# zhuker/lamejs

Measured on AMD Instinct MI355X. Metric: 1152-sample frames/s encoded (44.1kHz 128kbps CBR); bit-exact, higher is better.
Workload: dtype f64; 1 GPU; BASELINE configs[2]: stereo 44.1kHz 128kbps CBR, 1 stream(s) x 100000 synthetic sine frames per GPU; input=Int16 PCM resident in HBM, output=MP3 bytes in HBM, seed_repaired_frames=0, distinct_streams=1, distinct_devices=1

## Files before the change

### lamejs_amd/csrc/k_psy.h

```cpp
#pragma once
#include <type_traits>
#include "lhip_defs.h"
#include "lhip_wave.h"
#include "lhip_math.h"
#include "lhip_layout.h"

namespace lhip {

#ifdef LHIP_NO_FZ_PAD
LHIP_DEV int fzp(int a) { return a; }
LHIP_DEV int fzo(int c) { return c; }
#else
LHIP_DEV int fzp(int a) { return a + (a >> 5); }
LHIP_DEV int fzo(int c) { return c + (c >> 5); }
#endif
LHIP_DEV void fht_item0(float* fz, int base, int k1, int kx, int m) {
    const int k2 = k1 << 1, k3 = k2 + k1, k4 = k2 << 1;
    const int K1 = fzo(k1), K2 = fzo(k2), K3 = fzo(k3);
    float* fi = fz + fzp(base + m * k4);
    float* gi = fz + fzp(base + m * k4 + kx);
    double f0, f1, f2, f3;
    f1 = (double)fi[0] - (double)fi[K1];
    f0 = (double)fi[0] + (double)fi[K1];
    f3 = (double)fi[K2] - (double)fi[K3];
    f2 = (double)fi[K2] + (double)fi[K3];
    fi[K2] = (float)(f0 - f2);
    fi[0] = (float)(f0 + f2);
    fi[K3] = (float)(f1 - f3);
    fi[K1] = (float)(f1 + f3);
    f1 = (double)gi[0] - (double)gi[K1];
    f0 = (double)gi[0] + (double)gi[K1];
    f3 = LHIP_SQRT2 * (double)gi[K3];
    f2 = LHIP_SQRT2 * (double)gi[K2];
    gi[K2] = (float)(f0 - f2);
    gi[0] = (float)(f0 + f2);
    gi[K3] = (float)(f1 - f3);
    gi[K1] = (float)(f1 + f3);
}
LHIP_DEV void fht_item1(float* fz, int base, int k1, int kx, int m, int i, const double* tw) {
    const int k2 = k1 << 1, k3 = k2 + k1, k4 = k2 << 1;
    const int K1 = fzo(k1), K2 = fzo(k2), K3 = fzo(k3);
    (void)kx;
    float* fi = fz + fzp(base + m * k4 + i);
    float* gi = fz + fzp(base + m * k4 + k1 - i);
    const double c1 = tw[4 * (i - 1) + 0], s1 = tw[4 * (i - 1) + 1], c2 = tw[4 * (i - 1) + 2], s2 = tw[4 * (i - 1) + 3];
    double a, b, g0, f0, f1, g1, f2, g2, f3, g3;
    b = s2 * (double)fi[K1] - c2 * (double)gi[K1];
    a = c2 * (double)fi[K1] + s2 * (double)gi[K1];
    f1 = (double)fi[0] - a;
    f0 = (double)fi[0] + a;
    g1 = (double)gi[0] - b;
    g0 = (double)gi[0] + b;
    b = s2 * (double)fi[K3] - c2 * (double)gi[K3];
    a = c2 * (double)fi[K3] + s2 * (double)gi[K3];
    f3 = (double)fi[K2] - a;
    f2 = (double)fi[K2] + a;
    g3 = (double)gi[K2] - b;
    g2 = (double)gi[K2] + b;
    b = s1 * f2 - c1 * g3;
    a = c1 * f2 + s1 * g3;
    fi[K2] = (float)(f0 - a);
    fi[0] = (float)(f0 + a);
    gi[K3] = (float)(g1 - b);
    gi[K1] = (float)(g1 + b);
    b = c1 * g2 - s1 * f3;
    a = s1 * g2 + c1 * f3;
    gi[K2] = (float)(g0 - a);
    gi[0] = (float)(g0 + a);
    fi[K3] = (float)(f1 - b);
    fi[K1] = (float)(f1 + b);
}
LHIP_DEV void fht_pass(float* fz, int n, int k1, int kx, int lane, int nl, int base, const double* tw) {
    const int items = n / 8, nz = items / kx, kx1 = kx - 1;
    for (int t = lane - base; t < nz; t += nl) if (t >= 0) fht_item0(fz, 0, k1, kx, t);
    for (int t = lane - base; t < items - nz; t += nl) if (t >= 0) { const int m = t / kx1; fht_item1(fz, 0, k1, kx, m, 1 + t - m * kx1, tw); }
}

LHIP_DEV void fht_pass_blocks(float* fz, int nb, int n, int k1, int kx, int lane, int nl, const double* tw) {
    const int items = n / 8, nz = items / kx, kx1 = kx - 1, n1 = items - nz;
    for (int t = lane; t < nb * nz; t += nl) { const int b = t / nz; fht_item0(fz, b * n, k1, kx, t - b * nz); }
    for (int t = lane; t < nb * n1; t += nl) {
        const int b = t / n1, r = t - b * n1, m = r / kx1;
        fht_item1(fz, b * n, k1, kx, m, 1 + r - m * kx1, tw);
    }
}

struct PsyALds {
    float fz[BLKSIZE + BLKSIZE / 32];
    float fs[3][BLKSIZE_s];
    float fs_pad[3 * BLKSIZE_s / 32];
};
static_assert(offsetof(PsyALds, fs_pad) == offsetof(PsyALds, fs) + sizeof(float) * 3 * BLKSIZE_s, "the short transform buffer is one flat padded array");
#define PSYA_FE(L) ((L).fz)
#define PSYA_FES(L, b) ((L).fs[b])
#define PSYA_EB(L) ((L).fz + 516)
#define PSYA_MX(L) ((L).fz + 516 + CBANDS)
#define PSYA_AV(L) ((L).fz + 516 + 2 * CBANDS)
#define PSYA_EBS(L, b) ((L).fz + 516 + (3 + (b)) * CBANDS)

#if defined(LHIP_PHASE_PROF) && !defined(LHIP_HOSTSIM)
#define PSY_STAMP(i) psy_t_[i] = __builtin_amdgcn_s_memtime()
#define PSY_FLUSH() do { if (lane == 0 && ((gslot & 63) == 0 || (W.ngslots <= 4 && ch == 0 && gslot - sd.gslot0 == 1))) {    if (psy_t_[2] == 0) psy_t_[2] = psy_t_[1]; \
    for (int i_ = 0; i_ < 7; i_++) atomicAdd((unsigned long long*)W.prof + 22 + i_, psy_t_[i_ + 1] - psy_t_[i_]); atomicAdd((unsigned long long*)W.prof + 54, 1ull); } } while (0)
#define PSY_DECL() unsigned long long psy_t_[8] = {0, 0, 0, 0, 0, 0, 0, 0}
#else
#define PSY_STAMP(i) do {} while (0)
#define PSY_FLUSH() do {} while (0)
#define PSY_DECL() do {} while (0)
#endif
template <int K> LHIP_DEV int guarded_f32_of_sum(const double (&p)[K], double scale, double add, float* out) {
#if LHIP_NL == 1
    (void)p; (void)scale; (void)add; (void)out;
    return 0;
#else
    double s = 0.0;
#pragma unroll
    for (int k = 0; k < K; k++) s += p[k];
    s = wave_sumd(s);
    const float lo = (float)((s * (1.0 - 2e-13)) * scale + add), hi = (float)((s * (1.0 + 2e-13)) * scale + add);
    *out = lo;
#ifdef LHIP_WAVESIM
    if (lo == hi) {
        const float ref = (float)(wave_seq_sum<K>(p) * scale + add);
        if (ref != lo) { fprintf(stderr, "wavesim: guarded_f32_of_sum disagrees with the sequential sum (%a vs %a)\n", (double)lo, (double)ref); abort(); }
    }
#endif
    return lo == hi;
#endif
}

template <int F32, int UNIT, int MIX>
LHIP_DEV void psya_stage_new(const PcmSrc& P, int first, int lane, float* fz) {
    typedef typename std::conditional<F32 != 0, float, int16_t>::type elem_t;
    const int str = UNIT ? 1 : P.stride;
    const elem_t* src = (const elem_t*)P.src + (int64_t)first * str;
    if (MIX == 2) {
        const elem_t* src2 = (const elem_t*)P.src2 + (int64_t)first * str;
        enum { STG = 8 };
        for (int i0 = lane; i0 < BLKSIZE; i0 += LHIP_NL * STG) {
            typename std::conditional<F32 != 0, float, int>::type ra[STG], rb[STG];
#pragma unroll
            for (int k = 0; k < STG; k++) {
                int i = i0 + LHIP_NL * k;
                if (i >= BLKSIZE) i = BLKSIZE - 1;
                ra[k] = src[i * str]; rb[k] = src2[i * str];
            }
#pragma unroll
            for (int k = 0; k < STG; k++) { LHIP_PIN_LOADED(ra[k]); LHIP_PIN_LOADED(rb[k]); }
#pragma unroll
            for (int k = 0; k < STG; k++) {
                const int i = i0 + LHIP_NL * k;
                float v = F32 ? pcm_f32_clean((float)ra[k], P.limit) : (float)ra[k];
                if (P.do_scale) v = (float)((double)v * P.scale);
                v = pcm_mix(P, v, F32 ? pcm_f32_clean((float)rb[k], P.limit) : (float)rb[k]);
                if (i < BLKSIZE) fz[i] = v;
            }
        }
        return;
    }
    for (int i = lane; i < BLKSIZE; i += LHIP_NL) {
        float v = F32 ? pcm_f32_clean((float)src[i * str], P.limit) : (float)src[i * str];
        if (P.do_scale) v = (float)((double)v * P.scale);
        if (MIX) v = pcm_mix(P, v, 0.f);
        fz[i] = v;
    }
}

template <int PART = 0>
LHIP_DEV void kb_psyA(const Tables& T, const Workspace& W, const StreamDesc* SD, const StreamIO* IO, int gslot, int ch, int lane, PsyALds& L) {
    const int C = T.channels_out, Cp = T.psy_channels;
    const int st = W.gslot_stream[gslot];
    const StreamDesc sd = SD[st];
    const int q = gslot - sd.gslot0 - 1;
    if (q < 0) return;
    if (PART != 4 && ch < 2) {
        const PcmSrc P = pcm_source(T, W, sd, IO[st], ch);
        const int b0 = 576 * q + 304;
        if (!P.plane && b0 >= P.mf) {
            if (!P.mix) {
                if (!P.f32 && P.stride == 1) psya_stage_new<0, 1, 0>(P, b0 - P.mf, lane, L.fz);
                else if (!P.f32) psya_stage_new<0, 0, 0>(P, b0 - P.mf, lane, L.fz);
                else psya_stage_new<1, 0, 0>(P, b0 - P.mf, lane, L.fz);
            } else if (P.mix == 1) {
                if (!P.f32) psya_stage_new<0, 0, 1>(P, b0 - P.mf, lane, L.fz);
                else psya_stage_new<1, 0, 1>(P, b0 - P.mf, lane, L.fz);
            } else {
                if (!P.f32) psya_stage_new<0, 0, 2>(P, b0 - P.mf, lane, L.fz);
                else psya_stage_new<1, 0, 2>(P, b0 - P.mf, lane, L.fz);
            }
        } else {
            for (int i = lane; i < BLKSIZE; i += LHIP_NL) L.fz[i] = pcm_at(P, b0 + i);
        }
        wave_sync();
    }
#define buf(i) L.fz[i]
    const int64_t o = (int64_t)gslot * Cp + ch;
    PSY_DECL();
    PSY_STAMP(0);

    if (PART == 4) goto psya_tail;
    if (PART == 0 || PART == 1) {
        const float* fir = L.fz + 397;
        enum { HO = (576 + LHIP_NL - 1) / LHIP_NL };
        float* mag = &L.fs[0][0];
        if (ch >= 2) {
            const float* hl = W.hpf + (int64_t)gslot * 2 * 576;
            for (int i = lane; i < 576; i += LHIP_NL) {
                const double l = hl[i], r = hl[576 + i];
                float v = (ch == 2) ? (float)(l + r) : (float)(l - r);
                mag[i] = v < 0 ? -v : v;
            }
        } else {
            double x[HO + 21];
#pragma unroll
            for (int t = 0; t < HO + 21; t++) { const int n = HO * lane + t; x[t] = (n < 576 + 21) ? (double)fir[n] : 0.0; }
#pragma unroll
            for (int k = 0; k < HO; k++) {
                double sum1 = x[k + 10], sum2 = 0.0;
#pragma unroll
                for (int j = 0; j < 9; j += 2) {
                    sum1 += T.hpf_fircoef[j] * (x[k + j] + x[k + 21 - j]);
                    sum2 += T.hpf_fircoef[j + 1] * (x[k + j + 1] + x[k + 21 - j - 1]);
                }
                float v = (float)(sum1 + sum2);
                if (Cp == 4 && HO * lane + k < 576) W.hpf[((int64_t)gslot * 2 + ch) * 576 + HO * lane + k] = v;
                v = v < 0 ? -v : v;
                if (HO * lane + k < 576) mag[HO * lane + k] = v;
            }
        }
        wave_sync();
        enum { KP = (64 + LHIP_NL - 1) / LHIP_NL };
        float pk[9];
#pragma unroll
        for (int sbk = 0; sbk < 9; sbk++) {
            float m = 1.0f;
            for (int u = 0; u < KP; u++) { const float v = mag[sbk * 64 + lane + LHIP_NL * u]; if (m < v) m = v; }
            pk[sbk] = m;
        }
        wave_sync();
        {
            int pb[9];
#pragma unroll
            for (int sbk = 0; sbk < 9; sbk++) __builtin_memcpy(&pb[sbk], &pk[sbk], 4);
            wave_max_n(pb);
#pragma unroll
            for (int sbk = 0; sbk < 9; sbk++) __builtin_memcpy(&pk[sbk], &pb[sbk], 4);
        }
        if (lane == 0) {
#pragma unroll
            for (int sbk = 0; sbk < 9; sbk++) W.peaks[o * PK_STRIDE + sbk] = pk[sbk];
        }
    }
    if (PART == 1) return;

    PSY_STAMP(1);
    if (ch >= 2) {
        const float* fl = W.fht + (int64_t)gslot * 2 * FHT_STRIDE;
        for (int i = lane; i < FHT_STRIDE; i += LHIP_NL) {
            const double l = fl[i], r = fl[FHT_STRIDE + i];
            const float v = (ch == 2) ? (float)((l + r) * LHIP_SQRT2 * 0.5) : (float)((l - r) * LHIP_SQRT2 * 0.5);
            if (i < BLKSIZE) L.fz[fzp(i)] = v; else (&L.fs[0][0])[fzp(i - BLKSIZE)] = v;
        }
        wave_sync();
    } else {
    for (int it = lane; it < 3 * (BLKSIZE_s / 8); it += LHIP_NL) {
        const int b = it / (BLKSIZE_s / 8), j = it - b * (BLKSIZE_s / 8);
        const int k = (576 / 3) * (b + 1);
        const int i = T.fft_rv_tbl[j << 2] & 0xff;
        float* x = &L.fs[0][0] + fzp(b * BLKSIZE_s + 4 * j);
        double f0, f1, f2, f3, w;
        f0 = (double)T.window_s[i] * (double)buf(i + k);
        w = (double)T.window_s[0x7f - i] * (double)buf(i + k + 0x80);
        f1 = f0 - w; f0 = f0 + w;
        f2 = (double)T.window_s[i + 0x40] * (double)buf(i + k + 0x40);
        w = (double)T.window_s[0x3f - i] * (double)buf(i + k + 0xc0);
        f3 = f2 - w; f2 = f2 + w;
        x[0] = (float)(f0 + f2); x[2] = (float)(f0 - f2); x[1] = (float)(f1 + f3); x[3] = (float)(f1 - f3);
        f0 = (double)T.window_s[i + 0x01] * (double)buf(i + k + 0x01);
        w = (double)T.window_s[0x7e - i] * (double)buf(i + k + 0x81);
        f1 = f0 - w; f0 = f0 + w;
        f2 = (double)T.window_s[i + 0x41] * (double)buf(i + k + 0x41);
        w = (double)T.window_s[0x3e - i] * (double)buf(i + k + 0xc1);
        f3 = f2 - w; f2 = f2 + w;
        x[fzo(BLKSIZE_s / 2) + 0] = (float)(f0 + f2); x[fzo(BLKSIZE_s / 2) + 2] = (float)(f0 - f2);
        x[fzo(BLKSIZE_s / 2) + 1] = (float)(f1 + f3); x[fzo(BLKSIZE_s / 2) + 3] = (float)(f1 - f3);
    }
    {
        enum { KL = (BLKSIZE / 8 + LHIP_NL - 1) / LHIP_NL };
        float xin[KL][8];
#pragma unroll
        for (int u = 0; u < KL; u++) {
            const int jj = lane + LHIP_NL * u;
            if (jj < BLKSIZE / 8) {
                const int i = T.fft_rv_tbl[jj] & 0xff;
                xin[u][0] = buf(i); xin[u][1] = buf(i + 0x200); xin[u][2] = buf(i + 0x100); xin[u][3] = buf(i + 0x300);
                xin[u][4] = buf(i + 0x001); xin[u][5] = buf(i + 0x201); xin[u][6] = buf(i + 0x101); xin[u][7] = buf(i + 0x301);
            }
        }
        wave_sync();
#pragma unroll
        for (int u = 0; u < KL; u++) {
            const int jj = lane + LHIP_NL * u;
            if (jj < BLKSIZE / 8) {
                const int i = T.fft_rv_tbl[jj] & 0xff;
                float* x = L.fz + fzp(4 * jj);
                double f0, f1, f2, f3, w;
                f0 = (double)T.window[i] * (double)xin[u][0];
                w = (double)T.window[i + 0x200] * (double)xin[u][1];
                f1 = f0 - w; f0 = f0 + w;
                f2 = (double)T.window[i + 0x100] * (double)xin[u][2];
                w = (double)T.window[i + 0x300] * (double)xin[u][3];
                f3 = f2 - w; f2 = f2 + w;
                x[0] = (float)(f0 + f2); x[2] = (float)(f0 - f2); x[1] = (float)(f1 + f3); x[3] = (float)(f1 - f3);
                f0 = (double)T.window[i + 0x001] * (double)xin[u][4];
                w = (double)T.window[i + 0x201] * (double)xin[u][5];
                f1 = f0 - w; f0 = f0 + w;
                f2 = (double)T.window[i + 0x101] * (double)xin[u][6];
                w = (double)T.window[i + 0x301] * (double)xin[u][7];
                f3 = f2 - w; f2 = f2 + w;
                x[fzo(BLKSIZE / 2) + 0] = (float)(f0 + f2); x[fzo(BLKSIZE / 2) + 2] = (float)(f0 - f2);
                x[fzo(BLKSIZE / 2) + 1] = (float)(f1 + f3); x[fzo(BLKSIZE / 2) + 3] = (float)(f1 - f3);
            }
        }
    }
    wave_sync();

    PSY_STAMP(2);
    {
        int off = 0;
#pragma unroll
        for (int k1 = 4, kx = 2; k1 < BLKSIZE; k1 <<= 2, kx <<= 2) {
            fht_pass(L.fz, BLKSIZE, k1, kx, lane, LHIP_NL, 0, T.fht_twiddle + 4 * off);
            if (k1 < BLKSIZE_s) fht_pass_blocks(&L.fs[0][0], 3, BLKSIZE_s, k1, kx, lane, LHIP_NL, T.fht_twiddle + 4 * off);
            wave_sync();
            off += kx - 1;
        }
    }
    if (Cp == 4) {
        float* fo = W.fht + ((int64_t)gslot * 2 + ch) * FHT_STRIDE;
        for (int i = lane; i < FHT_STRIDE; i += LHIP_NL) fo[i] = (i < BLKSIZE) ? L.fz[fzp(i)] : (&L.fs[0][0])[fzp(i - BLKSIZE)];
    }
    }

    PSY_STAMP(3);
    {
        enum { KE = (BLKSIZE / 2 + 1 + LHIP_NL - 1) / LHIP_NL, KS = (3 * (BLKSIZE_s / 2 + 1) + LHIP_NL - 1) / LHIP_NL };
        float el[KE], es[KS];
#pragma unroll
        for (int u = 0; u < KE; u++) {
            const int j = lane + LHIP_NL * u;
            el[u] = 0.f;
            if (j == 0) { const float e0 = L.fz[0]; el[u] = (float)((double)e0 * (double)e0); }
            else if (j <= BLKSIZE / 2) { const double re = L.fz[fzp(j)], im = L.fz[fzp(BLKSIZE - j)]; el[u] = (float)((re * re + im * im) * 0.5); }
        }
#pragma unroll
        for (int u = 0; u < KS; u++) {
            const int it = lane + LHIP_NL * u;
            es[u] = 0.f;
            if (it < 3 * (BLKSIZE_s / 2 + 1)) {
                const int b = it / (BLKSIZE_s / 2 + 1), j = it - b * (BLKSIZE_s / 2 + 1);
                const float* fsf = &L.fs[0][0];
                if (j == 0) { const float e0 = fsf[fzp(b * BLKSIZE_s)]; es[u] = (float)((double)e0 * (double)e0); }
                else { const double re = fsf[fzp(b * BLKSIZE_s + j)], im = fsf[fzp(b * BLKSIZE_s + BLKSIZE_s - j)]; es[u] = (float)((re * re + im * im) * 0.5); }
            }
        }
        wave_sync();
#pragma unroll
        for (int u = 0; u < KE; u++) { const int j = lane + LHIP_NL * u; if (j <= BLKSIZE / 2) PSYA_FE(L)[j] = el[u]; }
#pragma unroll
        for (int u = 0; u < KS; u++) {
            const int it = lane + LHIP_NL * u;
            if (it < 3 * (BLKSIZE_s / 2 + 1)) { const int b = it / (BLKSIZE_s / 2 + 1), j = it - b * (BLKSIZE_s / 2 + 1); PSYA_FES(L, b)[j] = es[u]; }
        }
    }
    wave_sync();

    PSY_STAMP(4);
    {
        enum { K = (BLKSIZE / 2) / LHIP_NL };
        double pr[K];
#pragma unroll
        for (int k = 0; k < K; k++) { const int i = K * lane + k; pr[k] = (double)PSYA_FE(L)[i] * (double)T.eql_w[i]; }
        if (ch < 2) {
            float lf;
            if (!guarded_f32_of_sum<K>(pr, T.VO_SCALE, 0.0, &lf)) lf = (float)(wave_seq_sum<K>(pr) * T.VO_SCALE);
            if (lane == 0) W.loud[(int64_t)gslot * C + ch] = lf;
        }
        if (Cp == 4) {
#pragma unroll
            for (int k = 0; k < K; k++) { const int i = K * lane + k; pr[k] = (i >= 11) ? (double)PSYA_FE(L)[i] : 0.0; }
            const double last = (double)PSYA_FE(L)[BLKSIZE / 2];
            float tf;
            if (!guarded_f32_of_sum<K>(pr, 1.0, last, &tf)) tf = (float)(wave_seq_sum<K>(pr) + last);
            if (lane == 0) W.tot_ener[(int64_t)gslot * 4 + ch] = tf;
        }
    }

    PSY_STAMP(5);
    if (PART == 3) return;
psya_tail:
#if LHIP_NL == 1
    LHIP_LANE_ONCE(b, 0, T.npart_l) {
        double ebb = 0, m = 0;
        int j = T.lineoff_l[b];
        for (int i = 0; i < T.numlines_l[b]; ++i, ++j) {
            const double el = PSYA_FE(L)[j];
            ebb += el;
            if (m < el) m = el;
        }
        PSYA_EB(L)[b] = (float)ebb;
        PSYA_MX(L)[b] = (float)m;
        PSYA_AV(L)[b] = (float)(ebb * (double)T.rnumlines_l[b]);
    }
#else
    {
        enum { KF = 8 };
        static_assert(BLKSIZE / 2 == KF * LHIP_NL, "psy_fold is laid out for 8 lines per lane");
        const int32_t* pf = T.psy_fold + 3 * lane;
        const uint32_t marks = (uint32_t)pf[0], pw0 = (uint32_t)pf[1], pw1 = (uint32_t)pf[2];
        LHIP_LANE_ONCE(b, 0, CBANDS) PSYA_MX(L)[b] = 0.f;
        double tq[KF], keep[KF];
        float ev[KF];
#pragma unroll
        for (int k = 0; k < KF; k++) { ev[k] = PSYA_FE(L)[KF * lane + k]; tq[k] = (double)ev[k]; keep[k] = one_unless_bit(marks, k); }
        const float e512 = PSYA_FE(L)[BLKSIZE / 2];
        wave_sync();
        {
            float m = 0.f;
#pragma unroll
            for (int k = 0; k < KF; k++) {
                m = ((marks >> k) & 1u) ? ev[k] : fmax_nonneg(m, ev[k]);
                const int bnd = (int)(((k < 4 ? pw0 : pw1) >> (8 * (k & 3))) & 0xffu);
                float mm = m;
                if (lane == LHIP_NL - 1 && k == KF - 1 && !((marks >> (8 + k)) & 1u)) mm = fmax_nonneg(mm, e512);
                if (((marks >> (8 + k)) & 1u) || k == KF - 1) { int32_t bits; __builtin_memcpy(&bits, &mm, 4); lds_max((int32_t*)&PSYA_MX(L)[bnd], bits); }
            }
            if (lane == LHIP_NL - 1 && ((marks >> (8 + KF - 1)) & 1u)) {
                int32_t bits; __builtin_memcpy(&bits, &e512, 4); lds_max((int32_t*)&PSYA_MX(L)[T.npart_l - 1], bits);
            }
        }
        const int nsteps = (T.psy_maxlen_l + KF - 1) / KF + 1;
        double carry = 0.0;
        for (int st = 0; st + 1 < nsteps; st++) {
            double sacc = carry;
#pragma unroll
            for (int k = 0; k < KF; k++) sacc = __builtin_fma(sacc, keep[k], tq[k]);
            carry = wave_shr1d(sacc, 0.0);
        }
        {
            double sacc = carry;
#pragma unroll
            for (int k = 0; k < KF; k++) { sacc = __builtin_fma(sacc, keep[k], tq[k]); tq[k] = sacc; }
        }
#pragma unroll
        for (int k = 0; k < KF; k++) {
            const int bnd = (int)(((k < 4 ? pw0 : pw1) >> (8 * (k & 3))) & 0xffu);
            if ((marks >> (8 + k)) & 1u) { PSYA_EB(L)[bnd] = (float)tq[k]; PSYA_AV(L)[bnd] = (float)(tq[k] * (double)T.rnumlines_l[bnd]); }
        }
        if (lane == LHIP_NL - 1) {
            const int bl = T.npart_l - 1;
            const double ebb = ((marks >> (8 + KF - 1)) & 1u) ? (double)e512 : tq[KF - 1] + (double)e512;
            PSYA_EB(L)[bl] = (float)ebb; PSYA_AV(L)[bl] = (float)(ebb * (double)T.rnumlines_l[bl]);
        }
    }
#endif
    for (int it = lane; it < 3 * T.npart_s; it += LHIP_NL) {
        const int sblock = it / T.npart_s, b = it - sblock * T.npart_s;
        double ebb = 0;
        int j = T.lineoff_s[b];
        for (int i = 0; i < T.numlines_s[b]; ++i, ++j) ebb += (double)PSYA_FES(L, sblock)[j];
        PSYA_EBS(L, sblock)[b] = (float)ebb;
    }
    wave_sync();

    PSY_STAMP(6);
    for (int b = lane; b < CBANDS; b += LHIP_NL) {
        int k = 0;
        float ebv = 0.f;
        if (b < T.npart_l) {
            const int last = T.npart_l - 1;
            const int lo = b > 0 ? b - 1 : b, hi = b < last ? b + 1 : b;
            double a, m;
            int nl;
            if (b == 0) { a = (double)PSYA_AV(L)[0] + (double)PSYA_AV(L)[1]; nl = T.numlines_l[0] + T.numlines_l[1] - 1; }
            else if (b == last) { a = (double)PSYA_AV(L)[b - 1] + (double)PSYA_AV(L)[b]; nl = T.numlines_l[b - 1] + T.numlines_l[b] - 1; }
            else { a = (double)PSYA_AV(L)[b - 1] + (double)PSYA_AV(L)[b] + (double)PSYA_AV(L)[b + 1]; nl = T.numlines_l[b - 1] + T.numlines_l[b] + T.numlines_l[b + 1] - 1; }
            if (a > 0.0) {
                m = PSYA_MX(L)[lo];
                for (int t = lo + 1; t <= hi; t++) if (m < (double)PSYA_MX(L)[t]) m = PSYA_MX(L)[t];
                a = 20.0 * (m * (double)(hi - lo + 1) - a) / (a * nl);
                k = js_toint32(a);
                if (k > 8) k = 8;
            }
            ebv = PSYA_EB(L)[b];
        }
        W.eb_l[o * EBL_STRIDE + b] = ebv;
        W.mask_idx[o * EBL_STRIDE + b] = k;
    }
    for (int b = lane; b < CBANDS; b += LHIP_NL) {
        float ecbv[3] = {0.f, 0.f, 0.f}, ebv[3] = {0.f, 0.f, 0.f};
        if (b < T.npart_s) {
            enum { MT = 12 };
            const int k0 = T.s3ind_s[2 * b], k1 = T.s3ind_s[2 * b + 1], j0 = T.s3off_s[b];
            float cf[MT];
#pragma unroll
            for (int u = 0; u < MT; u++) cf[u] = (k0 + u <= k1) ? T.s3_ss[j0 + u] : 0.f;
            for (int sblock = 0; sblock < 3; sblock++) {
                const float* e = PSYA_EBS(L, sblock);
                double ecb = (double)cf[0] * (double)e[k0];
#pragma unroll
                for (int u = 1; u < MT; u++) if (k0 + u <= k1) ecb += (double)cf[u] * (double)e[k0 + u];
                for (int kk = k0 + MT; kk <= k1; kk++) ecb += (double)T.s3_ss[j0 + (kk - k0)] * (double)e[kk];
                ecbv[sblock] = (float)ecb;
                ebv[sblock] = e[b];
            }
        }
        for (int sblock = 0; sblock < 3; sblock++) {
            W.ecb_s[o * EBS_STRIDE + sblock * CBANDS + b] = ecbv[sblock];
            W.eb_s[o * EBS_STRIDE + sblock * CBANDS + b] = ebv[sblock];
        }
    }
    PSY_STAMP(7);
    if (PART == 0 || PART == 2) PSY_FLUSH();
#undef buf
}

LHIP_DEV int attack_flags_raw(const Tables& T, const float* cur, const float* prev, int chn) {
    const double thr = (chn == 3) ? T.attackthre_s : T.attackthre;
    float ai[4];
    ai[0] = (float)((double)prev[6] / (double)prev[4]);
    const double refv[3] = {(double)prev[7], (double)cur[1], (double)cur[4]};
    for (int t = 0; t < 3; t++) {
        double p = cur[3 * t];
        const double r = refv[t];
        if (p > r) p = p / r;
        else if (r > p * 10.0) p = r / (p * 10.0);
        else p = 0.0;
        ai[t + 1] = (float)p;
    }
    double en_short[4];
    en_short[0] = 0.0;
    for (int i = 0; i < 3; i++) en_short[0] += (double)prev[i + 6];
    en_short[1] = 0.0 + (double)cur[0]; en_short[2] = 0.0 + (double)cur[3]; en_short[3] = 0.0 + (double)cur[6];
    int a[4];
    for (int j = 0; j < 4; j++) a[j] = ((double)ai[j] > thr) ? 1 : 0;
    for (int i = 1; i < 4; i++) {
        double ratio;
        if (en_short[i - 1] > en_short[i]) ratio = en_short[i - 1] / en_short[i];
        else ratio = en_short[i] / en_short[i - 1];
        if (ratio < 1.7) { a[i] = 0; if (i == 1) a[0] = 0; }
    }
    return a[0] | (a[1] << 1) | (a[2] << 2) | (a[3] << 3);
}

LHIP_DEV void kb_scan_raw(const Tables& T, const Workspace& W, const StreamDesc* SD, int gslot) {
    const int Cp = T.psy_channels;
    const StreamDesc sd = SD[W.gslot_stream[gslot]];
    if (gslot - sd.gslot0 - 1 < 0) return;
    for (int ch = 0; ch < Cp; ch++) {
        const int64_t o = (int64_t)gslot * Cp + ch;
        W.att_raw[o] = attack_flags_raw(T, W.peaks + o * PK_STRIDE, W.peaks + (o - Cp) * PK_STRIDE, ch);
    }
}

LHIP_DEV int last_attack_after(const Workspace& W, int C, int gcarry, int gslot, int ch) {
    int flips = 0, g = gslot;
    for (;;) {
        if (g == gcarry) { const int v = W.last_attack[(int64_t)g * C + ch] != 0; return flips ? !v : v; }
        const int raw = W.att_raw[(int64_t)g * C + ch];
        const int a0 = raw & 1, a1 = (raw >> 1) & 1, a2 = (raw >> 2) & 1;
        int v;
        if (!a2) v = 0;
        else if (!a1) v = 1;
        else if (!a0) v = 0;
        else { flips ^= 1; g--; continue; }
        return flips ? !v : v;
    }
}

LHIP_DEV void kb_scan_attack(const Tables& T, const Workspace& W, const StreamDesc* SD, int gslot) {
    const int C = T.channels_out, Cp = T.psy_channels;
    const StreamDesc sd = SD[W.gslot_stream[gslot]];
    if (gslot - sd.gslot0 - 1 < 0) return;
    int ul[2] = {1, 1};
    for (int ch = 0; ch < Cp; ch++) {
        const int last = last_attack_after(W, Cp, sd.gslot0, gslot - 1, ch);
        const int raw = W.att_raw[(int64_t)gslot * Cp + ch];
        int a0 = raw & 1, a1 = (raw >> 1) & 1, a2 = (raw >> 2) & 1, a3 = (raw >> 3) & 1;
        if (a0 != 0 && last != 0) a0 = 0;
        if ((a0 + a1 + a2 + a3) != 0) {
            if (ch < 2) ul[ch] = 0;
            else ul[0] = ul[1] = 0;
            if (a1 != 0 && a0 != 0) a1 = 0;
            if (a2 != 0 && a1 != 0) a2 = 0;
            if (a3 != 0 && a2 != 0) a3 = 0;
        }
        W.att_clean[(int64_t)gslot * Cp + ch] = a0 | (a1 << 1) | (a2 << 2) | (a3 << 3);
        W.ul_tmp[(int64_t)gslot * Cp + ch] = a2;
    }
    if (T.short_blocks_coupled && !(ul[0] != 0 && ul[1] != 0)) ul[0] = ul[1] = 0;
    for (int ch = 0; ch < C; ch++) W.uselong[(int64_t)gslot * C + ch] = ul[ch];
}

LHIP_DEV void kb_scan_blocktype(const Tables& T, const Workspace& W, const StreamDesc* SD, int gslot) {
    const int C = T.channels_out;
    const StreamDesc sd = SD[W.gslot_stream[gslot]];
    const int q = gslot - sd.gslot0 - 1;
    if (q < 0) return;
    for (int ch = 0; ch < C; ch++) {
        int old;
        if (q == 0) old = W.tent[(int64_t)sd.gslot0 * C + ch];
        else {
            const int ul1 = W.uselong[(int64_t)(gslot - 1) * C + ch];
            int pshort;
            if (q == 1) pshort = W.tent[(int64_t)sd.gslot0 * C + ch] == SHORT_TYPE;
            else pshort = W.uselong[(int64_t)(gslot - 2) * C + ch] == 0;
            old = ul1 ? (pshort ? STOP_TYPE : NORM_TYPE) : SHORT_TYPE;
        }
        const int ul = W.uselong[(int64_t)gslot * C + ch];
        W.prev_short[(int64_t)gslot * C + ch] = (old == SHORT_TYPE) ? 1 : 0;
        int bt = NORM_TYPE;
        if (ul != 0) { if (old == SHORT_TYPE) bt = STOP_TYPE; }
        else {
            bt = SHORT_TYPE;
            if (old == NORM_TYPE) old = START_TYPE;
            if (old == STOP_TYPE) old = SHORT_TYPE;
        }
        W.blocktype[(int64_t)gslot * C + ch] = old;
        W.tent[(int64_t)gslot * C + ch] = bt;
    }
    const int Cp = T.psy_channels;
    for (int ch = 0; ch < Cp; ch++) W.last_attack[(int64_t)gslot * Cp + ch] = W.ul_tmp[(int64_t)gslot * Cp + ch];
}

#if defined(LHIP_HOSTSIM) && defined(LHIP_WAVESIM)
enum { ATH_NT = 128, ATH_SEG = 2 };
LHIP_DEV void block_sync() { wg_barrier(); }
LHIP_DEV int block_any(int p) { static int any_ = 0; wg_barrier(); if (p) any_ = 1; wg_barrier(); const int r = any_; wg_barrier(); any_ = 0; return r; }
#elif defined(LHIP_HOSTSIM)
enum { ATH_NT = 1, ATH_SEG = 1 << 20 };
LHIP_DEV void block_sync() {}
LHIP_DEV int block_any(int p) { return p != 0; }
#else
enum { ATH_NT = 1024, ATH_SEG = 16 };
LHIP_DEV void block_sync() { __syncthreads(); }
LHIP_DEV int block_any(int p) { return __syncthreads_or(p); }
#endif
struct AthLds { double e_adj[ATH_NT + 1], e_lim[ATH_NT + 1]; int known[ATH_NT + 1], first_reset[ATH_NT + 1]; double c_adj, c_lim, c_mp; };

LHIP_DEV void ath_step(const Tables& T, double max_pow, double& adj, double& lim) {
    if (T.ATH_useAdjust == 0) { adj = 1.0; return; }
    if (max_pow > 0.03125) {
        if (adj >= 1.0) adj = 1.0;
        else if (adj < lim) adj = lim;
        lim = 1.0;
    } else {
        const double adj_lim_new = 31.98 * max_pow + 0.000625;
        if (adj >= adj_lim_new) {
            adj *= adj_lim_new * 0.075 + 0.925;
            if (adj < adj_lim_new) adj = adj_lim_new;
        } else {
            if (lim >= adj_lim_new) adj = adj_lim_new;
            else if (adj < lim) adj = lim;
        }
        lim = adj_lim_new;
    }
}

LHIP_DEV double ath_max_pow(const Tables& T, const Workspace& W, const StreamDesc& sd, int C, int k) {
    const int GR = T.mode_gr;
    const int64_t g0 = (int64_t)(sd.gslot0 + GR * k) * C, g1 = g0 + C;
    double max_pow = W.loud[g0], gr2_max = (GR == 2) ? (double)W.loud[g1] : 0.0;
    if (C == 2) { max_pow += (double)W.loud[g0 + 1]; if (GR == 2) gr2_max += (double)W.loud[g1 + 1]; }
    else { max_pow += max_pow; gr2_max += gr2_max; }
    if (GR == 2) max_pow = max_pow > gr2_max ? max_pow : gr2_max;
    max_pow *= 0.5;
    max_pow *= T.ATH_aaSensitivityP;
    return max_pow;
}

LHIP_DEV void kb_scan_ath(const Tables& T, const Workspace& W, const StreamDesc* SD, int st, int tid, AthLds& L) {
    const int C = T.channels_out;
    const StreamDesc sd = SD[st];
    if (tid == 0) { L.c_adj = W.ath_adjust[sd.fslot0]; L.c_lim = W.ath_limit[sd.fslot0]; L.c_mp = 0.0; }
    block_sync();
    for (int k0 = 0; k0 < sd.nframes; k0 += ATH_NT * ATH_SEG) {
        const int rem = sd.nframes - k0;
        const int n = rem < ATH_NT * ATH_SEG ? rem : ATH_NT * ATH_SEG;
        const int seglen = (n + ATH_NT - 1) / ATH_NT;
        const int s0 = tid * seglen < n ? tid * seglen : n, s1 = (tid + 1) * seglen < n ? (tid + 1) * seglen : n;
        const double cadj = L.c_adj, clim = L.c_lim, prev_mp = L.c_mp;
        {
            int fr = -1;
            if (T.ATH_useAdjust != 0) {
                double pm = (s0 < s1) ? (s0 > 0 ? ath_max_pow(T, W, sd, C, k0 + s0 - 1) : prev_mp) : 0.0;
                for (int k = s0; k < s1; k++) {
                    const double m = ath_max_pow(T, W, sd, C, k0 + k);
                    if (pm > 0.03125 && m > 0.03125) { fr = k; break; }
                    pm = m;
                }
            } else if (s0 < s1) fr = s0;
            double a = 1.0, l = 1.0;
            if (fr >= 0) {
                l = (T.ATH_useAdjust != 0) ? 1.0 : clim;
                W.ath_adjust[sd.fslot0 + 1 + k0 + fr] = 1.0; W.ath_limit[sd.fslot0 + 1 + k0 + fr] = l;
                for (int k = fr + 1; k < s1; k++) {
                    ath_step(T, ath_max_pow(T, W, sd, C, k0 + k), a, l);
                    W.ath_adjust[sd.fslot0 + 1 + k0 + k] = a; W.ath_limit[sd.fslot0 + 1 + k0 + k] = l;
                }
            }
            L.first_reset[tid] = fr;
            L.known[tid + 1] = (fr >= 0) || (s0 >= s1);
            L.e_adj[tid + 1] = a; L.e_lim[tid + 1] = l;
            if (tid == 0) { L.known[0] = 1; L.e_adj[0] = cadj; L.e_lim[0] = clim; }
        }
        block_sync();
        int done = (s0 >= s1);
        for (int round = 0; round < ATH_NT + 1; round++) {
            int progressed = 0;
            if (!done && L.known[tid]) {
                double a = L.e_adj[tid], l = L.e_lim[tid];
                const int fr = L.first_reset[tid];
                const int stop = fr >= 0 ? fr : s1;
                for (int k = s0; k < stop; k++) {
                    ath_step(T, ath_max_pow(T, W, sd, C, k0 + k), a, l);
                    W.ath_adjust[sd.fslot0 + 1 + k0 + k] = a; W.ath_limit[sd.fslot0 + 1 + k0 + k] = l;
                }
                if (fr < 0) { L.e_adj[tid + 1] = a; L.e_lim[tid + 1] = l; }
                done = 1; progressed = 1;
            }
            block_sync();
            if (progressed && L.first_reset[tid] < 0) L.known[tid + 1] = 1;
            if (s0 >= s1 && L.known[tid] && !L.known[tid + 1]) { L.e_adj[tid + 1] = L.e_adj[tid]; L.e_lim[tid + 1] = L.e_lim[tid]; L.known[tid + 1] = 1; }
            block_sync();
            if (!block_any(!done || !L.known[tid + 1])) break;
        }
        if (s0 < s1 && s1 == n) { L.c_adj = L.e_adj[tid + 1]; L.c_lim = L.e_lim[tid + 1]; L.c_mp = ath_max_pow(T, W, sd, C, k0 + n - 1); }
        block_sync();
    }
}

struct PsyBTabs { double mt1[25], mt2[10], mt3[14], mtab[9]; };
enum { PSYB_S3_LDS = 1024 };
template <int NCH> struct PsyBLdsT : PsyBTabs {
    double ebm[CBANDS], athc[CBANDS];
    float thr_l[NCH][CBANDS + 2];
    union {
        struct { float thr_s[NCH][3][CBANDS + 2]; float E[NCH][E_STRIDE]; };
        float s3[PSYB_S3_LDS];
    };
};
typedef PsyBLdsT<2> PsyBLds;
typedef PsyBLdsT<4> PsyBLds4;

LHIP_DEV int ma_index16(double ratio) {
    const float t = fast_log2f((float)ratio) * 4.81647993062369912f;
    const float k = __builtin_floorf(t);
    const float fr = t - k;
    int i = -1;
    if (fr >= 2e-4f && fr <= 1.0f - 2e-4f) i = (int)k;
#ifdef LHIP_HOSTSIM
    if (i >= 0 && i != js_toint32(v8_log10_pos(ratio) * 16.0)) { fprintf(stderr, "hostsim: ma_index16 disagrees with the logarithm at %a\n", ratio); abort(); }
#endif
    return i;
}
LHIP_DEV int ma_index16_exact(double ratio) {
    int i = ma_index16(ratio);
    if (i < 0) i = js_toint32(v8_log10_pos(ratio) * 16.0);
    return i;
}

LHIP_DEV double mask_add_l(const Tables& T, const PsyBTabs& L, double ath_cb, double m1, double m2, int b) {
    double ratio;
    if (m2 > m1) {
        if (m2 < (m1 * T.ma_max_i2)) ratio = m2 / m1;
        else return (m1 + m2);
    } else {
        if (m1 >= (m2 * T.ma_max_i2)) return (m1 + m2);
        ratio = m1 / m2;
    }
    m1 += m2;
    if ((b + 3) <= 3 + 3) {
        if (ratio >= T.ma_max_i1) return m1;
        const int i = ma_index16_exact(ratio);
        return m1 * L.mt2[i];
    }
    const int i = ma_index16_exact(ratio);
    m2 = ath_cb;
    if (m1 < T.ma_max_m * m2) {
        if (m1 > m2) {
            double f = 1.0;
            if (i <= 13) f = L.mt3[i];
            const double r = v8_log10_pos(m1 / m2) * (10.0 / 15.0);
            return m1 * ((L.mt1[i] - f) * r + f);
        }
        if (i > 13) return m1;
        return m1 * L.mt3[i];
    }
    return m1 * L.mt1[i];
}


LHIP_DEV double ns_interp(double x, double y, double r) {
    if (r >= 1.0) return x;
    if (r <= 0.0) return y;
    if (y > 0.0) return v8_pow(x / y, r) * y;
    return 0.0;
}

template <int NCH> LHIP_DEV void kb_psyB(const Tables& T, const PowBase& pb10, const Workspace& W, const StreamDesc* SD, int gslot, int lane, PsyBLdsT<NCH>& L, int par = -1,
                                         int resv_size = 0, int resv_max = 0) {
    const int C = T.channels_out, Cp = T.psy_channels;
    const int st = W.gslot_stream[gslot];
    const StreamDesc sd = SD[st];
    const int q = gslot - sd.gslot0 - 1;
    if (q < 0) return;
    if (par >= 0 && q % T.mode_gr != par) return;
    double pcfact = 0.0;
    if (!T.disable_reservoir) pcfact = resv_max == 0 ? 0.0 : (double)resv_size / resv_max * 0.5;
    const int fs = sd.fslot0 + q / T.mode_gr;
    const double ath_adjust = W.ath_adjust[fs];
    for (int i = lane; i < 25; i += LHIP_NL) {
        L.mt1[i] = T.ma_table1[i];
        if (i < 10) L.mt2[i] = T.ma_table2[i];
        if (i < 14) L.mt3[i] = T.ma_table3[i];
        if (i < 9) L.mtab[i] = T.ma_tab[i];
    }
    wave_sync();

    for (int i = lane; i < T.n_s3_ll; i += LHIP_NL) L.s3[i] = T.s3_ll[i];
    LHIP_LANE_ONCE(k, 0, T.npart_l) L.athc[k] = (double)T.ATH_cb_l[k] * ath_adjust;
    for (int ch = 0; ch < Cp; ch++) {
        const int64_t o = (int64_t)gslot * Cp + ch;
        const float* eb_l = W.eb_l + o * EBL_STRIDE;
        const int32_t* midx = W.mask_idx + o * EBL_STRIDE;
        LHIP_LANE_ONCE(k, 0, T.npart_l) L.ebm[k] = (double)eb_l[k] * L.mtab[midx[k]];
        wave_sync();
        LHIP_LANE_ONCE(b, 0, T.npart_l) {
            const int k0 = T.s3ind[2 * b], k1 = T.s3ind[2 * b + 1], j0 = T.s3off_l[b];
            double ecb = (double)L.s3[j0] * L.ebm[k0];
            for (int kk = k0 + 1; kk <= k1; kk++)
                ecb = mask_add_l(T, L, L.athc[kk], ecb, (double)L.s3[j0 + (kk - k0)] * L.ebm[kk], kk - b);
            ecb *= 0.158489319246111;
            float thr = (float)ecb;
            if (!T.disable_reservoir) {
                const float n1 = W.nb1[(o - Cp) * EBL_STRIDE + b], n2 = W.nb2[(o - Cp) * EBL_STRIDE + b];
                if (pcfact > 0.0 && !W.prev_short[(int64_t)gslot * C + (ch & 1)]) {
                    const double a = 2 * (double)n1, b2 = 16 * (double)n2, m = a < b2 ? a : b2;
                    thr = (float)ns_interp(ecb < m ? ecb : m, ecb, pcfact);
                }
                W.nb2[o * EBL_STRIDE + b] = n1;
                W.nb1[o * EBL_STRIDE + b] = (float)ecb;
            }
            L.thr_l[ch][b] = thr;
        }
        wave_sync();
    }
    for (int ch = 0; ch < Cp; ch++) {
        const int64_t o = (int64_t)gslot * Cp + ch;
        const int pshort = W.prev_short[(int64_t)gslot * C + (ch & 1)];
        for (int it = lane; it < 3 * T.npart_s; it += LHIP_NL) {
            const int sblock = it / T.npart_s, b = it - sblock * T.npart_s;
            const float* e0 = W.ecb_s + o * EBS_STRIDE;
            const float* em = W.ecb_s + (o - Cp) * EBS_STRIDE;
            const float ecb = e0[sblock * CBANDS + b];
            const float nb1 = sblock >= 1 ? e0[(sblock - 1) * CBANDS + b] : em[2 * CBANDS + b];
            const float nb2 = sblock >= 2 ? e0[(sblock - 2) * CBANDS + b] : em[(sblock + 1) * CBANDS + b];
            double x = 2 * (double)nb1;
            float thr = (float)((double)ecb < x ? (double)ecb : x);
            if (pshort) {
                x = 16 * (double)nb2;
                const double y = thr;
                thr = (float)(x < y ? x : y);
            }
            L.thr_s[ch][sblock][b] = thr;
        }
    }
    wave_sync();

    for (int ch = 0; ch < Cp; ch++) {
        const int64_t o = (int64_t)gslot * Cp + ch;
        const float* eb_l = W.eb_l + o * EBL_STRIDE;
        float* Eo = L.E[ch];
        for (int sb = lane; sb < SBMAX_l; sb += LHIP_NL) {
            const int npart = T.npart_l;
            const int bstart = sb == 0 ? 0 : T.bo_l[sb - 1];
            float en_f = 0.f, thm_f = 0.f;
            if (sb == 0 || bstart < npart) {
                double enn = 0.0, thmm = 0.0;
                int b = bstart;
                if (sb > 0) {
                    const double w_next = 1.0 - (double)T.bo_l_weight[sb - 1];
                    enn = w_next * (double)eb_l[b];
                    thmm = w_next * (double)L.thr_l[ch][b];
                    b++;
                }
                const int bo = T.bo_l[sb];
                const int b_lim = bo < npart ? bo : npart;
                while (b < b_lim) { enn += (double)eb_l[b]; thmm += (double)L.thr_l[ch][b]; b++; }
                en_f = (float)enn; thm_f = (float)thmm;
                if (b < npart) {
                    const double w_curr = T.bo_l_weight[sb];
                    en_f = (float)((double)en_f + w_curr * (double)eb_l[b]);
                    thm_f = (float)((double)thm_f + w_curr * (double)L.thr_l[ch][b]);
                }
            }
            Eo[E_EN_L + sb] = en_f;
            Eo[E_THM_L + sb] = thm_f;
        }
        for (int it = lane; it < 3 * SBMAX_s; it += LHIP_NL) {
            const int sblock = it / SBMAX_s, sb = it - sblock * SBMAX_s;
            const float* ebs = W.eb_s + o * EBS_STRIDE + sblock * CBANDS;
            const float* thr = L.thr_s[ch][sblock];
            const int npart = T.npart_s;
            const int bstart = sb == 0 ? 0 : T.bo_s[sb - 1];
            float en_f = 0.f, thm_f = 0.f;
            if (sb == 0 || bstart < npart) {
                double enn = 0.0, thmm = 0.0;
                int b = bstart;
                if (sb > 0) {
                    const double w_next = 1.0 - (double)T.bo_s_weight[sb - 1];
                    enn = w_next * (double)ebs[b];
                    thmm = w_next * (double)thr[b];
                    b++;
                }
                const int bo = T.bo_s[sb];
                const int b_lim = bo < npart ? bo : npart;
                while (b < b_lim) { enn += (double)ebs[b]; thmm += (double)thr[b]; b++; }
                en_f = (float)enn; thm_f = (float)thmm;
                if (b < npart) {
                    const double w_curr = T.bo_s_weight[sb];
                    en_f = (float)((double)en_f + w_curr * (double)ebs[b]);
                    thm_f = (float)((double)thm_f + w_curr * (double)thr[b]);
                }
            }
            Eo[E_EN_S + sb * 3 + sblock] = en_f;
            Eo[E_THM_S + sb * 3 + sblock] = thm_f;
        }
    }
    wave_sync();
    for (int ch = 0; ch < Cp; ch++) {
        const int64_t o = (int64_t)gslot * Cp + ch;
        const float* pk = W.peaks + o * PK_STRIDE;
        const int att = W.att_clean[o];
        float* Eo = L.E[ch];
        LHIP_LANE_ONCE(sb, 0, SBMAX_s) {
            float prev = pcfact > 0.0 ? W.E[(o - Cp) * E_STRIDE + E_THM_S + sb * 3 + 2] : 0.f;
            for (int sblock = 0; sblock < 3; sblock++) {
                double thmm = Eo[E_THM_S + sb * 3 + sblock];
                thmm *= 0.8;
                if ((att >> (sblock + 1)) & 1) { const double p = ns_interp(prev, thmm, 0.6 * pcfact); thmm = thmm < p ? thmm : p; }
                if ((att >> sblock) & 1) { const double p = ns_interp(prev, thmm, 0.3 * pcfact); thmm = thmm < p ? thmm : p; }
                const double e3 = pk[sblock * 3 + 0], e4 = pk[sblock * 3 + 1], e5 = pk[sblock * 3 + 2];
                const double enn = e3 + e4 + e5;
                if (e5 * 6 < enn) {
                    thmm *= 0.5;
                    if (e4 * 6 < enn) thmm *= 0.5;
                }
                prev = (float)thmm;
                Eo[E_THM_S + sb * 3 + sblock] = prev;
            }
        }
    }
    wave_sync();
    if ((T.mode == 0 || T.mode == 1) && T.interChRatio > 0.0 && C > 1) {
        const double r_ = T.interChRatio;
        float nl[2] = {0.f, 0.f};
        for (int i = lane; i < SBMAX_l + 3 * SBMAX_s; i += LHIP_NL) {
            const int idx = E_THM_L + i;
            const double l = L.E[0][idx], r = L.E[1][idx];
            nl[0] = (float)(l + r * r_);
            nl[1] = (float)(r + l * r_);
            L.E[0][idx] = nl[0];
            L.E[1][idx] = nl[1];
        }
        wave_sync();
    }
    if constexpr (NCH == 4) if (Cp == 4) {
        const double msfix = T.msfix;
        const bool do_ns = d_abs(msfix) > 0.0;
        const double athlower_l = do_ns ? v8_pow_base(pb10, T.ATHlower * ath_adjust) : 0.0;
        const double athlower_s = athlower_l * ((double)BLKSIZE_s / BLKSIZE);
        for (int i = lane; i < SBMAX_l + 3 * SBMAX_s; i += LHIP_NL) {
            const int it = E_THM_L + i, ie = E_EN_L + i;
            const bool lng = i < SBMAX_l;
            const int sb = lng ? i : (i - SBMAX_l) / 3;
            float t0 = L.E[0][it], t1 = L.E[1][it], t2 = L.E[2][it], t3 = L.E[3][it];
            if (!((double)t0 > 1.58 * (double)t1 || (double)t1 > 1.58 * (double)t0)) {
                const double m = lng ? (double)T.mld_l[sb] : (double)T.mld_s[sb];
                double mld = m * (double)L.E[3][ie];
                const double lo1 = (double)t3 < mld ? (double)t3 : mld;
                const double rmid = (double)t2 > lo1 ? (double)t2 : lo1;
                mld = m * (double)L.E[2][ie];
                const double lo2 = (double)t2 < mld ? (double)t2 : mld;
                const double rside = (double)t3 > lo2 ? (double)t3 : lo2;
                t2 = (float)rmid; t3 = (float)rside;
            }
            if (do_ns) {
                const double ath = lng ? (double)T.ATH_cb_l[T.bm_l[sb]] * athlower_l : (double)T.ATH_cb_s[T.bm_s[sb]] * athlower_s;
                const double a0 = (double)t0 > ath ? (double)t0 : ath, a1 = (double)t1 > ath ? (double)t1 : ath;
                const double thmLR = a0 < a1 ? a0 : a1;
                double thmM = (double)t2 > ath ? (double)t2 : ath, thmS = (double)t3 > ath ? (double)t3 : ath;
                if (thmLR * (msfix * 2.0) < thmM + thmS) {
                    const double f = thmLR * (msfix * 2.0) / (thmM + thmS);
                    thmM *= f;
                    thmS *= f;
                }
                t2 = (float)(thmM < (double)t2 ? thmM : (double)t2);
                t3 = (float)(thmS < (double)t3 ? thmS : (double)t3);
            }
            L.E[2][it] = t2; L.E[3][it] = t3;
        }
        wave_sync();
    }
    for (int ch = 0; ch < Cp; ch++)
        for (int i = lane; i < E_STRIDE; i += LHIP_NL) W.E[((int64_t)gslot * Cp + ch) * E_STRIDE + i] = L.E[ch][i];
}

}
```

### lamejs_amd/csrc/lhip_api.cpp

```cpp
#include "../../include/lamejs_hip.h"
#include "lhip_defs.h"
#include "lhip_wave.h"
#include "lhip_math.h"
#include "lhip_layout.h"
#include "k_psy.h"
#include "k_fb.h"
#include "k_quant.h"
#if !defined(LHIP_HOSTSIM) || defined(LHIP_WAVESIM)
#include "k_quant_tail.h"
#endif
#include "k_quant_fast.h"
#include "k_quant_probe.h"
#include "k_bits.h"
#include "k_crc.h"
#include "k_ingest.h"
#include "k_gain.h"

#include <string>
#include <vector>
#include <map>
#include <mutex>
#include <thread>
#include <atomic>
#include <memory>
// ... 325 lines not shown
    std::vector<int16_t> zeros(z, 0);
    const void* l = zeros.data();
    const void* r = zeros.data();
    int64_t w = 0;
    const double end_padding = flush_end_padding(s);
    const int rc = tagged_call(&s, 1, nullptr, &out, &out_cap, &w, false, [&](uint8_t* const* o, const size_t* c, int64_t* wr) -> int {
        return encode_many(&s, 1, LHIP_PCM_S16, &l, &r, &z, o, c, wr, false, true, true); });
    if (rc < 0) return rc;
    s->mf_samples_to_encode = 0;
    if (s->tag) { s->tag->padding = end_padding; s->tag->flushed = true; }
    return w;
}

static int encode_batch_pcm_inner(lhip_stream* const* streams, size_t nstreams, int format, const void* const* left, const void* const* right,
                                  const size_t* nsamples, uint8_t* const* out, const size_t* out_cap, int64_t* written);
int lhip_encode_batch_pcm(lhip_stream* const* streams, size_t nstreams, int format, const void* const* left, const void* const* right,
                          const size_t* nsamples, uint8_t* const* out, const size_t* out_cap, int64_t* written) {
    return tagged_call(streams, nstreams, nsamples, out, out_cap, written, false, [&](uint8_t* const* o, const size_t* c, int64_t* wr) -> int {
        return encode_batch_pcm_inner(streams, nstreams, format, left, right, nsamples, o, c, wr); });
}
static int encode_batch_pcm_inner(lhip_stream* const* streams, size_t nstreams, int format, const void* const* left, const void* const* right,
                                  const size_t* nsamples, uint8_t* const* out, const size_t* out_cap, int64_t* written) {
    if (!fmt_ok(format)) { set_err("unknown sample format"); return LHIP_ERR_INTERNAL; }
    if (fmt_scanned(format) && streams && left && nsamples)
        for (size_t i = 0; i < nstreams; i++)
            if (streams[i] && streams[i]->magic == 0x4c484950 && !host_samples_ok(i, streams[i]->ts->T.channels_in, streams[i]->ts->T.pcm_limit, format, left[i], right ? right[i] : nullptr, nsamples[i])) {
                for (size_t k = 0; k < nstreams; k++) if (written) written[k] = LHIP_ERR_INTERNAL;
                return LHIP_ERR_INTERNAL;
            }
    if (nstreams > 1 && streams && left && nsamples && out && out_cap) {
        static const bool no_chunk = []() { const char* e = getenv("LAMEJS_HIP_NO_HOST_CHUNKS"); return e && e[0] == '1'; }();
        bool ok = !no_chunk;
        size_t total = 0;
        for (size_t i = 0; i < nstreams && ok; i++) {
            ok = streams[i] && streams[i]->magic == 0x4c484950 && streams[i]->ctx == streams[0]->ctx && streams[i]->ts.get() == streams[0]->ts.get() && left[i] && nsamples[i] > 0;
            if (ok) for (size_t k = 0; k < i; k++) if (streams[k] == streams[i]) { ok = false; break; }
            total += nsamples[i];
        }
        if (ok && streams[0]->ts->T.disable_reservoir && !streams[0]->ts->T.rs_frac) {
            const Tables& T = streams[0]->ts->T;
            if (total > (size_t)4 * host_chunk_schedule().first * 576 * T.mode_gr * T.rs_ratio) return encode_host_groups(streams, nstreams, format, left, right, nsamples, out, out_cap, written);
        }
    }
    return encode_many(streams, nstreams, format, left, right, nsamples, out, out_cap, written, false, true);
}
int lhip_encode_batch(lhip_stream* const* streams, size_t nstreams, const int16_t* const* left, const int16_t* const* right,
                      const size_t* nsamples, uint8_t* const* out, const size_t* out_cap, int64_t* written) {
    return lhip_encode_batch_pcm(streams, nstreams, LHIP_PCM_S16, (const void* const*)left, (const void* const*)right, nsamples, out, out_cap, written);
}

int lhip_flush_batch(lhip_stream* const* streams, size_t nstreams, uint8_t* const* out, const size_t* out_cap, int64_t* written) {
    std::vector<std::vector<int16_t>> zs(nstreams);
    std::vector<const void*> l(nstreams);
    std::vector<size_t> ns(nstreams);
    bool any_frac = false;
    for (size_t i = 0; i < nstreams; i++) any_frac |= streams[i] && streams[i]->magic == 0x4c484950 && streams[i]->ts->T.rs_frac;
    if (any_frac) {
        int rc = 0;
        for (size_t i = 0; i < nstreams; i++) {
            const int64_t w = lhip_flush(streams[i], out[i], out_cap[i]);
            if (written) written[i] = w;
            if (w < 0 && rc == 0) rc = (int)w;
        }
        return rc;
    }
    for (size_t i = 0; i < nstreams; i++) {
        if (!streams[i] || streams[i]->magic != 0x4c484950) { set_err("bad stream handle"); return LHIP_ERR_BAD_HANDLE; }
        ns[i] = flush_zeros(streams[i]);
        zs[i].assign(ns[i] ? ns[i] : 1, 0);
        l[i] = zs[i].data();
    }
    std::vector<double> end_padding(nstreams);
    for (size_t i = 0; i < nstreams; i++) end_padding[i] = flush_end_padding(streams[i]);
    const int rc = tagged_call(streams, nstreams, ns.data(), out, out_cap, written, false, [&](uint8_t* const* o, const size_t* c, int64_t* wr) -> int {
        return encode_many(streams, nstreams, LHIP_PCM_S16, l.data(), l.data(), ns.data(), o, c, wr, false, true, true); });
    if (rc >= 0) for (size_t i = 0; i < nstreams; i++) {
        streams[i]->mf_samples_to_encode = 0;
        if (streams[i]->tag && ns[i] > 0) { streams[i]->tag->padding = end_padding[i]; streams[i]->tag->flushed = true; }
    }
    return rc;
}

int lhip_encode_batch_device(lhip_stream* const* streams, size_t nstreams, const int16_t* const* d_left, const int16_t* const* d_right,
                             const size_t* nsamples, uint8_t* const* d_out, const size_t* out_cap, int64_t* written, int sync) {
    return lhip_encode_batch_device_pcm(streams, nstreams, LHIP_PCM_S16, (const void* const*)d_left, (const void* const*)d_right, nsamples, d_out, out_cap, written, sync);
}
int lhip_encode_batch_device_pcm(lhip_stream* const* streams, size_t nstreams, int format, const void* const* d_left, const void* const* d_right,
                                 const size_t* nsamples, uint8_t* const* d_out, const size_t* out_cap, int64_t* written, int sync) {
    if (!fmt_ok(format)) { set_err("unknown sample format"); return LHIP_ERR_INTERNAL; }
    return tagged_call(streams, nstreams, nsamples, d_out, out_cap, written, true, [&](uint8_t* const* o, const size_t* c, int64_t* wr) -> int {
        return encode_many(streams, nstreams, format, d_left, d_right, nsamples, o, c, wr, true, sync != 0); });
}
int64_t lhip_last_batch_rejected_samples(void) {
    if (g_rej_pending) {
        Context* ctx = g_rej_pending;
        g_rej_pending = nullptr;
        std::lock_guard<std::mutex> lk(ctx->mu);
        unsigned long long v = 0;
        if (!rt::set_device(ctx->device) || !rt::d2h(&v, ctx->ws.rejected.p, sizeof v, ctx->stream) || !rt::sync(ctx->stream)) return LHIP_ERR_INTERNAL;
        g_rejected = (int64_t)v;
    }
    return g_rejected;
}

struct StateHdr { uint32_t magic, bytes; int32_t mf_size, mf_samples_to_encode, slot_lag, config; int64_t frame_num, rs_n_in; };
static int32_t state_config_tag(const Tables& T) {
    const int32_t f[] = {T.channels_out, T.mode, T.disable_reservoir != 0, T.samplerate_index, T.version, T.bitrate_index, T.rs_ratio,
                         T.out_samplerate, T.in_samplerate, T.brate, T.mode_gr, T.psy_channels};
    uint32_t h = 2166136261u;
    for (int32_t v : f) for (int b = 0; b < 4; b++) { h ^= (uint32_t)(v >> (8 * b)) & 0xffu; h *= 16777619u; }
    return (int32_t)h;
}
size_t lhip_state_bytes(const lhip_stream* s) {
    if (!s || s->magic != 0x4c484950) return 0;
    return sizeof(StateHdr) + sizeof(StreamState);
}
int lhip_state_get(lhip_stream* s, void* buf, size_t cap) {
    if (!s || s->magic != 0x4c484950) { set_err("bad stream handle"); return LHIP_ERR_BAD_HANDLE; }
    if (s->ts->T.rs_frac) { set_err("lhip_state_get: not for fractionalResample streams (call-sequence streams: the resampler's clock is not part of the state record)"); return LHIP_ERR_INTERNAL; }
    if (!buf || cap < lhip_state_bytes(s)) { set_err("state buffer too small"); return LHIP_ERR_BUFFER_TOO_SMALL; }
    Context* ctx = s->ctx;
    std::lock_guard<std::mutex> lk(ctx->mu);
    if (!rt::set_device(ctx->device)) return LHIP_ERR_INTERNAL;
    StateHdr h; memset(&h, 0, sizeof h);
    h.magic = 0x5453484cu; h.bytes = (uint32_t)lhip_state_bytes(s);
    h.mf_size = s->mf_size; h.mf_samples_to_encode = s->mf_samples_to_encode; h.slot_lag = s->slot_lag; h.frame_num = s->frame_num; h.rs_n_in = s->rs_n_in;
    h.config = state_config_tag(s->ts->T);
    memcpy(buf, &h, sizeof h);
    if (!rt::set_device(ctx->device) || !rt::d2h((uint8_t*)buf + sizeof h, s->d_state, sizeof(StreamState), ctx->stream) || !rt::sync(ctx->stream)) return LHIP_ERR_INTERNAL;
    {
        const Tables& T = s->ts->T;
        StreamState* S = (StreamState*)((uint8_t*)buf + sizeof h);
        for (int ch = 0; ch < 2; ch++) {
            const int live = ch < T.channels_out ? s->mf_size : 0;
            for (int i = live; i < MF_NEEDED; i++) S->pcm_tail[ch][i] = 0.f;
        }
        if (T.rs_ratio == 1) memset(S->rs_old, 0, sizeof S->rs_old);
        if (T.disable_reservoir) { memset(S->nb1, 0, sizeof S->nb1); memset(S->nb2, 0, sizeof S->nb2); memset(&S->rv, 0, sizeof S->rv); }
    }
    return 0;
}
int lhip_state_set(lhip_stream* s, const void* buf, size_t n) {
    if (!s || s->magic != 0x4c484950) { set_err("bad stream handle"); return LHIP_ERR_BAD_HANDLE; }
    StateHdr h;
    if (s->ts->T.rs_frac) { set_err("lhip_state_set: not for fractionalResample streams"); return LHIP_ERR_INTERNAL; }
    if (!buf || n < sizeof h) { set_err("state blob too small"); return LHIP_ERR_INTERNAL; }
    memcpy(&h, buf, sizeof h);
    Context* ctx = s->ctx;
    std::lock_guard<std::mutex> lk(ctx->mu);
    if (h.magic != 0x5453484cu || h.bytes != lhip_state_bytes(s) || n < h.bytes || h.config != state_config_tag(s->ts->T)) { set_err("state blob does not belong to this build / configuration"); return LHIP_ERR_INTERNAL; }
    if (!rt::set_device(ctx->device)) return LHIP_ERR_INTERNAL;
    if (!rt::set_device(ctx->device) || !rt::h2d(s->d_state, (const uint8_t*)buf + sizeof h, sizeof(StreamState), ctx->stream) || !rt::sync(ctx->stream)) return LHIP_ERR_INTERNAL;
    s->mf_size = h.mf_size; s->mf_samples_to_encode = h.mf_samples_to_encode; s->slot_lag = h.slot_lag; s->frame_num = h.frame_num; s->rs_n_in = h.rs_n_in;
    if (s->tag) s->tag->moved = true;
    if (s->gain) s->gain->moved = true;
    return 0;
}
size_t lhip_seek_tail_samples(const lhip_stream* s) {
    if (!s || s->magic != 0x4c484950) return 0;
    return (size_t)(MF_INIT + 576 * s->ts->T.mode_gr);
}
int lhip_seek(lhip_stream* s, int64_t sample_pos, const int16_t* tail_left, const int16_t* tail_right) {
    if (!s || s->magic != 0x4c484950) { set_err("bad stream handle"); return LHIP_ERR_BAD_HANDLE; }
    const Tables& T = s->ts->T;
    const int frame = 576 * T.mode_gr, ntail = MF_INIT + frame;
    Context* ctx = s->ctx;
    std::lock_guard<std::mutex> lk(ctx->mu);
    if (T.rs_ratio != 1 || !T.disable_reservoir) { set_err("lhip_seek: not for resampling or bit-reservoir streams"); return LHIP_ERR_INTERNAL; }
    if (s->frame_num != 0 || s->mf_size != MF_INIT) { set_err("lhip_seek: the stream has been used"); return LHIP_ERR_INTERNAL; }
    if (sample_pos < 2 * frame || sample_pos % frame != 0 || !tail_left) { set_err("lhip_seek: position must be a whole number (>= 2) of frames"); return LHIP_ERR_INTERNAL; }
    if (T.channels_in == 2 && !tail_right) { set_err("lhip_seek: a two-channel stream needs both tails"); return LHIP_ERR_INTERNAL; }
    const bool down = T.in_mix == 2;
    std::vector<float> t((size_t)2 * MF_NEEDED, 0.f);
    for (int ch = 0; ch < T.channels_out; ch++) {
        const int16_t* src = (ch == 1 && tail_right) ? tail_right : tail_left;
        const bool do_g2 = ch ? T.do_scale_right : T.do_scale_left;
        const double g2 = ch ? T.scale_right : T.scale_left;
        for (int i = 0; i < ntail; i++) {
            float v = (float)src[i];
            if (T.do_scale) v = (float)((double)v * T.scale);
            if (do_g2) v = (float)((double)v * g2);
            if (down) {
                float b = (float)tail_right[i];
                if (T.do_scale_right) b = (float)((double)b * T.scale_right);
                v = (float)(0.5 * ((double)v + (double)b));
            }
            t[(size_t)ch * MF_NEEDED + i] = v;
        }
    }
    if (!rt::set_device(ctx->device) || !rt::h2d((uint8_t*)s->d_state + offsetof(StreamState, pcm_tail), t.data(), sizeof(float) * 2 * MF_NEEDED, ctx->stream) || !rt::sync(ctx->stream)) return LHIP_ERR_INTERNAL;
    const int64_t k = sample_pos / frame;
    s->frame_num = k - 1;
    if (s->tag) s->tag->moved = true;
    if (s->gain) s->gain->moved = true;
    s->rs_n_in = sample_pos;
    s->mf_size = ntail;
    s->mf_samples_to_encode = 576 + 1152 + frame;
    if (T.frac_SpF != 0) {
        int64_t m = ((int64_t)T.frac_SpF - (k - 1) * (int64_t)T.frac_SpF) % T.out_samplerate;
        if (m < 0) m += T.out_samplerate;
        s->slot_lag = (int)m;
    }
    return 0;
}

int64_t lhip_frac_call_limit(const lhip_stream* s) {
    if (!s || s->magic != 0x4c484950) { set_err("bad stream handle"); return LHIP_ERR_BAD_HANDLE; }
    return s->ts->T.rs_frac ? frac_call_limit(s->ts->T) : 0;
}
int lhip_debug_frac_call(const lhip_stream* s, size_t nsamples, int32_t* k, int32_t* frames) {
    if (!s || s->magic != 0x4c484950) { set_err("bad stream handle"); return LHIP_ERR_BAD_HANDLE; }
    const Tables& T = s->ts->T;
    if (!T.rs_frac) { set_err("not a fractionalResample stream"); return LHIP_ERR_INTERNAL; }
    const FracPass fp = frac_pass(T, s->rs_itime, (double)nsamples);
    if (k) *k = fp.k;
    const int F = call_frames(s, nsamples);
    if (frames) *frames = F;
    if (F < 0) { set_err(frac_refusal(T, nsamples)); return LHIP_ERR_INTERNAL; }
    return 0;
}
int lhip_debug_frac_flush(const lhip_stream* s, int32_t* bytes, int32_t* clean, int cap) {
    if (!s || s->magic != 0x4c484950) { set_err("bad stream handle"); return LHIP_ERR_BAD_HANDLE; }
    if (!s->ts->T.rs_frac) { set_err("not a fractionalResample stream"); return LHIP_ERR_INTERNAL; }
    std::vector<FracStep> steps;
    if (!frac_flush_plan(s, steps)) return LHIP_ERR_INTERNAL;
    int n = 0;
    for (const FracStep& st : steps) if (st.frame) { if (n < cap) { if (bytes) bytes[n] = st.bytes; if (clean) clean[n] = st.clean ? 1 : 0; } n++; }
    return n;
}

int lhip_debug_release_context(int device) {
#ifndef LHIP_HOSTSIM
    Context* ctx = get_context(device);
    std::lock_guard<std::mutex> lk(ctx->mu);
    if (ctx->live_streams != 0) { set_err("lhip_debug_release_context: the context still has streams"); return LHIP_ERR_INTERNAL; }
    if (!rt::set_device(ctx->device)) return LHIP_ERR_INTERNAL;
    (void)hipStreamSynchronize((hipStream_t)ctx->stream);
    WorkSet& ws = ctx->ws;
    if (ws.aux_stream) { (void)hipStreamSynchronize((hipStream_t)ws.aux_stream); (void)hipStreamDestroy((hipStream_t)ws.aux_stream); (void)hipEventDestroy((hipEvent_t)ws.ev_fork); (void)hipEventDestroy((hipEvent_t)ws.ev_join); ws.aux_stream = ws.ev_fork = ws.ev_join = nullptr; }
    if (ctx->own_stream) { (void)hipStreamDestroy((hipStream_t)ctx->stream); ctx->stream = nullptr; ctx->own_stream = false; }
#else
    (void)device;
#endif
    return 0;
}

int lhip_set_hip_stream(int device, void* hip_stream) {
#ifndef LHIP_HOSTSIM
    if (device < 0) { if (hipGetDevice(&device) != hipSuccess) return LHIP_ERR_INTERNAL; }
#else
    if (device < 0) device = 0;
#endif
    Context* ctx = get_context(device);
    std::lock_guard<std::mutex> lk(ctx->mu);
    ctx->stream = hip_stream;
    return 0;
}

void lhip_last_batch_stats(int64_t* frames, int64_t* repaired_frames, int64_t* repair_iterations) {
#ifndef LHIP_HOSTSIM
    if (g_stat_pending) {
        Context* ctx = g_stat_pending;
        g_stat_pending = nullptr;
        std::lock_guard<std::mutex> lk(ctx->mu);
        int32_t fx[3] = {0, 0, 0};
        WorkSet& ws = ctx->ws;
        void* st = ctx->stream;
        if (rt::set_device(ctx->device) && rt::d2h(fx, (const int32_t*)ws.nflagged.p + FX_STATS, sizeof fx, st) && rt::sync(st)) {
            g_stat_repaired = fx[0]; g_stat_iters = fx[1];
            if (fx[2]) set_err("seed-chain repair did not converge");
        }
    }
#endif
    if (frames) *frames = g_stat_frames;
    if (repaired_frames) *repaired_frames = g_stat_repaired;
    if (repair_iterations) *repair_iterations = g_stat_iters;
}

int lhip_debug_last_paths(uint32_t* mask) {
    if (!mask) { set_err("lhip_debug_last_paths: null argument"); return LHIP_ERR_INTERNAL; }
    *mask = g_last_paths;
    return 0;
}

int64_t lhip_debug_read(int what, void* dst, size_t cap) {
    if (what == 11) {
        if (!dst) { set_err("lhip_debug_read: null argument"); return LHIP_ERR_INTERNAL; }
        const size_t n = cap < sizeof g_last_quant ? cap : sizeof g_last_quant; memcpy(dst, &g_last_quant, n); return (int64_t)n;
    }
#ifdef LHIP_HOSTSIM
    if (what == 10) {
        const int64_t v[2] = {(int64_t)__atomic_load_n(&round_stats().head, __ATOMIC_RELAXED), (int64_t)__atomic_load_n(&round_stats().full, __ATOMIC_RELAXED)};
        const size_t n = cap < sizeof v ? cap : sizeof v; memcpy(dst, v, n); return (int64_t)n;
    }
    if (what == 12) {
        const int64_t v[3] = {(int64_t)__atomic_load_n(&noise_line_stats().n7, __ATOMIC_RELAXED), (int64_t)__atomic_load_n(&noise_line_stats().n9, __ATOMIC_RELAXED), (int64_t)__atomic_load_n(&noise_line_stats().n3, __ATOMIC_RELAXED)};
        const size_t n = cap < sizeof v ? cap : sizeof v; memcpy(dst, v, n); return (int64_t)n;
    }
#endif
#ifdef LHIP_PHASE_PROF
    if (what == 9) { const size_t n = cap < sizeof g_call_prof ? cap : sizeof g_call_prof; memcpy(dst, g_call_prof, n); return (int64_t)n; }
#endif
    Context* ctx = nullptr;
    { std::lock_guard<std::mutex> lk(g_ctx_mu); for (auto& kv : g_ctx) if (kv.second->ws.have_last) ctx = kv.second.get(); }
    if (!ctx) { set_err("no batch has run"); return LHIP_ERR_INTERNAL; }
    std::lock_guard<std::mutex> lk(ctx->mu);
    rt::set_device(ctx->device);
    const WorkSet& ws = ctx->ws;
    const Workspace& W = ws.lastW;
    const size_t GC = (size_t)W.ngslots * ws.lastC;
    const void* src = nullptr; size_t n = 0;
    switch (what) {
        case 0: src = W.xr; n = GC * 576 * 4; break;
        case 1: src = W.blocktype; n = GC * 4; break;
        case 2: src = W.E; n = (size_t)W.ngslots * ws.lastCp * E_STRIDE * 4; break;
        case 3: src = W.ath_adjust; n = (size_t)W.nfslots * 8; break;
        case 4: src = W.side; n = (size_t)W.nframes_total * 2 * ws.lastC * sizeof(GrSide); break;
        case 5: src = W.sb; n = GC * SB_STRIDE * 4; break;
        case 6: src = W.peaks; n = GC * PK_STRIDE * 4; break;
        case 7: src = W.prof; n = PROF_BYTES; break;
        case 8: src = W.nflagged; n = 256; break;
        default: set_err("unknown tap"); return LHIP_ERR_INTERNAL;
    }
    if (n > cap) n = cap;
    if (!rt::d2h(dst, src, n, ctx->stream) || !rt::sync(ctx->stream)) return LHIP_ERR_INTERNAL;
    return (int64_t)n;
}

int lhip_stream_info(const lhip_stream* s, lhip_stream_info_t* info) {
    if (!s || s->magic != 0x4c484950) { set_err("bad stream handle"); return LHIP_ERR_BAD_HANDLE; }
    if (!info) { set_err("lhip_stream_info: null argument"); return LHIP_ERR_INTERNAL; }
    if (!s->tag) { set_err("lhip_stream_info: the stream was not created with the infoTag option (its totals are not kept)"); return LHIP_ERR_INTERNAL; }
    const TagTotals& v = *s->tag;
    info->frames = v.frames; info->audio_bytes = v.bytes; info->music_crc = v.crc & 0xffff; info->delay = s->ts->tag.delay;
    info->padding = v.padding < 0 ? -1 : (int32_t)v.padding; info->tag_bytes = s->ts->tag.size;
    return 0;
}
int64_t lhip_info_tag(lhip_stream* s, uint8_t* out, size_t cap) {
    if (!s || s->magic != 0x4c484950) { set_err("bad stream handle"); return LHIP_ERR_BAD_HANDLE; }
    if (!s->tag) { set_err("lhip_info_tag: the stream was not created with the infoTag option"); return LHIP_ERR_INTERNAL; }
    if (s->tag->moved) { set_err("lhip_info_tag: the stream was moved with lhip_seek or lhip_state_set; state blobs do not carry the tag's totals (combining the tags of shards is not supported)"); return LHIP_ERR_INTERNAL; }
    if (!s->tag->flushed) { set_err("lhip_info_tag: the stream has not been flushed (the tag reports the totals and the end padding of the complete stream)"); return LHIP_ERR_INTERNAL; }
    const size_t n = (size_t)s->ts->tag.size;
    if (!out || cap < n) { set_err("output buffer too small"); return LHIP_ERR_BUFFER_TOO_SMALL; }
    uint32_t radio = 0;
    if (s->gain) {
        int32_t tenth = 0; int64_t windows = 0, samples = 0;
        const int rc = lhip_replay_gain(s, &tenth, &windows, &samples);
        if (rc < 0) return rc;
        if (rc == 0) radio = gain_tag_field(tenth);
    }
    tag_write(s->ts->T, s->ts->tag, *s->tag, out, radio);
    return (int64_t)n;
}
size_t lhip_debug_crc_span(void) { return (size_t)CRC_SPAN_BYTES; }
int lhip_debug_crc16(const void* bytes, size_t n, size_t misalign, uint32_t* crc) {
    if ((!bytes && n) || !crc || misalign > 15 || n > (size_t)1 << 40) { set_err("lhip_debug_crc16: bad argument"); return LHIP_ERR_INTERNAL; }
    if (rt::device_count() <= 0) { set_err("no HIP device available (this library has no CPU fallback)"); return LHIP_ERR_INTERNAL; }
    CrcDesc d;
    d.n = (int64_t)n; d.n_dev = nullptr; d.part0 = 0; d.nparts = (int32_t)((n + CRC_SPAN_BYTES - 1) / CRC_SPAN_BYTES);
    uint8_t* buf = (uint8_t*)rt::dmalloc(n + 32);
    uint8_t* aux = (uint8_t*)rt::dmalloc(sizeof(CrcDesc) + 16 + (size_t)d.nparts * 4);
    bool ok = buf && aux;
    if (ok) {
        d.base = buf + ((16 - ((uintptr_t)buf & 15)) & 15) + misalign;
        CrcDesc* dD = (CrcDesc*)aux; uint32_t* dOut = (uint32_t*)(aux + sizeof(CrcDesc)); uint32_t* dPart = dOut + 4;
        ok = rt::h2d((void*)d.base, bytes, n, nullptr) && rt::h2d(dD, &d, sizeof d, nullptr) && rt::sync(nullptr);
#ifndef LHIP_HOSTSIM
        if (ok) {
            if (d.nparts > 0) hipLaunchKernelGGL(g_out_crc, dim3(d.nparts), dim3(64), 0, 0, (const CrcDesc*)dD, 1, dPart);
            hipLaunchKernelGGL(g_out_crc_fold, dim3(1), dim3(64), 0, 0, (const CrcDesc*)dD, (const uint32_t*)dPart, dOut);
            const hipError_t e = hipGetLastError();
            if (e != hipSuccess) { set_err(std::string("g_out_crc: ") + hipGetErrorString(e)); ok = false; }
        }
#else
        if (ok) {
#ifdef LHIP_WAVESIM
            for (int b = 0; b < d.nparts; b++) wsim::run([&](int lane_) { kb_out_crc(dD, crc_find_stream(dD, 1, b), b, lane_, dPart); });
            wsim::run([&](int lane_) { kb_crc_fold(dD, 0, lane_, dPart, dOut); });
#else
            for (int b = 0; b < d.nparts; b++) kb_out_crc(dD, crc_find_stream(dD, 1, b), b, 0, dPart);
            kb_crc_fold(dD, 0, 0, dPart, dOut);
#endif
        }
#endif
        uint32_t r = 0;
        ok = ok && rt::d2h(&r, dOut, 4, nullptr) && rt::sync(nullptr);
        *crc = r & 0xffff;
    } else set_err("hipMalloc failed");
    rt::dfree(buf); rt::dfree(aux);
    return ok ? 0 : LHIP_ERR_INTERNAL;
}
int lhip_debug_ingest(int format, int channels, const void* bytes, size_t nsamples, size_t misalign, float* left, float* right, int64_t* rejected) {
    const int type = fmt_type(format);
    if (!fmt_ok(format) || !fmt_ingest(type) || (channels != 1 && channels != 2) || (!bytes && nsamples) || !left || (channels == 2 && !right) || !rejected || misalign > 15 ||
        nsamples > (size_t)1 << 31 || (fmt_bps(type) >= 4 && misalign % fmt_bps(type))) { set_err("lhip_debug_ingest: bad argument"); return LHIP_ERR_INTERNAL; }
    if (rt::device_count() <= 0) { set_err("no HIP device available (this library has no CPU fallback)"); return LHIP_ERR_INTERNAL; }
    const size_t bps = fmt_bps(type), nb = nsamples * bps * (size_t)channels;
    const bool il = (format & LHIP_PCM_INTERLEAVED) && channels == 2;
    *rejected = 0;
    if (nsamples == 0) return 0;
    uint8_t* buf = (uint8_t*)rt::dmalloc(16 + misalign + nb);
    float* pl = (float*)rt::dmalloc(nsamples * 4);
    float* pr = channels == 2 ? (float*)rt::dmalloc(nsamples * 4) : nullptr;
    uint8_t* aux = (uint8_t*)rt::dmalloc(sizeof(IngestDesc) + 16);
    bool ok = buf && pl && (pr || channels == 1) && aux && ((uintptr_t)buf & 15) == 0;
    uint8_t* const smp = buf ? buf + 16 + misalign : nullptr;
#if defined(LHIP_HOSTSIM) && defined(LHIP_ASAN_POISON)
    if (ok) ASAN_POISON_MEMORY_REGION(buf, 16 + (misalign & ~(size_t)7));
#endif
    if (ok) {
        IngestDesc d; memset(&d, 0, sizeof d);
        d.type = type; d.blk0 = 0; d.inter = il ? 1 : 0; d.narr = (channels == 2 && !il) ? 2 : 1;
        d.src[0] = smp; d.src[1] = d.narr == 2 ? smp + nsamples * bps : nullptr;
        d.dst[0] = pl; d.dst[1] = channels == 2 ? pr : pl;
        d.nelem = (int64_t)nsamples * (il ? 2 : 1); d.tiles = ingest_tiles(type, d.nelem);
        const int grid = (int)(d.tiles * d.narr);
        IngestDesc* dD = (IngestDesc*)aux; unsigned long long* dC = (unsigned long long*)(aux + sizeof(IngestDesc));
        unsigned long long zero = 0, cnt = 0;
        ok = rt::h2d(smp, bytes, nb, nullptr) && rt::h2d(dD, &d, sizeof d, nullptr) && rt::h2d(dC, &zero, 8, nullptr) && rt::sync(nullptr);
#ifndef LHIP_HOSTSIM
        if (ok) {
            hipLaunchKernelGGL(g_ingest, dim3(grid), dim3(64), 0, 0, (const IngestDesc*)dD, 1, PCM_F32_LIMIT, dC);
            const hipError_t e = hipGetLastError();
            if (e != hipSuccess) { set_err(std::string("g_ingest: ") + hipGetErrorString(e)); ok = false; }
        }
#else
        if (ok) {
            alignas(16) static thread_local uint8_t LI[ING_WINDOW];
            for (int b = 0; b < grid; b++) {
#ifdef LHIP_WAVESIM
                wsim::run([&](int lane_) { const unsigned r = kb_ingest(dD, 0, b, lane_, LI, PCM_F32_LIMIT); if (lane_ == 0) *dC += r; });
#else
                *dC += kb_ingest(dD, 0, b, 0, LI, PCM_F32_LIMIT);
#endif
            }
        }
#endif
        ok = ok && rt::d2h(left, pl, nsamples * 4, nullptr) && (channels == 1 || rt::d2h(right, pr, nsamples * 4, nullptr)) && rt::d2h(&cnt, dC, 8, nullptr) && rt::sync(nullptr);
        *rejected = (int64_t)cnt;
    } else set_err("hipMalloc failed");
#if defined(LHIP_HOSTSIM) && defined(LHIP_ASAN_POISON)
    if (buf) ASAN_UNPOISON_MEMORY_REGION(buf, 16 + misalign);
#endif
    rt::dfree(buf); rt::dfree(pl); rt::dfree(pr); rt::dfree(aux);
    return ok ? 0 : LHIP_ERR_INTERNAL;
}
static int gain_fetch(lhip_stream* s, const char* who, std::vector<uint32_t>& A, GainState& gs) {
    if (!s || s->magic != 0x4c484950) { set_err("bad stream handle"); return LHIP_ERR_BAD_HANDLE; }
    if (!s->gain) { set_err(std::string(who) + ": the stream was not created with the replayGain option"); return LHIP_ERR_INTERNAL; }
    if (s->gain->moved) { set_err(std::string(who) + ": the stream was moved with lhip_seek or lhip_state_set (or a chunked call failed half way); state blobs do not carry the analysis' history and histogram"); return LHIP_ERR_INTERNAL; }
    Context* ctx = s->ctx;
    std::lock_guard<std::mutex> lk(ctx->mu);
    A.assign(GAIN_BINS, 0u);
    if (!rt::set_device(ctx->device) || !rt::d2h(&gs, s->gain->state(), sizeof gs, ctx->stream) || !rt::d2h(A.data(), s->gain->bins(), (size_t)GAIN_BINS * 4, ctx->stream) || !rt::sync(ctx->stream)) return LHIP_ERR_INTERNAL;
    return 0;
}
int lhip_replay_gain(lhip_stream* s, int32_t* tenth_db, int64_t* windows, int64_t* samples) {
    if (!tenth_db || !windows || !samples) { set_err("lhip_replay_gain: null argument"); return LHIP_ERR_INTERNAL; }
    std::vector<uint32_t> A; GainState gs;
    const int rc = gain_fetch(s, "lhip_replay_gain", A, gs);
    if (rc < 0) return rc;
    *samples = gs.samples;
    return gain_result(A.data(), tenth_db, windows);
}
int lhip_debug_gain_histogram(lhip_stream* s, uint32_t* A) {
    if (!A) { set_err("lhip_debug_gain_histogram: null argument"); return LHIP_ERR_INTERNAL; }
    std::vector<uint32_t> v; GainState gs;
    const int rc = gain_fetch(s, "lhip_debug_gain_histogram", v, gs);
    if (rc < 0) return rc;
    memcpy(A, v.data(), (size_t)GAIN_BINS * 4);
    return 0;
}
int lhip_debug_gain_windows(int fs, int channels, const float* l, const float* r, size_t n, int32_t* bins, double* energies) {
    const int ri = gain_rate_index(fs);
    if (ri < 0 || (channels != 1 && channels != 2) || !l || (channels == 2 && !r) || n == 0 || n > 0x7fffffff || !bins || !energies) { set_err("lhip_debug_gain_windows: bad argument"); return LHIP_ERR_INTERNAL; }
    if (rt::device_count() <= 0) { set_err("no HIP device available (this library has no CPU fallback)"); return LHIP_ERR_INTERNAL; }
    const size_t nwin = n / (size_t)gain_window(ri);
    std::unique_ptr<GainRec> g(gain_create(fs, channels, nullptr));
    float* src = (float*)rt::dmalloc((size_t)channels * n * 4);
    int32_t* dB = (int32_t*)rt::dmalloc(nwin * 4 + 4); double* dE = (double*)rt::dmalloc(nwin * 8 + 8);
    StreamIO* dIO = (StreamIO*)rt::dmalloc(sizeof(StreamIO)); StreamDesc* dSD = (StreamDesc*)rt::dmalloc(sizeof(StreamDesc)); GainDesc* dGD = (GainDesc*)rt::dmalloc(sizeof(GainDesc));
    GainPlan P; GainRec* rec = g.get(); const int64_t nn = (int64_t)n;
    bool ok = g && src && dB && dE && dIO && dSD && dGD && gain_plan(&rec, &nn, 1, P, dB, dE);
    float* rows = ok ? (float*)rt::dmalloc(P.row_floats * 4) : nullptr;
    ok = ok && rows;
    if (ok) {
        gain_bind_rows(P, rows);
        Tables T; memset(&T, 0, sizeof T);
        T.channels_out = channels; T.channels_in = channels; T.rs_ratio = 1; T.pcm_limit = PCM_F32_LIMIT; T.scale = 1.0;
        Workspace W; memset(&W, 0, sizeof W);
        StreamDesc sd; memset(&sd, 0, sizeof sd);
        StreamIO io; memset(&io, 0, sizeof io);
        io.src[0] = src; io.src[1] = channels == 2 ? src + n : src; io.f32 = 1; io.stride = 1; io.n_new = (int32_t)n; io.n_in = (int32_t)n;
        ok = rt::h2d(src, l, n * 4, nullptr) && (channels == 1 || rt::h2d(src + n, r, n * 4, nullptr)) && rt::h2d(dIO, &io, sizeof io, nullptr) && rt::h2d(dSD, &sd, sizeof sd, nullptr) &&
             rt::h2d(dGD, P.d.data(), sizeof(GainDesc), nullptr) && rt::sync(nullptr);
#ifndef LHIP_HOSTSIM
        if (ok) {
            hipLaunchKernelGGL(g_gain_stage, dim3(P.stage_blocks), dim3(GAIN_STAGE_NT), 0, 0, T, W, (const StreamDesc*)dSD, (const StreamIO*)dIO, (const GainDesc*)dGD, 1);
            if (P.waves > 0) { if (channels == 2) hipLaunchKernelGGL(g_gain<2>, dim3(P.waves), dim3(64), 0, 0, (const GainDesc*)dGD, 1); else hipLaunchKernelGGL(g_gain<1>, dim3(P.waves), dim3(64), 0, 0, (const GainDesc*)dGD, 1); }
            const hipError_t e = hipGetLastError();
            if (e != hipSuccess) { set_err(std::string("g_gain: ") + hipGetErrorString(e)); ok = false; }
        }
#else
        if (ok) gain_sim_run(T, W, dSD, dIO, dGD, 1, P.stage_blocks, P.waves);
#endif
        ok = ok && rt::d2h(bins, dB, nwin * 4, nullptr) && rt::d2h(energies, dE, nwin * 8, nullptr) && rt::sync(nullptr);
    } else if (g) set_err("hipMalloc failed");
    rt::dfree(src); rt::dfree(dB); rt::dfree(dE); rt::dfree(dIO); rt::dfree(dSD); rt::dfree(dGD); rt::dfree(rows);
    return ok ? (int)nwin : LHIP_ERR_INTERNAL;
}
static const char* probe_check_record(const ProbeIn& I, const int32_t* pretab) {
    if (I.block_type < 0 || I.block_type > 3) return "block_type outside 0..3";
    if (I.global_gain < 0 || I.global_gain > 255) return "global_gain outside 0..255";
    if ((I.scalefac_scale | 1) != 1 || (I.preflag | 1) != 1) return "scalefac_scale / preflag outside 0..1";
    const bool sh = I.block_type == SHORT_TYPE;
    if (sh && I.preflag) return "preflag on a short block (pretab has long bands only)";
    for (int w = 0; w < 3; w++) if (I.subblock_gain[w] < 0 || I.subblock_gain[w] > 7 || (!sh && I.subblock_gain[w])) return "subblock_gain outside 0..7 (0 unless the block is short)";
    if (!(I.ath_adjust > 0.0) || !(I.ath_adjust < 1e30)) return "ath_adjust not positive and finite";
    for (int i = 0; i < 576; i++) if (!(std::fabs((double)I.xr[i]) < 1e30)) return "xr not finite";
    for (int i = 0; i < E_STRIDE; i++) if (!(I.ratio[i] >= 0.f) || !(I.ratio[i] < 3e38f)) return "ratio negative or not finite";
    const int psymax = sh ? 3 * SBPSY_s : SBPSY_l;
    for (int sfb = 0; sfb < SFBMAX; sfb++) if (I.scalefac[sfb] < 0 || I.scalefac[sfb] > 255) return "scalefac outside 0..255";
    for (int sfb = 0; sfb < psymax; sfb++) {
        for (int flip = 0; flip < 2; flip++) {
            const int sf = I.scalefac[sfb] ^ flip;
            const int st = I.global_gain - ((sf + (I.preflag ? pretab[sfb] : 0)) << (I.scalefac_scale + 1)) - (sh ? I.subblock_gain[sfb % 3] : 0) * 8;
            if (st < -Q_MAX2 || st > Q_MAX) return "a band's step outside the pow20 table";
        }
    }
    if (I.flags & ~1) return "unknown flag";
    if (I.flags & 1) for (int i = 0; i < 576; i++) if (I.ix_in[i] < 0 || I.ix_in[i] > IXMAX_VAL) return "ix_in outside 0..IXMAX_VAL";
    return nullptr;
}
int lhip_debug_quant_probe(lhip_stream* s, const void* in, size_t n, void* out, int max_workgroups) {
    if (!s || s->magic != 0x4c484950) { set_err("bad stream handle"); return LHIP_ERR_BAD_HANDLE; }
    if (!in || !out || n == 0 || n > (size_t)1 << 20 || max_workgroups < 0) { set_err("lhip_debug_quant_probe: bad argument"); return LHIP_ERR_INTERNAL; }
    if (s->ts->fast) { set_err("lhip_debug_quant_probe: a quality 7 stream (its table set never calls calc_noise)"); return LHIP_ERR_INTERNAL; }
    const lhtb_entry* pt = find_entry(s->ts->blob.data(), "pretab");
    if (!pt || pt->dtype != 1 || pt->count < (uint32_t)SBMAX_l) { set_err("lhip_debug_quant_probe: tables blob without pretab"); return LHIP_ERR_INTERNAL; }
    const int32_t* pretab = (const int32_t*)(s->ts->blob.data() + pt->offset);
    const ProbeIn* rec = (const ProbeIn*)in;
    for (size_t i = 0; i < n; i++) {
        ProbeIn I; memcpy(&I, rec + i, sizeof I);
        if (const char* why = probe_check_record(I, pretab)) { set_err("lhip_debug_quant_probe: record " + std::to_string(i) + ": " + why); return LHIP_ERR_INTERNAL; }
    }
    Context* ctx = s->ctx;
    std::lock_guard<std::mutex> lk(ctx->mu);
    if (!rt::set_device(ctx->device)) return LHIP_ERR_INTERNAL;
    void* st = ctx->stream;
    ProbeIn* dIn = (ProbeIn*)rt::dmalloc(n * sizeof(ProbeIn));
    ProbeOut* dOut = (ProbeOut*)rt::dmalloc(n * sizeof(ProbeOut));
    bool ok = dIn && dOut;
    if (ok) {
        ok = rt::h2d(dIn, in, n * sizeof(ProbeIn), st) && rt::dzero(dOut, n * sizeof(ProbeOut), st);
        const int nn = (int)n;
#ifndef LHIP_HOSTSIM
        if (ok) {
            const int grid = max_workgroups > 0 ? (nn < max_workgroups ? nn : max_workgroups) : (nn < 1024 ? nn : 1024);
            ProbeArgs a; a.T = s->ts->T; a.pb = s->ts->pb10; a.in = dIn; a.out = dOut; a.n = nn; a.grid = grid;
            const std::string e = probe_launch(rt::phys(ctx->device), a, st);
            if (!e.empty()) { set_err("g_quant_probe: " + e); ok = false; }
        }
#else
        if (ok) {
            ok = rt::sync(st);
            const int cap = max_workgroups > 0 && max_workgroups < PROBE_SIM_WAVES ? max_workgroups : PROBE_SIM_WAVES;
            if (ok) quant_probe_sim_run(s->ts->T, s->ts->pb10, dIn, dOut, nn, nn < cap ? nn : cap);
        }
#endif
        ok = ok && rt::d2h(out, dOut, n * sizeof(ProbeOut), st) && rt::sync(st);
    } else set_err("hipMalloc failed");
    rt::dfree(dIn); rt::dfree(dOut);
    return ok ? 0 : LHIP_ERR_INTERNAL;
}
int lhip_debug_info_toc(const int64_t* frames, size_t ncalls, int kbps, uint8_t* toc) {
    if ((!frames && ncalls) || !toc || kbps <= 0) { set_err("lhip_debug_info_toc: bad argument"); return LHIP_ERR_INTERNAL; }
    std::unique_ptr<TagTotals> v(new TagTotals());
    for (size_t i = 0; i < ncalls; i++) { if (frames[i] < 0) { set_err("lhip_debug_info_toc: bad argument"); return LHIP_ERR_INTERNAL; } tag_toc_add(*v, frames[i], kbps); }
    tag_toc(*v, toc);
    return v->pos;
}

int lhip_kernel_timing(int enable) {
#ifndef LHIP_HOSTSIM
    std::lock_guard<std::mutex> lk(g_kt_mu);
    g_kt_on = enable != 0;
    for (int i = 0; i < KT_N; i++) { g_kt_ms[i] = 0; g_kt_calls[i] = 0; }
    return KT_N;
#else
    (void)enable; return 0;
#endif
}

int lhip_kernel_times(int idx, const char** name, double* total_ms, int64_t* launches) {
#ifndef LHIP_HOSTSIM
    if (idx < 0 || idx >= KT_N) return -1;
    std::lock_guard<std::mutex> lk(g_kt_mu);
    if (name) *name = g_kt_names[idx];
    if (total_ms) *total_ms = g_kt_ms[idx];
    if (launches) *launches = g_kt_calls[idx];
    return 0;
#else
    (void)idx; (void)name; (void)total_ms; (void)launches; return -1;
#endif
}

// ... 42 lines not shown
```

### lamejs_amd/csrc/lhip_batch.h

```cpp
#pragma once
struct Job {
    lhip_stream* s; const void* l; const void* r; size_t n; uint8_t* out; size_t cap; int64_t written;
    int F; int64_t bytes;
    int64_t n_out;
    bool flush = false;
    double rs_len = -1;
    double rs_used = 0;
    int f32 = 0, inter = 0;
    bool count_rejected = false;
    int type = 0;
    void set_format(int format) { type = format & ~LHIP_PCM_INTERLEAVED; f32 = type == LHIP_PCM_F32; inter = (format & LHIP_PCM_INTERLEAVED) != 0; }
};
static_assert(LHIP_PCM_U8 == ING_U8 && LHIP_PCM_S24 == ING_S24 && LHIP_PCM_S32 == ING_S32 && LHIP_PCM_F32N == ING_F32N && LHIP_PCM_F64N == ING_F64N && LHIP_PCM_F64 == ING_F64, "k_ingest.h states the header's sample types");
static inline size_t fmt_bps(int type) { return type == LHIP_PCM_S16 ? 2 : type == LHIP_PCM_F32 ? 4 : (size_t)ingest_bps(type); }
static inline bool fmt_ok(int format) {
    const int t = format & ~LHIP_PCM_INTERLEAVED;
    return format >= 0 && (t == LHIP_PCM_S16 || t == LHIP_PCM_F32 || t == LHIP_PCM_U8 || t == LHIP_PCM_S24 || t == LHIP_PCM_S32 || t == LHIP_PCM_F32N || t == LHIP_PCM_F64N || t == LHIP_PCM_F64);
}
static inline int fmt_type(int format) { return format & ~LHIP_PCM_INTERLEAVED; }
static inline bool fmt_ingest(int type) { return type >= LHIP_PCM_U8; }

static int64_t rs_outputs(int64_t n_in_total, int r) { return n_in_total > 16 ? (n_in_total - 16 + r - 1) / r : 0; }

struct FracPass { int k; double num_used; int j_last; };
static FracPass frac_pass(const Tables& T, double itime, double len) {
    const int frame = 576 * T.mode_gr;
    int k, j = 0;
    for (k = 0; k < frame; k++) {
        j = (int)floor(k * T.resample_ratio - itime);
        if ((31 + j - 15.5) >= len) break;
    }
    const double reach = 31 + j - 15.5;
    return FracPass{k, len < reach ? len : reach, j};
}
static int64_t frac_call_limit(const Tables& T) { return (int64_t)floor((576 * T.mode_gr - 1) * T.resample_ratio - 15.5) + 15; }
static std::string frac_refusal(const Tables& T, size_t n) {
    return "fractionalResample: the reference does not consume a call of " + std::to_string(n) + " samples whole at this point of the stream (its resampler would turn to fractional "
           "positions and NaN samples); nothing was consumed -- calls of at most " + std::to_string(frac_call_limit(T)) + " samples are always accepted for this configuration";
}
static int host_next_padding(const Tables& T, int* slot_lag) {
    if (T.frac_SpF == 0) return 0;
    int64_t m = (int64_t)*slot_lag % T.out_samplerate; if (m < 0) m += T.out_samplerate;
    const int pad = (m - T.frac_SpF) < 0 ? 1 : 0;
    m = (m - T.frac_SpF) % T.out_samplerate; if (m < 0) m += T.out_samplerate;
    *slot_lag = (int)m;
    return pad;
}

static int64_t batch_bytes(const TableSet& ts, int slot_lag, int F) {
    int64_t npad = 0;
    const Tables& T = ts.T;
    if (T.frac_SpF != 0 && F > 0) {
        const int64_t sr = T.out_samplerate;
        int64_t m0 = slot_lag % sr; if (m0 < 0) m0 += sr;
        const int64_t need = (int64_t)F * T.frac_SpF - m0;
        npad = need > 0 ? (need + sr - 1) / sr : 0;
    }
    return (int64_t)F * ts.base_frame_bytes + npad;
}
static int call_frames(const lhip_stream* s, size_t nsamples) {
    const Tables& T = s->ts->T;
    const int frame = 576 * T.mode_gr, mf_needed = 1024 + frame - 272;
    int64_t n_out;
    if (T.rs_frac) {
        if (nsamples == 0) return 0;
        const FracPass fp = frac_pass(T, s->rs_itime, (double)nsamples);
        if (fp.k >= frame || s->rs_flushed) return -1;
        n_out = fp.k;
    } else n_out = T.rs_ratio == 1 ? (int64_t)nsamples : rs_outputs(s->rs_n_in + (int64_t)nsamples, T.rs_ratio) - rs_outputs(s->rs_n_in, T.rs_ratio);
    const int64_t total = (int64_t)s->mf_size + n_out;
    return total >= mf_needed ? (int)((total - mf_needed) / frame) + 1 : 0;
}

static std::atomic<int> g_spec_start{180}, g_spec_step{4};
#ifdef LHIP_PHASE_PROF
static double g_call_prof[8];
#define CALL_STAMP(i) do { const auto n_ = std::chrono::steady_clock::now(); g_call_prof[i] += std::chrono::duration<double>(n_ - cp_t_).count(); cp_t_ = n_; } while (0)
#else
#define CALL_STAMP(i) do {} while (0)
#endif
enum { FX_STATS_OFF = 32 * 4 };
enum { SMALL_CALL_BYTES = 1 << 20 };
struct CallLayout {
    size_t desc_sd, desc_io, desc_fm, desc_gm, desc_bytes;
    size_t sm_out, sm_nfl, sm_ob, sm_sf, sm_rv, sm_desc, sm_in, sm_end, copy_in, copy_out;
    void set(int S, int nfs, int ngs, size_t FR, int64_t out_total, size_t in_bytes) {
        auto a16 = [](size_t v) { return (v + 15) & ~(size_t)15; };
        desc_sd = 0; desc_io = a16(desc_sd + (size_t)S * sizeof(StreamDesc)); desc_fm = a16(desc_io + (size_t)S * sizeof(StreamIO));
        desc_gm = a16(desc_fm + (size_t)nfs * 4); desc_bytes = desc_gm + (size_t)ngs * 4;
        sm_out = 0; sm_nfl = a16((size_t)out_total + 64); sm_ob = sm_nfl + 256; sm_sf = a16(sm_ob + (size_t)S * 4 + 64); sm_rv = sm_sf + a16(FR * 4);
        sm_desc = sm_rv + a16(FR * 4); sm_in = a16(sm_desc + desc_bytes); sm_end = sm_in + in_bytes + 64;
        copy_in = sm_end - 64 - sm_nfl;
        copy_out = sm_sf;
    }
    size_t pin(size_t o) const { return o - sm_nfl; }
};
struct BatchPlan {
    TableSet* ts = nullptr;
    bool dev_io = false, resv = false, count_rej = false, use_frame = false, small = false;
    bool count_f32 = false;
    int ingest = 0, ingest_tiles = 0; size_t ingest_floats = 0; const IngestDesc* dING = nullptr;
    int S = 0, nfs = 0, ngs = 0, nfr = 0, maxF = 0;
    uint32_t paths = 0;
    QuantLaunch ql;
    int64_t pcm_plane = 0, in_total = 0, out_total = 0, repaired = 0, iters = 0;
    size_t in_bytes = 0, FR = 1;
    std::vector<StreamDesc> sd; std::vector<StreamIO> io;
    std::vector<int64_t> out_rel;
    CallLayout L; Workspace W;
    const StreamDesc* dSD = nullptr; const StreamIO* dIO = nullptr;
    int crc_mode = 0, crc_parts = 0;
    uint32_t* crc_dst = nullptr;
    std::vector<uint32_t> crc;
    GainPlan gain; const GainDesc* dGD = nullptr;
};

static bool plan_batch(Context* ctx, std::vector<Job>& jobs, bool dev_io, BatchPlan& P) {
    TableSet& ts = *jobs[0].s->ts;
    const Tables& T = ts.T;
    const int Cin = T.channels_in;
    const int GR = T.mode_gr, frame = 576 * GR, mf_needed = 1024 + frame - 272;
    const int S = (int)jobs.size();
    const bool resv = !T.disable_reservoir;
    P.ts = &ts; P.dev_io = dev_io; P.S = S; P.resv = resv;
    P.sd.resize(S); P.io.resize(S);
    for (int i = 0; i < S; i++) {
        Job& j = jobs[i];
        lhip_stream* s = j.s;
        if (s->ts.get() != &ts) { set_err("batch: all streams must share one configuration"); return false; }
        if (T.rs_frac) {
            FracPass fp = frac_pass(T, s->rs_itime, j.rs_len >= 0 ? j.rs_len : (double)j.n);
            if (j.n == 0 && j.rs_len < 0) fp = FracPass{0, 0.0, 0};
            if ((fp.k >= frame && j.rs_len < 0) || (s->rs_flushed && j.n > 0)) { j.written = LHIP_ERR_INTERNAL; set_err(s->rs_flushed ? std::string("fractionalResample: the stream has been flushed") : frac_refusal(T, j.n)); return false; }
            j.n_out = fp.k; j.rs_used = fp.num_used;
        } else
        j.n_out = T.rs_ratio == 1 ? (int64_t)j.n : rs_outputs(s->rs_n_in + (int64_t)j.n, T.rs_ratio) - rs_outputs(s->rs_n_in, T.rs_ratio);
        const int64_t total = (int64_t)s->mf_size + j.n_out;
        if (total > 0x7fffffff || (int64_t)j.n > 0x7fffffff) { set_err("too many samples in one call"); return false; }
        j.F = total >= mf_needed ? (int)((total - mf_needed) / frame) + 1 : 0;
        j.bytes = batch_bytes(ts, s->slot_lag, j.F);
        if (resv)
            j.bytes = (int64_t)j.F * (ts.base_frame_bytes + 1) + (j.F > 0 || j.flush ? 512 + RESV_HQ * RESV_HDR : 0) + (j.flush ? 1440 + RESV_HQ * RESV_HDR : 0);
        if ((size_t)j.bytes > j.cap) { j.written = LHIP_ERR_BUFFER_TOO_SMALL; set_err("output buffer too small"); return false; }
        StreamDesc& d = P.sd[i];
        memset(&d, 0, sizeof d);
        d.nframes = j.F; d.fslot0 = P.nfs; d.gslot0 = P.ngs; d.out_slot0 = P.nfr;
        d.pcm_off = P.pcm_plane; d.out_off = P.out_total; d.seg_len = (int)total; d.first_call = s->frame_num == 0;
        d.slot_lag = s->slot_lag; d.frame_num0 = s->frame_num; d.flush = (resv && j.flush) ? 1 : 0;
        P.nfs += j.F + 1; P.ngs += GR * j.F + 1; P.nfr += j.F;
        if (j.F > P.maxF) P.maxF = j.F;
        P.pcm_plane += (total + 63) & ~(int64_t)63;
        P.in_total += (int64_t)j.n; P.out_total += (j.bytes + 15) & ~(int64_t)15;
        if (fmt_ingest(j.type)) {
            const size_t b = fmt_bps(j.type);
            P.in_bytes += (j.n * (size_t)Cin * (b > 4 ? b : 4) + 15) & ~(size_t)15;
            if (j.n > 0) { P.ingest++; P.ingest_floats += (size_t)Cin * ((j.n + 3) & ~(size_t)3); }
        } else
        P.in_bytes += (j.n * (size_t)Cin * fmt_bps(j.type) + 3) & ~(size_t)3;
        P.count_f32 |= j.count_rejected && j.f32 && j.n > 0;
        P.count_rej |= j.count_rejected && (j.f32 || (fmt_ingest(j.type) && ingest_is_float(j.type))) && j.n > 0;
    }
    static const bool no_frame = []() { const char* e = getenv("LAMEJS_HIP_NO_FRAME_KERNEL"); return e && e[0] == '1'; }();
    P.use_frame = P.maxF <= 1 && !no_frame && S <= ctx->num_cus;
    return true;
}
static bool bind_workspace(Context* ctx, BatchPlan& P) {
    WorkSet& ws = ctx->ws; const Tables& T = P.ts->T; Workspace& W = P.W; CallLayout& L = P.L;
    const int C = T.channels_out, S = P.S, nfs = P.nfs, ngs = P.ngs, nfr = P.nfr;
    memset(&W, 0, sizeof W);
    W.spec_start = g_spec_start; W.spec_step = g_spec_step; W.mode_gr = T.mode_gr;
    W.nstreams = S; W.nframes_total = nfr; W.nfslots = nfs; W.ngslots = ngs; W.pcm_plane = P.pcm_plane;
    const int Cp = T.psy_channels;
    const size_t GC = (size_t)ngs * C, GP = (size_t)ngs * Cp, FR = P.FR = (size_t)(nfr > 0 ? nfr : 1);
#define BIND(name, type, bytes) do { if (!ws.name.ensure(bytes)) return false; W.name = (type*)ws.name.p; } while (0)
    BIND(pcm, float, T.rs_ratio != 1 ? (size_t)P.pcm_plane * C * 4 + 64 : 64);
    BIND(peaks, float, GP * PK_STRIDE * 4); BIND(loud, float, GC * 4); BIND(eb_l, float, GP * EBL_STRIDE * 4); BIND(mask_idx, int32_t, GP * EBL_STRIDE * 4);
    BIND(eb_s, float, GP * EBS_STRIDE * 4); BIND(ecb_s, float, GP * EBS_STRIDE * 4); BIND(att_raw, int32_t, GP * 4); BIND(uselong, int32_t, GC * 4); BIND(ul_tmp, int32_t, GP * 4); BIND(last_attack, int32_t, GP * 4);
    BIND(tent, int32_t, GC * 4); BIND(prev_short, int32_t, GC * 4); BIND(blocktype, int32_t, GC * 4); BIND(ath_adjust, double, (size_t)nfs * 8);
    BIND(ath_limit, double, (size_t)nfs * 8); BIND(E, float, GP * E_STRIDE * 4); BIND(sb, float, GC * SB_STRIDE * 4); BIND(xr, float, GC * 576 * 4);
    BIND(att_clean, int32_t, GP * 4); BIND(nb1, float, GP * EBL_STRIDE * 4); BIND(nb2, float, GP * EBL_STRIDE * 4); BIND(fr, FrameResv, FR * sizeof(FrameResv)); BIND(out_bytes, int32_t, (size_t)S * 4 + 64);
    BIND(fht, float, Cp == 4 ? (size_t)ngs * 2 * FHT_STRIDE * 4 : 64); BIND(hpf, float, Cp == 4 ? (size_t)ngs * 2 * 576 * 4 : 64); BIND(tot_ener, float, (size_t)ngs * 4 * 4);
    BIND(side, GrSide, FR * 2 * C * sizeof(GrSide)); BIND(l3, int16_t, FR * 2 * C * 576 * 2); BIND(seed, int32_t, (size_t)nfs * C * 2 * 4);
    BIND(vdig, uint32_t, FR * 2 * C * VD_WORDS * 4);
    BIND(seed_flag, int32_t, FR * 4); BIND(reval, int32_t, FR * 4); BIND(nflagged, int32_t, 256); BIND(slow_list, int32_t, (size_t)nfs * 4); BIND(frame_bytes, int32_t, FR * 4);
    BIND(prof, unsigned long long, PROF_BYTES);
#undef BIND
    W.vdig_n = (int64_t)FR * 2 * C; W.work_ctr = W.nflagged + 16; W.out = nullptr;
    L.set(S, nfs, ngs, FR, P.out_total, P.in_bytes);
    static const bool no_small = []() { const char* e = getenv("LAMEJS_HIP_NO_SMALL_CALLS"); return e && e[0] == '1'; }();
    P.small = !P.dev_io && !no_small && L.sm_end <= SMALL_CALL_BYTES;
    if (P.small && !(ws.pin_in.ensure(L.pin(L.sm_end)) && ws.pin_out.ensure(L.copy_out))) P.small = false;
    if (P.small) {
        if (!ws.small.ensure(L.sm_end)) return false;
        uint8_t* const smb = (uint8_t*)ws.small.p;
        W.nflagged = (int32_t*)(smb + L.sm_nfl); W.work_ctr = W.nflagged + 16; W.out_bytes = (int32_t*)(smb + L.sm_ob);
        W.seed_flag = (int32_t*)(smb + L.sm_sf); W.reval = (int32_t*)(smb + L.sm_rv);
    } else if (!P.dev_io && !(ws.in16.ensure(P.in_bytes + 64) && ws.out8.ensure((size_t)P.out_total + 64))) return false;
    if (P.small) P.paths |= LHIP_PATH_SMALL_CALL;
    if (P.ts->tag.on) { P.crc_mode = P.small ? 1 : 2; P.crc.assign((size_t)S, 0u); }
    return true;
}
static bool stage_crc(Context* ctx, const std::vector<Job>& jobs, BatchPlan& P, uint32_t* crc_log) {
    WorkSet& ws = ctx->ws; const int S = P.S;
    std::vector<CrcDesc> cd((size_t)S);
    int64_t parts = 0;
    for (int i = 0; i < S; i++) {
        CrcDesc& d = cd[i];
        d.base = P.io[i].out; d.n = jobs[i].bytes; d.n_dev = P.resv ? P.W.out_bytes + i : nullptr;
        d.part0 = (int32_t)parts; d.nparts = (int32_t)((jobs[i].bytes + CRC_SPAN_BYTES - 1) / CRC_SPAN_BYTES);
        parts += d.nparts;
    }
    if (parts > 0x7fffffff) { set_err("too many output bytes in one call for the Info tag's CRC"); return false; }
    P.crc_parts = (int)parts;
    if (!ws.crc_desc.ensure((size_t)S * sizeof(CrcDesc)) || !ws.crc_part.ensure((size_t)parts * 4 + 64) || !ws.crc_out.ensure((size_t)S * 4 + 64)) return false;
    if (!rt::h2d(ws.crc_desc.p, cd.data(), (size_t)S * sizeof(CrcDesc), ctx->stream)) return false;
    P.crc_dst = crc_log ? crc_log : (uint32_t*)ws.crc_out.p;
    return true;
}
static bool stage_gain(Context* ctx, const std::vector<Job>& jobs, BatchPlan& P) {
    WorkSet& ws = ctx->ws; const int S = P.S;
    std::vector<GainRec*> recs((size_t)S); std::vector<int64_t> n((size_t)S);
    for (int i = 0; i < S; i++) { recs[i] = jobs[i].s->gain.get(); n[i] = jobs[i].n_out; }
    if (!gain_plan(recs.data(), n.data(), S, P.gain)) return false;
    if (P.gain.stage_blocks == 0) return true;
    if (!ws.gain_rows.ensure(P.gain.row_floats * 4 + 64) || !ws.gain_desc.ensure((size_t)S * sizeof(GainDesc))) return false;
    gain_bind_rows(P.gain, (float*)ws.gain_rows.p);
    if (!rt::h2d(ws.gain_desc.p, P.gain.d.data(), (size_t)S * sizeof(GainDesc), ctx->stream)) return false;
    P.dGD = (const GainDesc*)ws.gain_desc.p;
    return true;
}
static bool stage_inputs(Context* ctx, std::vector<Job>& jobs, BatchPlan& P) {
    WorkSet& ws = ctx->ws; void* st = ctx->stream; const Tables& T = P.ts->T; Workspace& W = P.W; const CallLayout& L = P.L;
    std::vector<StreamDesc>& sd = P.sd; std::vector<StreamIO>& io = P.io; std::vector<int64_t>& out_rel = P.out_rel;
    const int S = P.S, Cin = T.channels_in, GR = T.mode_gr, nfs = P.nfs, ngs = P.ngs; const size_t FR = P.FR; const bool small = P.small, dev_io = P.dev_io, resv = P.resv;
    uint8_t* const smb = (uint8_t*)ws.small.p;
    std::vector<int32_t> fmap(nfs), gmap(ngs);
    out_rel.resize(S);
    size_t in_off = 0;
    uint8_t* const pin = small ? (uint8_t*)ws.pin_in.p : nullptr;
    if (small) memset(pin, 0, L.pin(L.sm_desc));
    for (int i = 0; i < S; i++) {
        Job& j = jobs[i];
        for (int k = 0; k <= j.F; k++) fmap[sd[i].fslot0 + k] = i;
        for (int k = 0; k <= GR * j.F; k++) gmap[sd[i].gslot0 + k] = i;
        StreamIO& o = io[i];
        o.state = j.s->d_state; o.n_new = (int)j.n_out; o.mf_size = j.s->mf_size; o.n_in = (int)j.n;
        o.rs_p0 = T.rs_ratio <= 1 ? 0 : (int)(rs_outputs(j.s->rs_n_in, T.rs_ratio) * T.rs_ratio - 16 - j.s->rs_n_in);
        o.rs_itime = j.s->rs_itime;
        out_rel[i] = sd[i].out_off;
        const size_t bps = fmt_bps(j.type);
        const bool il = j.inter && Cin == 2;
        const bool ing = fmt_ingest(j.type);
        o.f32 = j.f32 ? 1 : 0; o.stride = il ? 2 : 1;
        if (ing && small) {
            uint8_t* base = smb + L.sm_in; uint8_t* hbase = pin + L.pin(L.sm_in);
            float* h0 = (float*)(hbase + in_off); float* h1 = Cin == 2 ? h0 + j.n : nullptr;
            const bool one = Cin == 2 && !il && (!j.r || j.r == j.l);
            (void)ingest_host(j.type, j.l, j.r, j.n, one ? 1 : Cin, il, h0, h1, T.pcm_limit);
            o.f32 = 1; o.stride = 1;
            o.src[0] = base + in_off; o.src[1] = (Cin == 2 && !one) ? base + in_off + j.n * 4 : o.src[0];
            in_off = (in_off + j.n * 4 * (size_t)Cin + 15) & ~(size_t)15;
            o.out = smb + L.sm_out + sd[i].out_off;
            continue;
        }
        if (dev_io) {
            o.src[0] = j.l; o.src[1] = il ? (const void*)((const uint8_t*)j.l + bps) : ((Cin == 2 && j.r) ? j.r : j.l); o.out = j.out;
        } else {
            uint8_t* base = small ? smb + L.sm_in : (uint8_t*)ws.in16.p;
            uint8_t* hbase = small ? pin + L.pin(L.sm_in) : nullptr;
            const size_t plane = j.n * bps * (il ? 2 : 1);
            o.src[0] = base + in_off;
            if (small) memcpy(hbase + in_off, j.l, plane);
            else if (!rt::h2d((void*)o.src[0], j.l, plane, st)) return false;
            if (il) o.src[1] = base + in_off + bps;
            in_off += plane;
            if (Cin == 2 && !il) {
                o.src[1] = base + in_off;
                if (small) memcpy(hbase + in_off, j.r ? j.r : j.l, plane);
                else if (!rt::h2d((void*)o.src[1], j.r ? j.r : j.l, plane, st)) return false;
                in_off += plane;
            } else if (!il) o.src[1] = o.src[0];
            in_off = ing ? (in_off + 15) & ~(size_t)15 : (in_off + 3) & ~(size_t)3;
            o.out = (small ? smb + L.sm_out : (uint8_t*)ws.out8.p) + sd[i].out_off;
        }
    }
    if (P.ingest && !small) {
        if (!ws.ingest.ensure(P.ingest_floats * 4 + 64) || !ws.ingest_desc.ensure((size_t)S * sizeof(IngestDesc))) return false;
        std::vector<IngestDesc> id((size_t)S);
        float* plane = (float*)ws.ingest.p;
        int64_t blk = 0;
        for (int i = 0; i < S; i++) {
            const Job& j = jobs[i]; StreamIO& o = io[i]; IngestDesc& d = id[i];
            memset(&d, 0, sizeof d);
            d.blk0 = (int32_t)blk; d.type = j.type;
            if (!fmt_ingest(j.type) || j.n == 0) continue;
            const bool il = j.inter && Cin == 2;
            const bool two = Cin == 2 && !il && o.src[1] != o.src[0];
            const size_t pl = (j.n + 3) & ~(size_t)3;
            d.src[0] = (const uint8_t*)o.src[0]; d.src[1] = two ? (const uint8_t*)o.src[1] : nullptr;
            d.dst[0] = plane; d.dst[1] = (il || two) ? plane + pl : plane;
            d.inter = il ? 1 : 0; d.narr = two ? 2 : 1; d.nelem = (int64_t)j.n * (il ? 2 : 1); d.tiles = ingest_tiles(j.type, d.nelem);
            blk += d.tiles * d.narr;
            o.f32 = 1; o.stride = 1; o.src[0] = d.dst[0]; o.src[1] = d.dst[1];
            plane += pl * (size_t)Cin;
        }
        if (blk > 0x7fffffff) { set_err("too many samples in one call"); return false; }
        P.ingest_tiles = (int)blk;
        if (!rt::h2d(ws.ingest_desc.p, id.data(), (size_t)S * sizeof(IngestDesc), st)) return false;
        P.dING = (const IngestDesc*)ws.ingest_desc.p;
    }
    if (!small && !ws.desc.ensure(L.desc_bytes)) return false;
    uint8_t* const ddesc = small ? smb + L.sm_desc : (uint8_t*)ws.desc.p;
    {
        std::vector<uint8_t> stage_v;
        uint8_t* stage = nullptr;
        if (small) stage = pin + L.pin(L.sm_desc);
        else { stage_v.assign(L.desc_bytes, 0); stage = stage_v.data(); }
        if (small) memset(stage, 0, L.sm_in - L.sm_desc);
        for (int i = 0; i < S; i++) sd[i].out_off = (int64_t)(uintptr_t)io[i].out;
        memcpy(stage + L.desc_sd, sd.data(), (size_t)S * sizeof(StreamDesc));
        memcpy(stage + L.desc_io, io.data(), (size_t)S * sizeof(StreamIO));
        memcpy(stage + L.desc_fm, fmap.data(), (size_t)nfs * 4);
        memcpy(stage + L.desc_gm, gmap.data(), (size_t)ngs * 4);
        if (small) { if (!rt::h2d(smb + L.sm_nfl, pin, L.copy_in, st)) return false; }
        else if (!rt::h2d(ddesc, stage, L.desc_bytes, st)) return false;
    }
    W.fslot_stream = (const int32_t*)(ddesc + L.desc_fm); W.gslot_stream = (const int32_t*)(ddesc + L.desc_gm);
    if (!small) {
        if (!rt::dzero(ws.seed_flag.p, FR * 4, st)) return false;
        if (!rt::dzero(ws.reval.p, FR * 4, st)) return false;
        if (resv && !rt::dzero(ws.out_bytes.p, (size_t)S * 4, st)) return false;
        if (!rt::dzero(ws.nflagged.p, 256, st)) return false;
    }
#if defined(LHIP_PHASE_PROF) || defined(LHIP_WAVE_TIMES)
    if (!rt::dzero(ws.prof.p, PROF_BYTES, st)) return false;
#endif
    P.dSD = (const StreamDesc*)(ddesc + L.desc_sd);
    P.dIO = (const StreamIO*)(ddesc + L.desc_io);
    W.io = P.dIO;
    return true;
}
static bool fetch_outputs(Context* ctx, std::vector<Job>& jobs, BatchPlan& P, bool want_sync, int32_t* fx_dst, bool fetch_fx, int32_t (&fx)[3], bool fetch_crc) {
    WorkSet& ws = ctx->ws; void* st = ctx->stream; const Workspace& W = P.W; const CallLayout& L = P.L;
    const int S = P.S, nfr = P.nfr; const bool small = P.small, dev_io = P.dev_io, resv = P.resv;
    const uint8_t* const smb = (const uint8_t*)ws.small.p;
    if (fx_dst) {
        if (nfr > 0) { if (!rt::d2d(fx_dst, (const uint8_t*)W.nflagged + FX_STATS_OFF, 12, st)) return false; }
        else if (!rt::dzero(fx_dst, 12, st)) return false;
    }
    if (small) {
        const uint8_t* po = (const uint8_t*)ws.pin_out.p;
        if (!rt::d2h(ws.pin_out.p, smb, L.copy_out, st) || !rt::sync(st)) return false;
        memcpy(fx, po + L.sm_nfl + FX_STATS_OFF, sizeof fx);
        if (resv) for (int i = 0; i < S; i++) jobs[i].bytes = ((const int32_t*)(po + L.sm_ob))[i];
        for (int i = 0; i < S; i++) if (jobs[i].bytes > 0) memcpy(jobs[i].out, po + L.sm_out + P.out_rel[i], (size_t)jobs[i].bytes);
        if (P.crc_mode == 1) for (int i = 0; i < S; i++) P.crc[i] = crc16r_host(po + L.sm_out + P.out_rel[i], (size_t)jobs[i].bytes);
    } else {
        if (fetch_fx && !rt::d2h(fx, (const int32_t*)ws.nflagged.p + FX_STATS_OFF / 4, sizeof fx, st)) return false;
        std::vector<int32_t> ob;
        if (resv) {
            ob.assign((size_t)S, 0);
            if (!rt::d2h(ob.data(), ws.out_bytes.p, (size_t)S * 4, st) || !rt::sync(st)) return false;
            for (int i = 0; i < S; i++) jobs[i].bytes = ob[i];
        }
        if (fetch_crc && !rt::d2h(P.crc.data(), P.crc_dst, (size_t)S * 4, st)) return false;
        if (!dev_io) {
            for (int i = 0; i < S; i++)
                if (jobs[i].bytes > 0 && !rt::d2h(jobs[i].out, P.io[i].out, (size_t)jobs[i].bytes, st)) return false;
            if (!rt::sync(st)) return false;
        } else if (want_sync || fetch_crc) {
            if (!rt::sync(st)) return false;
        }
    }
    return true;
}
static void advance_streams(std::vector<Job>& jobs, const Tables& T) {
    const int frame = 576 * T.mode_gr;
    for (int i = 0; i < (int)jobs.size(); i++) {
        Job& j = jobs[i];
        lhip_stream* s = j.s;
        const int64_t total = (int64_t)s->mf_size + j.n_out;
        if (j.n > 0) {
            if (s->mf_samples_to_encode < 1) s->mf_samples_to_encode = 576 + 1152;
            s->mf_samples_to_encode += (int)j.n_out;
        }
        s->rs_n_in += (int64_t)j.n;
        if (T.rs_frac) {
            const double len = j.rs_len >= 0 ? j.rs_len : (double)j.n;
            s->rs_itime += j.rs_used - j.n_out * T.resample_ratio;
            if (s->rs_inbuf_len == 0 || s->rs_inbuf_nsamples < len) { s->rs_inbuf_len = (int64_t)floor(len); s->rs_inbuf_nsamples = len; }
        }
        s->mf_samples_to_encode -= frame * j.F;
        s->mf_size = (int)(total - (int64_t)frame * j.F);
        if (T.frac_SpF != 0 && j.F > 0) {
            int64_t m = ((int64_t)s->slot_lag - (int64_t)j.F * T.frac_SpF) % T.out_samplerate;
            if (m < 0) m += T.out_samplerate;
            s->slot_lag = (int)m;
        }
        s->frame_num += j.F;
        j.written = j.bytes;
    }
}

#ifdef LHIP_HOSTSIM
#include "lhip_pipeline_sim.h"
#else
#include "lhip_pipeline_hip.h"
#endif

static bool run_batch(Context* ctx, std::vector<Job>& jobs, bool dev_io, bool want_sync, int32_t* fx_dst = nullptr, uint32_t* crc_log = nullptr) {
    if (jobs.empty()) return true;
#ifdef LHIP_PHASE_PROF
    auto cp_t_ = std::chrono::steady_clock::now();
    g_call_prof[7] += 1;
#endif
    std::lock_guard<std::mutex> lk(ctx->mu);
    if (!rt::set_device(ctx->device)) return false;
    BatchPlan P;
    if (!plan_batch(ctx, jobs, dev_io, P) || !bind_workspace(ctx, P)) return false;
    CALL_STAMP(0);
    if (!stage_inputs(ctx, jobs, P)) return false;
    if (P.crc_mode == 2 && !stage_crc(ctx, jobs, P, crc_log)) return false;
    if (P.ts->gain_on && !stage_gain(ctx, jobs, P)) return false;
    CALL_STAMP(1);

    g_rejected = 0; g_rej_pending = nullptr;
    if (!run_pipeline(ctx, P)) return false;
    if (P.gain.stage_blocks > 0) { for (int i = 0; i < P.S; i++) if (P.gain.d[i].n > 0) { GainRec& g = *jobs[i].s->gain; g.samples += P.gain.d[i].n; g.cur ^= 1; } }
    CALL_STAMP(2);
    int32_t fx[3] = {0, 0, 0};
    const bool fetch_fx = P.nfr > 0 && (!dev_io || want_sync || g_kt_on_());
    if (!fetch_outputs(ctx, jobs, P, want_sync, fx_dst, fetch_fx, fx, P.crc_mode == 2 && !crc_log) || !collect_kernel_times(ctx->stream)) return false;
    CALL_STAMP(3);
    advance_streams(jobs, P.ts->T);
    if (P.crc_mode && !crc_log) for (int i = 0; i < P.S; i++) tag_account(*jobs[i].s->tag, jobs[i].F, jobs[i].bytes, P.crc[i], P.ts->T.brate);
    if (!collect_repair_stats(ctx, P, fetch_fx, fx)) return false;
    g_stat_frames = P.nfr; g_stat_repaired = P.repaired; g_stat_iters = P.iters; g_last_paths = P.paths; g_last_quant = P.ql;
    WorkSet& ws = ctx->ws;
    ws.lastW = P.W; ws.lastC = P.ts->T.channels_out; ws.lastCp = P.ts->T.psy_channels; ws.have_last = true;
    return true;
}
```

### lamejs_amd/csrc/lhip_context.h

```cpp
#pragma once
struct DevBuf {
    void* p = nullptr; size_t cap = 0;
    bool ensure(size_t n) {
        if (n <= cap) return true;
        rt::dfree(p);
        cap = n + n / 4 + 4096;
        p = rt::dmalloc(cap);
        if (!p) { cap = 0; set_err("hipMalloc(workspace) failed"); return false; }
        return true;
    }
    ~DevBuf() { rt::dfree(p); }
};

struct PinBuf {
    void* p = nullptr; size_t cap = 0;
    bool ensure(size_t n) {
        if (n <= cap) return true;
        rt::host_free_pinned(p);
        cap = n + n / 4 + 4096;
        p = rt::host_alloc_pinned(cap);
        if (!p) { cap = 0; return false; }
        return true;
    }
    void release() { rt::host_free_pinned(p); p = nullptr; cap = 0; }
};

struct WorkSet {
    DevBuf pcm, peaks, loud, eb_l, mask_idx, eb_s, ecb_s, att_raw, uselong, ul_tmp, last_attack, tent, prev_short, blocktype,
        ath_adjust, ath_limit, E, sb, xr, side, l3, seed, seed_flag, nflagged, slow_list, frame_bytes, desc, in16, rejected, out8, prof, fht, hpf, tot_ener, reval, att_clean, nb1, nb2, fr, out_bytes, vdig, small;
    DevBuf crc_desc, crc_part, crc_out;
    DevBuf ingest, ingest_desc;
    DevBuf gain_rows, gain_desc;
    PinBuf pin_in, pin_out;
    Workspace lastW; int lastC = 0, lastCp = 0; bool have_last = false;
    void* aux_stream = nullptr; void* ev_fork = nullptr; void* ev_join = nullptr;
};

struct Context {
    int device = 0;
    void* stream = nullptr;
    std::mutex mu;
    void* ev_coop[2] = {nullptr, nullptr};
    bool own_stream = false;
    int live_streams = 0;
    std::map<std::string, std::shared_ptr<TableSet>> tables;
    WorkSet ws;
    int num_cus = 256;
    int qfast_wg_per_cu[4] = {0, 0, 0, 0};
    int fixup_wg_per_cu = 0;
    void* copy_stream = nullptr; void* ev_in[2] = {nullptr, nullptr}; void* ev_done[2] = {nullptr, nullptr};
    DevBuf chunk_crc;
    DevBuf chunk_in, chunk_out, chunk_fx, state_bak;
    std::mutex chunk_mu;
};

static std::mutex g_ctx_mu;
static std::map<int, std::unique_ptr<Context>> g_ctx;

static Context* get_context(int device) {
    std::lock_guard<std::mutex> lk(g_ctx_mu);
    auto it = g_ctx.find(device);
    if (it != g_ctx.end()) return it->second.get();
    std::unique_ptr<Context> c(new Context());
    c->device = device;
#ifndef LHIP_HOSTSIM
    { int n = 0; if (hipDeviceGetAttribute(&n, hipDeviceAttributeMultiprocessorCount, rt::phys(device)) == hipSuccess && n > 0) c->num_cus = n; }
    if (rt::alias_n() && device > 0 && hipSetDevice(0) == hipSuccess) { void* st = nullptr; if (rt::stream_create(&st)) { c->stream = st; c->own_stream = true; } }
#endif
    Context* r = c.get();
    g_ctx[device] = std::move(c);
    return r;
}

struct lhip_stream {
    uint32_t magic = 0x4c484950;
    Context* ctx = nullptr;
    std::shared_ptr<TableSet> ts;
    StreamState* d_state = nullptr;
    int mf_size = MF_INIT;
    int mf_samples_to_encode = 576 + 1152;
    int slot_lag = 0;
    int64_t frame_num = 0;
    int64_t rs_n_in = 0;
    double rs_itime = 0;
    double rs_inbuf_nsamples = 0;
    int64_t rs_inbuf_len = 0;
    bool rs_flushed = false;
    std::unique_ptr<TagTotals> tag;
    std::unique_ptr<GainRec> gain;
    ~lhip_stream() { rt::dfree(d_state); magic = 0; }
};
```

### lamejs_amd/csrc/lhip_kernels.h

```cpp
#pragma once
#define XCD_GRID(n) (8 * (((n) + 7) / 8))
static __device__ __forceinline__ int xcd_item(int b, int n) { const int it = (b & 7) * ((n + 7) >> 3) + (b >> 3); return it < n && (b >> 3) < ((n + 7) >> 3) ? it : -1; }
__global__ __launch_bounds__(64) void g_load(Tables T, Workspace W, const StreamDesc* SD, const StreamIO* IO) { kb_load(T, W, SD, IO, blockIdx.x, threadIdx.x); }
__global__ __launch_bounds__(64) void g_save(Tables T, Workspace W, const StreamDesc* SD, const StreamIO* IO) { kb_save(T, W, SD, IO, blockIdx.x, threadIdx.x); }
#ifndef LHIP_WPB
#define LHIP_WPB 4
#endif
enum { WPB = LHIP_WPB };
#define XCD_GRID_W(n) XCD_GRID(((n) + WPB - 1) / WPB)
static __device__ __forceinline__ int xcd_wave_item(int n, int* lane) {
    const int wv = __builtin_amdgcn_readfirstlane((int)(threadIdx.x >> 6));
    *lane = (int)(threadIdx.x & 63);
    const int g = xcd_item(blockIdx.x, (n + WPB - 1) / WPB);
    const int it = g * WPB + wv;
    return (g >= 0 && it < n) ? it : -1;
}
#define WAVE_LDS(TYPE, NAME) __shared__ TYPE NAME##_[WPB]; TYPE& NAME = NAME##_[__builtin_amdgcn_readfirstlane((int)(threadIdx.x >> 6))]
__global__ __launch_bounds__(64 * WPB) void g_psyA(Tables T, Workspace W, const StreamDesc* SD, const StreamIO* IO, int chn0, int nch) {
    WAVE_LDS(PsyALds, L);
    int lane;
    const int it = xcd_wave_item(W.ngslots * nch, &lane);
    if (it >= 0) kb_psyA(T, W, SD, IO, it / nch, chn0 + it % nch, lane, L);
}
__global__ __launch_bounds__(256) void g_prep(Tables T, Workspace W, const StreamDesc* SD, const StreamIO* IO, int nstreams) {
    kb_prep(T, W, SD, IO, nstreams, (int64_t)blockIdx.x * blockDim.x + threadIdx.x, (int64_t)gridDim.x * blockDim.x);
}
__global__ __launch_bounds__(256) void g_count_rejected(const StreamIO* IO, int nstreams, int C, float limit, unsigned long long* ctr) {
    const unsigned long long bad = kb_count_rejected(IO, nstreams, C, limit, (int64_t)blockIdx.x * blockDim.x + threadIdx.x, (int64_t)gridDim.x * blockDim.x);
    if (bad) atomicAdd(ctr, bad);
}
__global__ __launch_bounds__(64) void g_scan_raw(Tables T, Workspace W, const StreamDesc* SD, int ngs) { const int g = blockIdx.x * 64 + threadIdx.x; if (g < ngs) kb_scan_raw(T, W, SD, g); }
__global__ __launch_bounds__(64) void g_scan_attack(Tables T, Workspace W, const StreamDesc* SD, int ngs) { const int g = blockIdx.x * 64 + threadIdx.x; if (g < ngs) kb_scan_attack(T, W, SD, g); }
__global__ __launch_bounds__(64) void g_scan_blocktype(Tables T, Workspace W, const StreamDesc* SD, int ngs) { const int g = blockIdx.x * 64 + threadIdx.x; if (g < ngs) kb_scan_blocktype(T, W, SD, g); }
__global__ __launch_bounds__(ATH_NT) void g_scan_ath(Tables T, Workspace W, const StreamDesc* SD) { __shared__ AthLds L; kb_scan_ath(T, W, SD, blockIdx.x, threadIdx.x, L); }
template <int NCH> __global__ __launch_bounds__(64 * WPB) void g_psyB(Tables T, PowBase pb, Workspace W, const StreamDesc* SD, int par) {
    WAVE_LDS(PsyBLdsT<NCH>, L);
    int lane;
    const int it = xcd_wave_item(W.ngslots, &lane);
    if (it >= 0) kb_psyB<NCH>(T, pb, W, SD, it, lane, L, par);
}
__global__ __launch_bounds__(64, 4) void g_poly(Tables T, Workspace W, const StreamDesc* SD, const StreamIO* IO, int nitems) {
    __shared__ PolyLds L;
    const int it = xcd_item(blockIdx.x, (nitems + POLY_PER_WAVE - 1) / POLY_PER_WAVE);
    if (it >= 0) kb_polyphase(T, W, SD, IO, it, nitems, threadIdx.x, L);
}
__global__ __launch_bounds__(64) void g_mdct(Tables T, Workspace W, const StreamDesc* SD) {
    __shared__ MdctLds L;
    const int it = xcd_item(blockIdx.x, W.ngslots);
    if (it >= 0) kb_mdct(T, W, SD, it, threadIdx.x, L);
}
#ifdef LHIP_PHASE_PROF
enum { QWAVES = 7 };
#else
enum { QWAVES = 8 };
#endif
#ifndef LHIP_QOCC
#define LHIP_QOCC 4
#endif
LHIP_DEV int next_frame_slot(int32_t* ctr) {
    int v = 0;
    if ((threadIdx.x & 63) == 0) v = atomicAdd(ctr, 1);
    return __builtin_amdgcn_readfirstlane(v);
}
struct QArgs { Tables T; PowBase pb; Workspace W; const StreamDesc* SD; int chain, nfs, ctr; };
#ifdef LHIP_QVGPR
#define LHIP_QUANT_BOUNDS __attribute__((amdgpu_flat_work_group_size(1, 64 * QWAVES), amdgpu_waves_per_eu(LHIP_QOCC, 8), amdgpu_num_vgpr((LHIP_QVGPR) / 2)))
#else
#define LHIP_QUANT_BOUNDS __launch_bounds__(64 * QWAVES, LHIP_QOCC)
#endif
template <int RESV, int SKIP> __global__ LHIP_QUANT_BOUNDS void g_quant(QArgs a_unused) {
    __shared__ QuantTabs Q;
    __shared__ QuantLds L[QWAVES];
    __shared__ TailShare TS;
#ifndef LHIP_PHASE_PROF
    static_assert(QWAVES * sizeof(QuantLds) + sizeof(QuantTabs) + sizeof(TailShare) <= 80 * 1024, "g_quant: LDS budget for 2 workgroups per CU exceeded");
#endif
    const QArgs* A = (const QArgs*)__builtin_amdgcn_kernarg_segment_ptr();
    q_copy_tabs(A->T, Q, threadIdx.x, 64 * QWAVES);
    if (threadIdx.x == 0) TS.drawing = QWAVES;
    if (threadIdx.x < QWAVES) TS.offer[threadIdx.x].state = 0;
    const bool tail_help_on = !RESV && A->T.channels_out == 2;
    __syncthreads();
    const int wv = __builtin_amdgcn_readfirstlane(threadIdx.x >> 6);
#ifdef LHIP_PHASE_PROF
    L[wv].prof[threadIdx.x & 63] = 0;
#endif
#if defined(LHIP_PHASE_PROF) || defined(LHIP_WAVE_TIMES)
    const unsigned long long wave_t0_ = wall_clock64();
#endif
    int hint[3] = {-1, -1, -1};
    for (;;) {
        const int fslot = next_frame_slot(A->W.work_ctr + A->ctr);
        if (fslot >= A->nfs) break;
        if constexpr (!RESV) kb_quant_th<SKIP>(A->T, A->pb, A->W, A->SD, fslot, threadIdx.x & 63, L[wv], Q, hint, TS, wv);
        else kb_quant<0, RESV, SKIP>(A->T, A->pb, A->W, A->SD, fslot, A->chain, threadIdx.x & 63, L[wv], Q, -1, nullptr, nullptr, nullptr);
        hint[0] = __builtin_amdgcn_readfirstlane(hint[0]); hint[1] = __builtin_amdgcn_readfirstlane(hint[1]); hint[2] = __builtin_amdgcn_readfirstlane(hint[2]);
    }
    if (tail_help_on) tail_help<SKIP>(A->T, A->pb, A->W, A->SD, threadIdx.x & 63, L, wv, QWAVES, Q, TS);
#ifdef LHIP_PHASE_PROF
    atomicAdd((unsigned long long*)A->W.prof + (threadIdx.x & 63), (unsigned long long)L[wv].prof[threadIdx.x & 63]);
#endif
#if defined(LHIP_PHASE_PROF) || defined(LHIP_WAVE_TIMES)
    {
        const int wid = blockIdx.x * QWAVES + wv;
        if ((threadIdx.x & 63) == 0 && wid < 8192) { A->W.prof[64 + 2 * wid] = wave_t0_; A->W.prof[64 + 2 * wid + 1] = wall_clock64(); }
    }
#endif
}
template <int RESV, int SKIP> __global__ __launch_bounds__(128, LHIP_QOCC) void g_quant_pair(QArgs a_unused) {
    __shared__ QuantTabs Q;
    __shared__ QuantLds L[2];
    __shared__ int mbox[4];
    const QArgs* A = (const QArgs*)__builtin_amdgcn_kernarg_segment_ptr();
    q_copy_tabs(A->T, Q, threadIdx.x, 128);
    __syncthreads();
    const int wv = __builtin_amdgcn_readfirstlane(threadIdx.x >> 6);
    kb_quant<1, RESV, SKIP>(A->T, A->pb, A->W, A->SD, blockIdx.x, A->chain, threadIdx.x & 63, L[wv], Q, wv, mbox);
}
enum { QF_WAVES = 8 };
template <int PAIR, int SKIP> __global__ __launch_bounds__(64 * QF_WAVES, LHIP_QOCC) void g_quant_fast(QArgs a_unused) {
    __shared__ QuantTabs Q;
    __shared__ QuantLds L[QF_WAVES];
    __shared__ FastPair FP[QF_WAVES / 2];
#ifndef LHIP_PHASE_PROF
    static_assert(QF_WAVES * sizeof(QuantLds) + sizeof(QuantTabs) + sizeof(FP) <= 80 * 1024, "g_quant_fast: LDS budget for 2 workgroups per CU exceeded");
#endif
    static_assert(sizeof(FP) / sizeof(int) <= 64 * QF_WAVES, "the pair records are zeroed by one store per thread");
    const QArgs* A = (const QArgs*)__builtin_amdgcn_kernarg_segment_ptr();
    q_copy_tabs(A->T, Q, threadIdx.x, 64 * QF_WAVES);
    if (threadIdx.x < sizeof(FP) / sizeof(int)) ((int*)FP)[threadIdx.x] = 0;
    __syncthreads();
    const int wv = __builtin_amdgcn_readfirstlane(threadIdx.x >> 6), lane = threadIdx.x & 63;
    int hint[3] = {-1, -1, -1};
    for (int round = 1;; round++) {
        int fslot;
        if constexpr (PAIR != 0) {
            FastPair& fp = FP[wv >> 1];
            if ((wv & 1) == 0) { fslot = next_frame_slot(A->W.work_ctr + A->ctr); fast_pair_publish_slot(fp, round, fslot, lane); }
            else fslot = fast_pair_await_slot(fp, round, lane);
            if (fslot >= A->nfs) break;
            kb_quant_fast<1, SKIP>(A->T, A->pb, A->W, A->SD, fslot, lane, L[wv], Q, hint, wv & 1, &fp, round);
        } else {
            fslot = next_frame_slot(A->W.work_ctr + A->ctr);
            if (fslot >= A->nfs) break;
            kb_quant_fast<0, SKIP>(A->T, A->pb, A->W, A->SD, fslot, lane, L[wv], Q, hint);
        }
        hint[0] = __builtin_amdgcn_readfirstlane(hint[0]); hint[1] = __builtin_amdgcn_readfirstlane(hint[1]); hint[2] = __builtin_amdgcn_readfirstlane(hint[2]);
    }
}
__global__ __launch_bounds__(256) void g_validate_fast(Tables T, Workspace W, const StreamDesc* SD, int nfs) {
    __shared__ ValidateShare S;
    const int t = blockIdx.x * 256 + threadIdx.x, fslot = t >> 2;
    kb_validate_fast_quad(T, W, SD, fslot < nfs ? fslot : 0, t & 3, fslot < nfs, S);
}
enum { FX_NFLAG = 0, FX_NSLOW = 1, FX_WORK_REPAIR = 2, FX_WORK_SLOW = 3, FX_PARITY_STRIDE = 8, FX_BAR = 24, FX_STATS = 32 };
LHIP_DEV void grid_barrier(int32_t* bar, int nblocks) {
    __syncthreads();
    if (nblocks > 1 && threadIdx.x == 0) {
        __builtin_amdgcn_fence(__ATOMIC_RELEASE, "agent");
        asm volatile("s_waitcnt vmcnt(0)" ::: "memory");
        const int gen = __hip_atomic_load(bar + 1, __ATOMIC_RELAXED, __HIP_MEMORY_SCOPE_AGENT);
        if (__hip_atomic_fetch_add(bar, 1, __ATOMIC_RELAXED, __HIP_MEMORY_SCOPE_AGENT) == nblocks - 1) {
            __hip_atomic_store(bar, 0, __ATOMIC_RELAXED, __HIP_MEMORY_SCOPE_AGENT);
            __builtin_amdgcn_fence(__ATOMIC_RELEASE, "agent");
            asm volatile("s_waitcnt vmcnt(0)" ::: "memory");
            __hip_atomic_fetch_add(bar + 1, 1, __ATOMIC_RELAXED, __HIP_MEMORY_SCOPE_AGENT);
        } else {
            for (int n = 0; __hip_atomic_load(bar + 1, __ATOMIC_RELAXED, __HIP_MEMORY_SCOPE_AGENT) == gen; n++) { if (n > (1 << 26)) __builtin_trap(); __builtin_amdgcn_s_sleep(4); }
        }
        __builtin_amdgcn_fence(__ATOMIC_ACQUIRE, "agent");
    }
    __syncthreads();
}
#ifndef LHIP_FIXUP_OCC
#define LHIP_FIXUP_OCC 4
#endif
template <int SKIP> __global__ __launch_bounds__(64 * QWAVES, LHIP_FIXUP_OCC) void g_fixup(QArgs a_unused) {
    __shared__ QuantTabs Q;
    __shared__ QuantLds L[QWAVES];
    const QArgs* A = (const QArgs*)__builtin_amdgcn_kernarg_segment_ptr();
    const int nfs = A->nfs, nblocks = gridDim.x, nthr = 64 * QWAVES;
    const int wv = __builtin_amdgcn_readfirstlane(threadIdx.x >> 6), lane = threadIdx.x & 63;
    int32_t* base = A->W.nflagged;
    bool tabs = false;
    int repaired = 0, iters = 0, failed = 0;
    for (int it = 0;; it++) {
        int32_t* ctr = base + FX_PARITY_STRIDE * (it & 1);
        Workspace W = A->W;
        W.nflagged = ctr;
        if (blockIdx.x == 0 && threadIdx.x < FX_PARITY_STRIDE) base[FX_PARITY_STRIDE * ((it + 1) & 1) + threadIdx.x] = 0;
        if (it > 0) {
            for (int f = blockIdx.x * nthr + threadIdx.x; f < nfs; f += nblocks * nthr) kb_validate_fast(A->T, W, A->SD, f, it);
            grid_barrier(base + FX_BAR, nblocks);
        }
        const int nslow = __builtin_amdgcn_readfirstlane(__hip_atomic_load(ctr + FX_NSLOW, __ATOMIC_RELAXED, __HIP_MEMORY_SCOPE_AGENT));
        const int gw = blockIdx.x * QWAVES + wv, nw = nblocks * QWAVES;
        if (nslow > 0) {
            if (!tabs) { q_copy_tabs(A->T, Q, threadIdx.x, nthr); __syncthreads(); tabs = true; }
            for (int i = gw; i < nslow; i += nw)
                kb_validate<SKIP>(A->T, A->pb, W, A->SD, __builtin_amdgcn_readfirstlane(W.slow_list[i]), lane, L[wv], Q);
            grid_barrier(base + FX_BAR, nblocks);
        }
        const int nflag = __builtin_amdgcn_readfirstlane(__hip_atomic_load(ctr + FX_NFLAG, __ATOMIC_RELAXED, __HIP_MEMORY_SCOPE_AGENT));
        if (nflag == 0) break;
        repaired += nflag; iters++;
        if (iters > nfs + 2) { failed = 1; break; }
        if (!tabs) { q_copy_tabs(A->T, Q, threadIdx.x, nthr); __syncthreads(); tabs = true; }
        for (int b0 = gw; b0 < nfs; b0 += 64 * nw) {
            int flagged = 0;
            const int f = b0 + nw * lane;
            if (f < nfs) {
                const StreamDesc* sd = A->SD + W.fslot_stream[f];
                const int k = f - sd->fslot0 - 1;
                if (k >= 0) flagged = W.seed_flag[sd->out_slot0 + k] == 1;
            }
            uint64_t m = __ballot(flagged);
            while (m) {
                const int l = (int)__builtin_ctzll(m);
                m &= m - 1;
                const int fr = b0 + nw * l;
                kb_quant<0, 0, SKIP>(A->T, A->pb, W, A->SD, fr, 1, lane, L[wv], Q);
                if (lane == 0) {
                    const StreamDesc* sd = A->SD + W.fslot_stream[fr];
                    const int k = fr - sd->fslot0 - 1;
                    if (k + 1 < sd->nframes) W.reval[sd->out_slot0 + k + 1] = it + 1;
                }
            }
        }
        grid_barrier(base + FX_BAR, nblocks);
    }
    if (blockIdx.x == 0 && threadIdx.x == 0) { base[FX_STATS + 0] = repaired; base[FX_STATS + 1] = iters; base[FX_STATS + 2] = failed; }
}
__global__ __launch_bounds__(64) void g_bits(Tables T, Workspace W, const StreamDesc* SD) {
    __shared__ BitsLds L;
    kb_bits(T, W, SD, blockIdx.x, threadIdx.x, L);
}
__global__ __launch_bounds__(64) void g_resv_flush(Tables T, Workspace W, const StreamDesc* SD) {
    __shared__ BitsLds L;
    if (SD[blockIdx.x].flush) kb_resv_flush(T, W, blockIdx.x, threadIdx.x, L, W.io[blockIdx.x].state->rv, W.out_bytes + blockIdx.x);
}
__global__ __launch_bounds__(64) void g_out_crc(const CrcDesc* D, int nstreams, uint32_t* partial) {
    const int s = crc_find_stream(D, nstreams, (int)blockIdx.x);
    kb_out_crc(D, s, (int)blockIdx.x - D[s].part0, threadIdx.x, partial);
}
__global__ __launch_bounds__(64) void g_ingest(const IngestDesc* D, int nstreams, float limit, unsigned long long* ctr) {
    __shared__ __attribute__((aligned(16))) uint8_t L[ING_WINDOW];
    const int s = ingest_find_stream(D, nstreams, (int)blockIdx.x);
    const unsigned bad = kb_ingest(D, s, (int64_t)blockIdx.x - D[s].blk0, threadIdx.x, L, limit);
    if (ctr && bad && threadIdx.x == 0) atomicAdd(ctr, (unsigned long long)bad);
}
__global__ __launch_bounds__(GAIN_STAGE_NT) void g_gain_stage(Tables T, Workspace W, const StreamDesc* SD, const StreamIO* IO, const GainDesc* D, int nstreams) {
    const int s = gain_find_stream<true>(D, nstreams, (int)blockIdx.x);
    kb_gain_stage(T, W, SD, IO, D, s, (int64_t)((int)blockIdx.x - D[s].blk0) * GAIN_STAGE_NT + threadIdx.x);
}
template <int CH> __global__ __launch_bounds__(64) void g_gain(const GainDesc* D, int nstreams) {
    __shared__ float L[64 * CH * GAIN_STRIDE];
    const int s = gain_find_stream<false>(D, nstreams, (int)blockIdx.x);
    kb_gain<CH>(D, s, (int)blockIdx.x - D[s].wave0, threadIdx.x, L);
}
__global__ __launch_bounds__(64) void g_out_crc_fold(const CrcDesc* D, const uint32_t* partial, uint32_t* out) { kb_crc_fold(D, blockIdx.x, threadIdx.x, partial, out); }
#ifndef LHIP_FRAME_PIPE
#define LHIP_FRAME_PIPE 1
#endif
static constexpr bool g_frame_pipe = LHIP_FRAME_PIPE != 0;
__global__ __launch_bounds__(64 * RS_WAVES, 2) void g_resv_stream(QArgs a_unused) {
    __shared__ QuantTabs Q;
    __shared__ __attribute__((aligned(16))) unsigned char U[RS_WAVES][RS_LDS_PER_WAVE];
    __shared__ ResvState RV;
    __shared__ int mbox[4];
    __shared__ int32_t nout;
    __shared__ CountShare CS[2];
    const QArgs* A = (const QArgs*)__builtin_amdgcn_kernarg_segment_ptr();
    const int wv = __builtin_amdgcn_readfirstlane(threadIdx.x >> 6), lane = threadIdx.x & 63, st = blockIdx.x;
    q_copy_tabs(A->T, Q, threadIdx.x, 64 * RS_WAVES);
    static_assert(sizeof(ResvState) % 4 == 0, "the reservoir record is copied as words");
    ResvState* grv = &A->W.io[st].state->rv;
    for (int i = threadIdx.x; i < (int)(sizeof(ResvState) / 4); i += 64 * RS_WAVES) ((uint32_t*)&RV)[i] = ((const uint32_t*)grv)[i];
    if (threadIdx.x == 0) nout = 0;
    __syncthreads();
    const int F = __builtin_amdgcn_readfirstlane(A->SD[st].nframes);
    for (int k = 0; k <= F; k++)
        for (int stage = 0; stage < RS_STAGES; stage++) {
            kb_resv_stage<1>(stage, A->T, A->pb, A->W, A->SD, st, k, F, wv, lane, U[wv], Q, mbox, RV, &nout, (g_frame_pipe && A->ctr) ? CS : nullptr);
            __syncthreads();
        }
    if (wv == 3 && A->SD[st].flush) kb_resv_flush(A->T, A->W, st, lane, *(BitsLds*)U[3], RV, &nout);
    __syncthreads();
    for (int i = threadIdx.x; i < (int)(sizeof(ResvState) / 4); i += 64 * RS_WAVES) ((uint32_t*)grv)[i] = ((const uint32_t*)&RV)[i];
    if (threadIdx.x == 0) A->W.out_bytes[st] = nout;
}
template <int RESV> __global__ __launch_bounds__(64 * FR_WAVES) void g_frame(QArgs a_unused, const StreamIO* IO) {
    __shared__ QuantTabs Q;
    __shared__ __attribute__((aligned(16))) unsigned char U[FR_WAVES][FR_LDS_PER_WAVE];
    __shared__ int mbox[12];
    __shared__ CountShare CS[2];
    const QArgs* A = (const QArgs*)__builtin_amdgcn_kernarg_segment_ptr();
    const int wv = __builtin_amdgcn_readfirstlane(threadIdx.x >> 6), lane = threadIdx.x & 63;
    if (threadIdx.x < 2) CS[threadIdx.x].state = CS_IDLE;
#if defined(LHIP_PHASE_PROF) || defined(LHIP_HANDOFF_PROF)
    if (threadIdx.x < 8) CS[0].acc[threadIdx.x] = 0;
#endif
#ifdef LHIP_PHASE_PROF
    if (blockIdx.x == 0 && threadIdx.x == 0) { A->W.prof[FRAME_PROF_BASE + FR_STAGES + 1] = wall_clock64(); A->W.prof[FRAME_PROF_BASE + FR_STAGES + 3] = __builtin_amdgcn_s_memtime(); }
#endif
    q_copy_tabs(A->T, Q, threadIdx.x, 64 * FR_WAVES);
#pragma clang loop unroll(full)
    for (int stage = 0; stage < FR_STAGES; stage++) {
#ifdef LHIP_PHASE_PROF
        if (blockIdx.x == 0 && threadIdx.x == 0) A->W.prof[FRAME_PROF_BASE + stage] = __builtin_amdgcn_s_memtime();
        if (stage == FS_QUANT) ((QuantLds*)U[wv])->prof[lane] = 0;
#endif
        if (frame_stage_empty<RESV>(stage, A->T)) continue;
        kb_frame_stage<RESV, 1>(stage, A->T, A->pb, A->W, A->SD, IO, blockIdx.x, wv, FR_WAVES, lane, U[wv], Q, mbox, g_frame_pipe ? CS : nullptr);
#ifdef LHIP_PHASE_PROF
        if ((stage == FS_PSYA_POLY || stage == FS_BITS_SAVE) && blockIdx.x == 0 && lane == 0)
            A->W.prof[FRAME_PROF_BASE + (stage == FS_PSYA_POLY ? 40 : 48) + wv] = __builtin_amdgcn_s_memtime() - A->W.prof[FRAME_PROF_BASE + stage];
        if (stage == FS_QUANT && blockIdx.x == 0 && wv == 0 && (lane < 22 || (lane > 28 && lane != 54))) A->W.prof[lane] = ((QuantLds*)U[wv])->prof[lane];
        if (stage == FS_QUANT && blockIdx.x == 0 && wv == 2 && lane < 5) {
            A->W.prof[FRAME_PROF_BASE + 16 + lane] = ((QuantLds*)U[wv])->prof[PH_C_LOAD + lane]; A->W.prof[FRAME_PROF_BASE + 24 + lane] = ((QuantLds*)U[wv])->prof[32 + PH_C_LOAD + lane];
        }
        if (stage == FS_QUANT && blockIdx.x == 0 && wv == 0 && lane < 8) A->W.prof[FRAME_PROF_BASE + 32 + lane] = CS[0].acc[lane];
#endif
        __syncthreads();
    }
#ifdef LHIP_PHASE_PROF
    if (blockIdx.x == 0 && threadIdx.x == 0) { A->W.prof[FRAME_PROF_BASE + FR_STAGES] = __builtin_amdgcn_s_memtime(); A->W.prof[FRAME_PROF_BASE + FR_STAGES + 2] = wall_clock64(); }
#elif defined(LHIP_HANDOFF_PROF)
    if (blockIdx.x == 0 && threadIdx.x < 8) atomicAdd(A->W.prof + 32 + threadIdx.x, (unsigned long long)CS[0].acc[threadIdx.x]);
#endif
}
enum { KT_LOAD, KT_PREP, KT_PSYA, KT_SCAN, KT_PSYB, KT_POLY, KT_MDCT, KT_QUANT, KT_VALIDATE, KT_REPAIR, KT_BITS, KT_SAVE, KT_COUNT, KT_OUT_CRC, KT_INGEST, KT_GAIN_STAGE, KT_GAIN, KT_N };
static const char* const g_kt_names[KT_N] = {"load", "prep", "psyA", "scan", "psyB", "polyphase", "mdct", "quant", "validate", "repair", "bits", "save", "count_rejected", "out_crc", "ingest", "gain_stage", "gain"};
static std::atomic<bool> g_kt_on{false};
static std::mutex g_kt_mu;
static double g_kt_ms[KT_N];
static int64_t g_kt_calls[KT_N];
struct KtPending { int id; hipEvent_t a, b; };
static thread_local std::vector<KtPending> g_kt_pending;
static void kt_begin(int id, void* st) {
    if (!g_kt_on) return;
    KtPending p; p.id = id;
    hipEventCreate(&p.a); hipEventCreate(&p.b);
// ... 48 lines not shown
```

### lamejs_amd/csrc/lhip_pipeline_hip.h

```cpp
#pragma once
static inline bool g_kt_on_() { return g_kt_on; }
static_assert(FX_STATS_OFF == FX_STATS * 4, "counter block layout");
static bool collect_kernel_times(void* st) { if (g_kt_on) { if (!rt::sync(st)) return false; kt_collect(); } return true; }
static bool collect_repair_stats(Context* ctx, BatchPlan& P, bool fetch_fx, const int32_t* fx) {
    g_stat_pending = nullptr;
    if (fetch_fx) {
        P.repaired = fx[0]; P.iters = fx[1];
        if (fx[2]) { set_err("seed-chain repair did not converge"); return false; }
    } else if (P.nfr > 0) g_stat_pending = ctx;
    return true;
}
static int quant_grid_cap(int grid) {
    static const int cap = []() { const char* e = getenv("LAMEJS_HIP_QUANT_GRID_MAX"); return e ? atoi(e) : 0; }();
    return cap >= 1 && grid > cap ? cap : grid;
}
static bool run_pipeline(Context* ctx, BatchPlan& P) {
    const TableSet& ts = *P.ts; const Tables& T = ts.T; Workspace& W = P.W; const std::vector<StreamDesc>& sd = P.sd;
    const StreamDesc* dSD = P.dSD; const StreamIO* dIO = P.dIO;
    const int S = P.S, C = T.channels_out, ngs = P.ngs, nfs = P.nfs, nfr = P.nfr; const bool resv = P.resv, use_frame = P.use_frame;
    WorkSet& ws = ctx->ws; void* st = ctx->stream; const int64_t in_total = P.in_total;
    if (P.count_rej) {
        if (!ws.rejected.ensure(64) || !rt::dzero(ws.rejected.p, 8, st)) return false;
        int64_t nb = (in_total + 255) / 256;
        if (nb > 2048) nb = 2048;
        if (nb < 1) nb = 1;
        if (P.count_f32) LAUNCHB(KT_COUNT, g_count_rejected, (int)nb, 256, st, dIO, S, T.channels_in, T.pcm_limit, (unsigned long long*)ws.rejected.p);
        g_rej_pending = ctx;
    }
    if (P.ingest_tiles > 0) {
        P.paths |= LHIP_PATH_INGEST;
        LAUNCH(KT_INGEST, g_ingest, P.ingest_tiles, st, P.dING, S, T.pcm_limit, P.count_rej ? (unsigned long long*)ws.rejected.p : (unsigned long long*)nullptr);
    }
    if (use_frame) {
        QArgs qa; qa.T = T; qa.pb = ts.pb10; qa.W = W; qa.SD = dSD; qa.chain = 0; qa.nfs = nfs; qa.ctr = 0;
        P.paths |= resv ? LHIP_PATH_FRAME_RESV : LHIP_PATH_FRAME;
        if (resv) LAUNCHB(KT_QUANT, g_frame<1>, S, 64 * FR_WAVES, st, qa, dIO); else LAUNCHB(KT_QUANT, g_frame<0>, S, 64 * FR_WAVES, st, qa, dIO);
        if (resv) { bool any_flush = false; for (int i = 0; i < S; i++) any_flush |= sd[i].flush != 0; if (any_flush) { P.paths |= LHIP_PATH_RESV_FLUSH; LAUNCH(KT_BITS, g_resv_flush, S, st, T, W, dSD); } }
    } else {
    P.paths |= LHIP_PATH_SEPARATE | (T.rs_ratio != 1 ? LHIP_PATH_PREP : 0) | (T.psy_channels == 4 ? LHIP_PATH_PSY4 : 0);
    LAUNCH(KT_LOAD, g_load, S, st, T, W, dSD, dIO);
    if (T.rs_ratio != 1) {
        int64_t nb = (in_total / C + 255) / 256;
        if (nb > 8192) nb = 8192;
        if (nb < 1) nb = 1;
        LAUNCHB(KT_PREP, g_prep, (int)nb, 256, st, T, W, dSD, dIO, S);
    }
    LAUNCHB(KT_PSYA, g_psyA, XCD_GRID_W(ngs * C), 64 * WPB, st, T, W, dSD, dIO, 0, C);
    if (T.psy_channels == 4) LAUNCHB(KT_PSYA, g_psyA, XCD_GRID_W(ngs * 2), 64 * WPB, st, T, W, dSD, dIO, 2, 2);
    LAUNCH(KT_SCAN, g_scan_raw, (ngs + 63) / 64, st, T, W, dSD, ngs);
    LAUNCH(KT_SCAN, g_scan_attack, (ngs + 63) / 64, st, T, W, dSD, ngs);
    LAUNCH(KT_SCAN, g_scan_blocktype, (ngs + 63) / 64, st, T, W, dSD, ngs);
    bool forked = false;
    struct AuxJoin {
        void* aux = nullptr;
        ~AuxJoin() { if (aux) (void)hipStreamSynchronize((hipStream_t)aux); }
    } aux_guard;
    if (!g_kt_on) {
        if (!ws.aux_stream) {
            hipStream_t a; hipEvent_t e1, e2;
            if (hipStreamCreateWithFlags(&a, hipStreamNonBlocking) == hipSuccess && hipEventCreateWithFlags(&e1, hipEventDisableTiming) == hipSuccess &&
                hipEventCreateWithFlags(&e2, hipEventDisableTiming) == hipSuccess) { ws.aux_stream = a; ws.ev_fork = e1; ws.ev_join = e2; }
        }
        if (ws.aux_stream && hipEventRecord((hipEvent_t)ws.ev_fork, (hipStream_t)st) == hipSuccess &&
            hipStreamWaitEvent((hipStream_t)ws.aux_stream, (hipEvent_t)ws.ev_fork, 0) == hipSuccess) {
            LAUNCHB(KT_SCAN, g_scan_ath, S, ATH_NT, ws.aux_stream, T, W, dSD);
            aux_guard.aux = ws.aux_stream;
            HIPCK(hipEventRecord((hipEvent_t)ws.ev_join, (hipStream_t)ws.aux_stream));
            forked = true;
        }
    }
    if (!forked) LAUNCHB(KT_SCAN, g_scan_ath, S, ATH_NT, st, T, W, dSD);
    LAUNCH(KT_POLY, g_poly, XCD_GRID((ngs * C + POLY_PER_WAVE - 1) / POLY_PER_WAVE), st, T, W, dSD, dIO, ngs * C);
    LAUNCH(KT_MDCT, g_mdct, XCD_GRID(ngs), st, T, W, dSD);
    if (forked) { HIPCK(hipStreamWaitEvent((hipStream_t)st, (hipEvent_t)ws.ev_join, 0)); aux_guard.aux = nullptr; }
    if (resv) {
        QArgs qa; qa.T = T; qa.pb = ts.pb10; qa.W = W; qa.SD = dSD; qa.chain = 2; qa.nfs = nfs; qa.ctr = S <= ctx->num_cus ? 1 : 0;
        P.paths |= qa.ctr ? LHIP_PATH_RESV_STREAM_HELPERS : LHIP_PATH_RESV_STREAM_NOHELPERS;
        LAUNCHB(KT_QUANT, g_resv_stream, S, 64 * RS_WAVES, st, qa);
    } else {
    if (T.psy_channels == 4) LAUNCHB(KT_PSYB, g_psyB<4>, XCD_GRID_W(ngs), 64 * WPB, st, T, ts.pb10, W, dSD, -1);
    else LAUNCHB(KT_PSYB, g_psyB<2>, XCD_GRID_W(ngs), 64 * WPB, st, T, ts.pb10, W, dSD, -1);
    int qgrid = (nfs + QWAVES - 1) / QWAVES;
    if (qgrid > ctx->num_cus * 2) qgrid = ctx->num_cus * 2;
    qgrid = quant_grid_cap(qgrid);
#ifdef LHIP_PHASE_PROF
    const bool pair = false;
#else
    static const int pair_max = []() { const char* e = getenv("LAMEJS_HIP_PAIR_MAX_FRAMES"); return e ? atoi(e) : -1; }();
    const bool pair = (C == 2 && nfs <= (pair_max >= 0 ? pair_max : 6 * ctx->num_cus));
#endif
    const bool fastq = ts.fast && fast_quant_allowed();
    P.paths |= fastq ? LHIP_PATH_QUANT_FAST : pair ? LHIP_PATH_QUANT_PAIR : LHIP_PATH_QUANT_PERSISTENT;
    if (fastq) {
        QArgs qa; qa.T = T; qa.pb = ts.pb10; qa.W = W; qa.SD = dSD; qa.chain = 0; qa.nfs = nfs; qa.ctr = 0;
        const void* const fns[4] = {(const void*)g_quant_fast<0, 0>, (const void*)g_quant_fast<0, 1>, (const void*)g_quant_fast<1, 0>, (const void*)g_quant_fast<1, 1>};
        int& wg_per_cu = ctx->qfast_wg_per_cu[(C == 2 ? 2 : 0) + (ts.skip_tail ? 1 : 0)];
        if (wg_per_cu == 0) {
            int nb = 0;
            if (hipOccupancyMaxActiveBlocksPerMultiprocessor(&nb, fns[(C == 2 ? 2 : 0) + (ts.skip_tail ? 1 : 0)], 64 * QF_WAVES, 0) != hipSuccess || nb < 1) nb = 1;
            wg_per_cu = nb;
        }
        const int per_wg = C == 2 ? QF_WAVES / 2 : QF_WAVES;
        int fq = (nfs + per_wg - 1) / per_wg;
        if (fq > ctx->num_cus * wg_per_cu) fq = ctx->num_cus * wg_per_cu;
        fq = quant_grid_cap(fq);
        P.ql.workgroups = fq; P.ql.waves = QF_WAVES; P.ql.nfs = nfs; P.ql.kernel = QL_FAST; P.ql.pair = C == 2; P.ql.skip = ts.skip_tail;
        if (C == 2) { if (ts.skip_tail) LAUNCHB(KT_QUANT, (g_quant_fast<1, 1>), fq, 64 * QF_WAVES, st, qa); else LAUNCHB(KT_QUANT, (g_quant_fast<1, 0>), fq, 64 * QF_WAVES, st, qa); }
        else { if (ts.skip_tail) LAUNCHB(KT_QUANT, (g_quant_fast<0, 1>), fq, 64 * QF_WAVES, st, qa); else LAUNCHB(KT_QUANT, (g_quant_fast<0, 0>), fq, 64 * QF_WAVES, st, qa); }
    } else
    { QArgs qa; qa.T = T; qa.pb = ts.pb10; qa.W = W; qa.SD = dSD; qa.chain = 0; qa.nfs = nfs; qa.ctr = 0;
      P.ql.workgroups = pair ? nfs : qgrid; P.ql.waves = pair ? 2 : QWAVES; P.ql.nfs = nfs; P.ql.kernel = pair ? QL_PAIR : QL_PERSISTENT; P.ql.pair = pair; P.ql.skip = ts.skip_tail;
      if (pair) { if (ts.skip_tail) LAUNCHB(KT_QUANT, (g_quant_pair<0, 1>), nfs, 128, st, qa); else LAUNCHB(KT_QUANT, (g_quant_pair<0, 0>), nfs, 128, st, qa); }
      else { if (ts.skip_tail) LAUNCHB(KT_QUANT, (g_quant<0, 1>), qgrid, 64 * QWAVES, st, qa); else LAUNCHB(KT_QUANT, (g_quant<0, 0>), qgrid, 64 * QWAVES, st, qa); } }
    if (nfr > 0) {
        QArgs qa; qa.T = T; qa.pb = ts.pb10; qa.W = W; qa.SD = dSD; qa.chain = 1; qa.nfs = nfs; qa.ctr = 0;
        LAUNCHB(KT_VALIDATE, g_validate_fast, (nfs + 63) / 64, 256, st, T, W, dSD, nfs);
        int fgrid = (nfs + 63) / 64;
        if (ctx->fixup_wg_per_cu == 0) {
            int nb = 0;
            if (hipOccupancyMaxActiveBlocksPerMultiprocessor(&nb, (const void*)g_fixup<1>, 64 * QWAVES, 0) != hipSuccess || nb < 1) nb = 1;
            ctx->fixup_wg_per_cu = nb < LHIP_FIXUP_OCC / 2 ? nb : LHIP_FIXUP_OCC / 2;
        }
        if (fgrid > ctx->num_cus * ctx->fixup_wg_per_cu) fgrid = ctx->num_cus * ctx->fixup_wg_per_cu;
        if (fgrid < 1) fgrid = 1;
        P.paths |= fgrid == 1 ? LHIP_PATH_FIXUP_SINGLE : LHIP_PATH_FIXUP_COOP;
        const void* fixup_fn = ts.skip_tail ? (const void*)g_fixup<1> : (const void*)g_fixup<0>;
        if (fgrid == 1) { if (ts.skip_tail) LAUNCHB(KT_VALIDATE, g_fixup<1>, 1, 64 * QWAVES, st, qa); else LAUNCHB(KT_VALIDATE, g_fixup<0>, 1, 64 * QWAVES, st, qa); }
        else {
            kt_begin(KT_VALIDATE, st);
            void* kargs[] = {(void*)&qa};
            hipStream_t cst = (hipStream_t)st;
            if (ctx->own_stream) {
                if (!ctx->ev_coop[0]) { if (!rt::event_create(&ctx->ev_coop[0]) || !rt::event_create(&ctx->ev_coop[1])) return false; }
                if (!rt::event_record(ctx->ev_coop[0], st) || !rt::stream_wait_event(nullptr, ctx->ev_coop[0])) return false;
                cst = nullptr;
            }
            hipError_t e_ = hipLaunchCooperativeKernel(fixup_fn, dim3(fgrid), dim3(64 * QWAVES), kargs, 0, cst);
            if (ctx->own_stream && e_ == hipSuccess) { if (!rt::event_record(ctx->ev_coop[1], nullptr) || !rt::stream_wait_event(st, ctx->ev_coop[1])) return false; }
            kt_end(st);
            TRACE_SYNC(g_fixup_cooperative, st);
            if (e_ != hipSuccess) { set_err(std::string("g_fixup (cooperative launch): ") + hipGetErrorString(e_)); return false; }
        }
    }
    LAUNCH(KT_BITS, g_bits, nfs, st, T, W, dSD);
    }
    LAUNCH(KT_SAVE, g_save, S, st, T, W, dSD, dIO);
    }
    if (P.crc_mode == 2) {
        P.paths |= LHIP_PATH_OUT_CRC;
        LAUNCH(KT_OUT_CRC, g_out_crc, P.crc_parts, st, (const CrcDesc*)ws.crc_desc.p, S, (uint32_t*)ws.crc_part.p);
        LAUNCH(KT_OUT_CRC, g_out_crc_fold, S, st, (const CrcDesc*)ws.crc_desc.p, (const uint32_t*)ws.crc_part.p, P.crc_dst);
    }
    if (P.gain.stage_blocks > 0) {
        P.paths |= LHIP_PATH_GAIN;
        LAUNCHB(KT_GAIN_STAGE, g_gain_stage, P.gain.stage_blocks, GAIN_STAGE_NT, st, T, W, dSD, dIO, P.dGD, S);
        if (C == 2) LAUNCH(KT_GAIN, g_gain<2>, P.gain.waves, st, P.dGD, S); else LAUNCH(KT_GAIN, g_gain<1>, P.gain.waves, st, P.dGD, S);
    }
    return true;
}
```

### lamejs_amd/csrc/lhip_pipeline_sim.h

```cpp
#pragma once
#ifdef LHIP_WAVESIM
#define WAVE_RUN(...) wsim::run([&](int lane_) { __VA_ARGS__; })
#else
#define WAVE_RUN(...) do { const int lane_ = 0; __VA_ARGS__; } while (0)
#endif
#ifdef LHIP_WAVESIM
#define QUANT_RUN(chain_) do { if (pair) wsim::run_block(2, [&](int wave_, int lane_) { kb_quant<1, 0, 1>(T, ts.pb10, W, dSD, b, chain_, lane_, LQ2[wave_], QT, wave_, mbox); }); \
                       else WAVE_RUN(kb_quant<0, 0, 1>(T, ts.pb10, W, dSD, b, chain_, lane_, LQ, QT)); } while (0)
#else
#define QUANT_RUN(chain_) WAVE_RUN(kb_quant<0, 0, 1>(T, ts.pb10, W, dSD, b, chain_, lane_, LQ, QT))
#endif
static void gain_sim_run(const Tables& T, const Workspace& W, const StreamDesc* SD, const StreamIO* IO, const GainDesc* D, int S, int stage_blocks, int waves) {
    static thread_local float LG[LHIP_NL * 2 * GAIN_STRIDE];
    for (int b = 0; b < stage_blocks; b++) { const int s = gain_find_stream<true>(D, S, b); for (int t = 0; t < GAIN_STAGE_NT; t++) kb_gain_stage(T, W, SD, IO, D, s, (int64_t)(b - D[s].blk0) * GAIN_STAGE_NT + t); }
    for (int b = 0; b < waves; b++) {
        const int s = gain_find_stream<false>(D, S, b);
        if (D[s].channels == 2) WAVE_RUN(kb_gain<2>(D, s, b - D[s].wave0, lane_, LG)); else WAVE_RUN(kb_gain<1>(D, s, b - D[s].wave0, lane_, LG));
    }
}
enum { PROBE_SIM_WAVES = 3 };
static void quant_probe_sim_run(const Tables& T, const PowBase& pb, const ProbeIn* in, ProbeOut* out, int n, int grid) {
    static thread_local QuantLds LP[PROBE_SIM_WAVES]; static thread_local QuantTabs QT;
    q_load_tabs(T, QT, 0, 1);
    for (int b = 0; b < grid; b++)
        for (int r = b; r < n; r += grid) WAVE_RUN(kb_quant_probe(T, pb, in, out, r, lane_, LP[b], QT));
}
static inline bool g_kt_on_() { return false; }
static bool collect_kernel_times(void*) { return true; }
static bool collect_repair_stats(Context*, BatchPlan&, bool, const int32_t*) { return true; }
static bool run_pipeline(Context* ctx, BatchPlan& P) {
    const TableSet& ts = *P.ts; const Tables& T = ts.T; Workspace& W = P.W; const std::vector<StreamDesc>& sd = P.sd;
    const StreamDesc* dSD = P.dSD; const StreamIO* dIO = P.dIO;
    const int S = P.S, C = T.channels_out, ngs = P.ngs, nfs = P.nfs, nfr = P.nfr; const bool resv = P.resv, use_frame = P.use_frame;
    int64_t& repaired = P.repaired; int64_t& iters = P.iters;
    if (P.count_f32) g_rejected = (int64_t)kb_count_rejected(dIO, S, T.channels_in, T.pcm_limit, 0, 1);
    if (P.ingest_tiles > 0) {
        P.paths |= LHIP_PATH_INGEST;
        alignas(16) static thread_local uint8_t LI[ING_WINDOW];
        unsigned long long bad = 0;
        for (int b = 0; b < P.ingest_tiles; b++) { const int s = ingest_find_stream(P.dING, S, b); WAVE_RUN(const unsigned r = kb_ingest(P.dING, s, (int64_t)b - P.dING[s].blk0, lane_, LI, T.pcm_limit); if (lane_ == 0) bad += r); }
        if (P.count_rej) g_rejected += (int64_t)bad;
    }
    static thread_local PsyALds LA; static thread_local PsyBLds4 LB; static thread_local MdctLds LM; static thread_local PolyLds LP; static thread_local QuantLds LQ; static thread_local BitsLds LBi; static thread_local QuantTabs QT;
    q_load_tabs(T, QT, 0, 1);
    if (use_frame) {
        P.paths |= resv ? LHIP_PATH_FRAME_RESV : LHIP_PATH_FRAME;
        const int NW = FR_WAVES;
        alignas(16) static thread_local unsigned char UL[FR_WAVES][FR_LDS_PER_WAVE]; static thread_local int fmbox[12]; static thread_local CountShare fcs[2];
        for (int s = 0; s < S; s++) {
            fcs[0].state = CS_IDLE; fcs[1].state = CS_IDLE;
#ifdef LHIP_WAVESIM
            wsim::run_block(NW, [&](int wave_, int lane_) {
                for (int stage = 0; stage < FR_STAGES; stage++) {
                    if (resv ? frame_stage_empty<1>(stage, T) : frame_stage_empty<0>(stage, T)) continue;
                    if (resv) kb_frame_stage<1, 1>(stage, T, ts.pb10, W, dSD, dIO, s, wave_, NW, lane_, UL[wave_], QT, fmbox, fcs);
                    else kb_frame_stage<0, 1>(stage, T, ts.pb10, W, dSD, dIO, s, wave_, NW, lane_, UL[wave_], QT, fmbox, fcs);
                    wg_barrier();
                }
            });
#else
            for (int stage = 0; stage < FR_STAGES; stage++)
                for (int wv = 0; wv < NW; wv++) {
                    if (resv) kb_frame_stage<1, 0>(stage, T, ts.pb10, W, dSD, dIO, s, wv, NW, 0, UL[wv], QT, fmbox);
                    else kb_frame_stage<0, 0>(stage, T, ts.pb10, W, dSD, dIO, s, wv, NW, 0, UL[wv], QT, fmbox);
                }
#endif
        }
        if (resv) for (int s = 0; s < S; s++) if (sd[s].flush) P.paths |= LHIP_PATH_RESV_FLUSH;
        if (resv) for (int s = 0; s < S; s++) if (sd[s].flush) WAVE_RUN(kb_resv_flush(T, W, s, lane_, LBi, dIO[s].state->rv, W.out_bytes + s));
    } else {
    P.paths |= LHIP_PATH_SEPARATE | (T.rs_ratio != 1 ? LHIP_PATH_PREP : 0) | (T.psy_channels == 4 ? LHIP_PATH_PSY4 : 0);
    for (int s = 0; s < S; s++) WAVE_RUN(kb_load(T, W, dSD, dIO, s, lane_));
    if (T.rs_ratio != 1) kb_prep(T, W, dSD, dIO, S, 0, 1);
    for (int b = 0; b < ngs * C; b++) WAVE_RUN(kb_psyA(T, W, dSD, dIO, b / C, b % C, lane_, LA));
    if (T.psy_channels == 4) for (int b = 0; b < ngs * 2; b++) WAVE_RUN(kb_psyA(T, W, dSD, dIO, b / 2, 2 + b % 2, lane_, LA));
    for (int b = 0; b < ngs; b++) kb_scan_raw(T, W, dSD, b);
    for (int b = 0; b < ngs; b++) kb_scan_attack(T, W, dSD, b);
    for (int b = 0; b < ngs; b++) kb_scan_blocktype(T, W, dSD, b);
#ifdef LHIP_WAVESIM
    { static thread_local AthLds LAth; for (int s = 0; s < S; s++) wsim::run_block(ATH_NT / 64, [&](int wave_, int lane_) { kb_scan_ath(T, W, dSD, s, 64 * wave_ + lane_, LAth); }); }
#else
    { static thread_local AthLds LAth; for (int s = 0; s < S; s++) kb_scan_ath(T, W, dSD, s, 0, LAth); }
#endif
    if (!resv) for (int b = 0; b < ngs; b++) WAVE_RUN(kb_psyB<4>(T, ts.pb10, W, dSD, b, lane_, LB, -1));
    for (int b = 0; b < (ngs * C + POLY_PER_WAVE - 1) / POLY_PER_WAVE; b++) WAVE_RUN(kb_polyphase(T, W, dSD, dIO, b, ngs * C, lane_, LP));
    for (int b = 0; b < ngs; b++) WAVE_RUN(kb_mdct(T, W, dSD, b, lane_, LM));
    if (resv) {
#ifdef LHIP_WAVESIM
        P.paths |= LHIP_PATH_RESV_STREAM_HELPERS;
#else
        P.paths |= LHIP_PATH_RESV_STREAM_NOHELPERS;
#endif
        alignas(16) static thread_local unsigned char RU[RS_WAVES][RS_LDS_PER_WAVE]; static thread_local int rmbox[4]; static thread_local CountShare rcs[2];
        for (int s = 0; s < S; s++) {
            ResvState RV = dIO[s].state->rv;
            int32_t nout = 0;
            const int F = sd[s].nframes;
#ifdef LHIP_WAVESIM
            wsim::run_block(RS_WAVES, [&](int wave_, int lane_) {
                for (int k = 0; k <= F; k++)
                    for (int stage = 0; stage < RS_STAGES; stage++) { kb_resv_stage<1>(stage, T, ts.pb10, W, dSD, s, k, F, wave_, lane_, RU[wave_], QT, rmbox, RV, &nout, rcs); wg_barrier(); }
                if (wave_ == 3 && sd[s].flush) kb_resv_flush(T, W, s, lane_, *(BitsLds*)RU[3], RV, &nout);
            });
#else
            for (int k = 0; k <= F; k++)
                for (int stage = 0; stage < RS_STAGES; stage++)
                    for (int wv = 0; wv < RS_WAVES; wv++) kb_resv_stage<0>(stage, T, ts.pb10, W, dSD, s, k, F, wv, 0, RU[wv], QT, rmbox, RV, &nout);
            if (sd[s].flush) kb_resv_flush(T, W, s, 0, *(BitsLds*)RU[3], RV, &nout);
#endif
            dIO[s].state->rv = RV;
            W.out_bytes[s] = nout;
        }
    } else {
#ifdef LHIP_WAVESIM
    static thread_local QuantLds LQ2[2]; static thread_local int mbox[4];
    static const int pair_max = []() { const char* e = getenv("LAMEJS_HIP_PAIR_MAX_FRAMES"); return e ? atoi(e) : 12; }();
    const bool pair = (C == 2 && nfs <= pair_max);
#endif
    const bool fastq = ts.fast && fast_quant_allowed();
#ifdef LHIP_WAVESIM
    P.ql.workgroups = (!fastq && pair) ? nfs : 1; P.ql.waves = (!fastq && pair) ? 2 : 8; P.ql.kernel = fastq ? QL_FAST : pair ? QL_PAIR : QL_PERSISTENT; P.ql.pair = fastq ? C == 2 : pair;
#else
    P.ql.workgroups = 1; P.ql.waves = 3; P.ql.kernel = fastq ? QL_FAST : QL_PERSISTENT; P.ql.pair = fastq && C == 2;
#endif
    P.ql.nfs = nfs; P.ql.skip = ts.skip_tail;
#ifdef LHIP_WAVESIM
    P.paths |= fastq ? LHIP_PATH_QUANT_FAST : pair ? LHIP_PATH_QUANT_PAIR : LHIP_PATH_QUANT_PERSISTENT;
#else
    P.paths |= fastq ? LHIP_PATH_QUANT_FAST : LHIP_PATH_QUANT_PERSISTENT;
#endif
    if (fastq) {
#if defined(LHIP_WAVESIM)
        static thread_local QuantLds LF[8]; static thread_local FastPair FP[4];
        int ctr = 0;
        memset(FP, 0, sizeof FP);
        wsim::run_block(8, [&](int wave_, int lane_) {
            int hint[3] = {-1, -1, -1};
            for (int round = 1;; round++) {
                int f = 0;
                if (C == 2) {
                    FastPair& fp = FP[wave_ >> 1];
                    if ((wave_ & 1) == 0) { if (lane_ == 0) f = ctr++; f = wave_bcast(f, 0); fast_pair_publish_slot(fp, round, f, lane_); }
                    else f = fast_pair_await_slot(fp, round, lane_);
                    if (f >= nfs) break;
                    kb_quant_fast<1, 1>(T, ts.pb10, W, dSD, f, lane_, LF[wave_], QT, hint, wave_ & 1, &fp, round);
                } else {
                    if (lane_ == 0) f = ctr++;
                    f = wave_bcast(f, 0);
                    if (f >= nfs) break;
                    kb_quant_fast<0, 1>(T, ts.pb10, W, dSD, f, lane_, LF[wave_], QT, hint);
                }
            }
        });
#else
        int hints[3][3] = {{-1, -1, -1}, {-1, -1, -1}, {-1, -1, -1}};
        for (int b = 0; b < nfs; b++) WAVE_RUN(kb_quant_fast<0, 1>(T, ts.pb10, W, dSD, b, lane_, LQ, QT, hints[b % 3]));
#endif
    } else
#if defined(LHIP_WAVESIM)
    if (!pair) {
        static thread_local QuantLds LQ8[8]; static thread_local TailShare TS;
        int ctr = 0;
        TS.drawing = 8; for (int w = 0; w < 8; w++) TS.offer[w].state = 0;
        wsim::run_block(8, [&](int wave_, int lane_) {
            int hint[3] = {-1, -1, -1};
            for (;;) {
                int f = 0;
                if (lane_ == 0) f = ctr++;
                f = wave_bcast(f, 0);
                if (f >= nfs) break;
                kb_quant_th<1>(T, ts.pb10, W, dSD, f, lane_, LQ8[wave_], QT, hint, TS, wave_);
            }
            if (C == 2) tail_help<1>(T, ts.pb10, W, dSD, lane_, LQ8, wave_, 8, QT, TS);
        });
    } else
#endif
    {
        int hints[3][3] = {{-1, -1, -1}, {-1, -1, -1}, {-1, -1, -1}};
        for (int b = 0; b < nfs; b++) {
#ifdef LHIP_WAVESIM
            if (pair) { QUANT_RUN(0); continue; }
            int hl[64][3];
            for (int l = 0; l < 64; l++) for (int q = 0; q < 3; q++) hl[l][q] = hints[b % 3][q];
            WAVE_RUN(kb_quant<0, 0, 1>(T, ts.pb10, W, dSD, b, 0, lane_, LQ, QT, -1, nullptr, nullptr, hl[lane_]));
            for (int l = 1; l < 64; l++) for (int q = 0; q < 3; q++) if (hl[l][q] != hl[0][q]) { set_err("wavesim: seed hint not wave-uniform"); return false; }
            for (int q = 0; q < 3; q++) hints[b % 3][q] = hl[0][q];
#else
            WAVE_RUN(kb_quant<0, 0, 1>(T, ts.pb10, W, dSD, b, 0, lane_, LQ, QT, -1, nullptr, nullptr, hints[b % 3]));
#endif
        }
    }
    for (;;) {
        W.nflagged[0] = 0; W.nflagged[1] = 0;
        for (int b = 0; b < nfs; b++) kb_validate_fast(T, W, dSD, b);
        for (int i = 0; i < W.nflagged[1]; i++) WAVE_RUN(kb_validate<1>(T, ts.pb10, W, dSD, W.slow_list[i], lane_, LQ, QT));
        const int nf = W.nflagged[0];
        if (nf == 0) break;
        repaired += nf; iters++;
        for (int b = 0; b < nfs; b++) QUANT_RUN(1);
        if (iters > nfr + 2) { set_err("seed-chain repair did not converge"); return false; }
    }
    for (int b = 0; b < nfs; b++) WAVE_RUN(kb_bits(T, W, dSD, b, lane_, LBi));
    }
    for (int s = 0; s < S; s++) WAVE_RUN(kb_save(T, W, dSD, dIO, s, lane_));
    }
    if (P.crc_mode == 2) {
        P.paths |= LHIP_PATH_OUT_CRC;
        const CrcDesc* D = (const CrcDesc*)ctx->ws.crc_desc.p; uint32_t* part = (uint32_t*)ctx->ws.crc_part.p;
        for (int b = 0; b < P.crc_parts; b++) { const int s = crc_find_stream(D, S, b); WAVE_RUN(kb_out_crc(D, s, b - D[s].part0, lane_, part)); }
        for (int s = 0; s < S; s++) WAVE_RUN(kb_crc_fold(D, s, lane_, part, P.crc_dst));
    }
    if (P.gain.stage_blocks > 0) {
        P.paths |= LHIP_PATH_GAIN;
        gain_sim_run(T, W, dSD, dIO, P.dGD, S, P.gain.stage_blocks, P.gain.waves);
    }
    return true;
}
#undef QUANT_RUN
#undef WAVE_RUN
```

Before: 2.388 million frames/s.

## Split psychoacoustic stage A and skip short-block analysis when no short blocks follow

For large non-reservoir batches, psyA is split into part 1, which runs before the block-type scans, and part 2, which runs after them. Part 2 and psyB then skip the short-window FFT, energy, spreading and threshold work whenever the neighbouring granules are not SHORT_TYPE. This removes most short-block computation for tonal input such as sine waves, at the cost of one extra kernel launch and some re-staging of data between the parts. The diff also replaces the context scan used for stats lookup with a cached last-batch pointer.

Result: faster. 2.447 million frames/s, median of 6 (+2.5%).

```diff
diff --git a/lamejs_amd/csrc/k_psy.h b/lamejs_amd/csrc/k_psy.h
--- a/lamejs_amd/csrc/k_psy.h
+++ b/lamejs_amd/csrc/k_psy.h
@@ -129,6 +129,18 @@
 #endif
 }
 
+LHIP_DEV int psy_need_s(const Tables& T, const Workspace& W, const StreamDesc& sd, int gslot) {
+    if (gslot >= sd.gslot0 + T.mode_gr * sd.nframes) return 1;
+    const int C = T.channels_out;
+    int s = 0;
+    for (int ch = 0; ch < C; ch++) s |= W.blocktype[(int64_t)(gslot + 1) * C + ch] == SHORT_TYPE;
+    return uni(s);
+}
+LHIP_DEV int psy_need_f(const Tables& T, const Workspace& W, const StreamDesc& sd, int gslot) {
+    if (psy_need_s(T, W, sd, gslot)) return 1;
+    return psy_need_s(T, W, sd, gslot + 1);
+}
+
 template <int F32, int UNIT, int MIX>
 LHIP_DEV void psya_stage_new(const PcmSrc& P, int first, int lane, float* fz) {
     typedef typename std::conditional<F32 != 0, float, int16_t>::type elem_t;
@@ -166,8 +178,9 @@
     }
 }
 
-template <int PART = 0>
+template <int PART = 0, int LAZY = 0>
 LHIP_DEV void kb_psyA(const Tables& T, const Workspace& W, const StreamDesc* SD, const StreamIO* IO, int gslot, int ch, int lane, PsyALds& L) {
+    static_assert(LAZY == 0 || PART == 2, "the lazy form reads the block types: it exists for part 2 behind the scans only");
     const int C = T.channels_out, Cp = T.psy_channels;
     const int st = W.gslot_stream[gslot];
     const StreamDesc sd = SD[st];
@@ -198,6 +211,7 @@
     PSY_DECL();
     PSY_STAMP(0);
 
+    const bool shortw = LAZY ? psy_need_f(T, W, sd, gslot) != 0 : true;
     if (PART == 4) goto psya_tail;
     if (PART == 0 || PART == 1) {
         const float* fir = L.fz + 397;
@@ -256,14 +270,15 @@
     PSY_STAMP(1);
     if (ch >= 2) {
         const float* fl = W.fht + (int64_t)gslot * 2 * FHT_STRIDE;
-        for (int i = lane; i < FHT_STRIDE; i += LHIP_NL) {
+        const int nfht = shortw ? FHT_STRIDE : BLKSIZE;
+        for (int i = lane; i < nfht; i += LHIP_NL) {
             const double l = fl[i], r = fl[FHT_STRIDE + i];
             const float v = (ch == 2) ? (float)((l + r) * LHIP_SQRT2 * 0.5) : (float)((l - r) * LHIP_SQRT2 * 0.5);
             if (i < BLKSIZE) L.fz[fzp(i)] = v; else (&L.fs[0][0])[fzp(i - BLKSIZE)] = v;
         }
         wave_sync();
     } else {
-    for (int it = lane; it < 3 * (BLKSIZE_s / 8); it += LHIP_NL) {
+    if (shortw) for (int it = lane; it < 3 * (BLKSIZE_s / 8); it += LHIP_NL) {
         const int b = it / (BLKSIZE_s / 8), j = it - b * (BLKSIZE_s / 8);
         const int k = (576 / 3) * (b + 1);
         const int i = T.fft_rv_tbl[j << 2] & 0xff;
@@ -331,14 +346,15 @@
 #pragma unroll
         for (int k1 = 4, kx = 2; k1 < BLKSIZE; k1 <<= 2, kx <<= 2) {
             fht_pass(L.fz, BLKSIZE, k1, kx, lane, LHIP_NL, 0, T.fht_twiddle + 4 * off);
-            if (k1 < BLKSIZE_s) fht_pass_blocks(&L.fs[0][0], 3, BLKSIZE_s, k1, kx, lane, LHIP_NL, T.fht_twiddle + 4 * off);
+            if (k1 < BLKSIZE_s && shortw) fht_pass_blocks(&L.fs[0][0], 3, BLKSIZE_s, k1, kx, lane, LHIP_NL, T.fht_twiddle + 4 * off);
             wave_sync();
             off += kx - 1;
         }
     }
     if (Cp == 4) {
         float* fo = W.fht + ((int64_t)gslot * 2 + ch) * FHT_STRIDE;
-        for (int i = lane; i < FHT_STRIDE; i += LHIP_NL) fo[i] = (i < BLKSIZE) ? L.fz[fzp(i)] : (&L.fs[0][0])[fzp(i - BLKSIZE)];
+        const int nfht = shortw ? FHT_STRIDE : BLKSIZE;
+        for (int i = lane; i < nfht; i += LHIP_NL) fo[i] = (i < BLKSIZE) ? L.fz[fzp(i)] : (&L.fs[0][0])[fzp(i - BLKSIZE)];
     }
     }
 
@@ -354,9 +370,11 @@
             else if (j <= BLKSIZE / 2) { const double re = L.fz[fzp(j)], im = L.fz[fzp(BLKSIZE - j)]; el[u] = (float)((re * re + im * im) * 0.5); }
         }
 #pragma unroll
+        for (int u = 0; u < KS; u++) es[u] = 0.f;
+        if (shortw) {
+#pragma unroll
         for (int u = 0; u < KS; u++) {
             const int it = lane + LHIP_NL * u;
-            es[u] = 0.f;
             if (it < 3 * (BLKSIZE_s / 2 + 1)) {
                 const int b = it / (BLKSIZE_s / 2 + 1), j = it - b * (BLKSIZE_s / 2 + 1);
                 const float* fsf = &L.fs[0][0];
@@ -364,13 +382,16 @@
                 else { const double re = fsf[fzp(b * BLKSIZE_s + j)], im = fsf[fzp(b * BLKSIZE_s + BLKSIZE_s - j)]; es[u] = (float)((re * re + im * im) * 0.5); }
             }
         }
+        }
         wave_sync();
 #pragma unroll
         for (int u = 0; u < KE; u++) { const int j = lane + LHIP_NL * u; if (j <= BLKSIZE / 2) PSYA_FE(L)[j] = el[u]; }
+        if (shortw) {
 #pragma unroll
         for (int u = 0; u < KS; u++) {
             const int it = lane + LHIP_NL * u;
             if (it < 3 * (BLKSIZE_s / 2 + 1)) { const int b = it / (BLKSIZE_s / 2 + 1), j = it - b * (BLKSIZE_s / 2 + 1); PSYA_FES(L, b)[j] = es[u]; }
+        }
         }
     }
     wave_sync();
@@ -464,7 +485,7 @@
         }
     }
 #endif
-    for (int it = lane; it < 3 * T.npart_s; it += LHIP_NL) {
+    if (shortw) for (int it = lane; it < 3 * T.npart_s; it += LHIP_NL) {
         const int sblock = it / T.npart_s, b = it - sblock * T.npart_s;
         double ebb = 0;
         int j = T.lineoff_s[b];
@@ -497,7 +518,7 @@
         W.eb_l[o * EBL_STRIDE + b] = ebv;
         W.mask_idx[o * EBL_STRIDE + b] = k;
     }
-    for (int b = lane; b < CBANDS; b += LHIP_NL) {
+    if (shortw) for (int b = lane; b < CBANDS; b += LHIP_NL) {
         float ecbv[3] = {0.f, 0.f, 0.f}, ebv[3] = {0.f, 0.f, 0.f};
         if (b < T.npart_s) {
             enum { MT = 12 };
@@ -808,7 +829,7 @@
     return 0.0;
 }
 
-template <int NCH> LHIP_DEV void kb_psyB(const Tables& T, const PowBase& pb10, const Workspace& W, const StreamDesc* SD, int gslot, int lane, PsyBLdsT<NCH>& L, int par = -1,
+template <int NCH, int LAZY = 0> LHIP_DEV void kb_psyB(const Tables& T, const PowBase& pb10, const Workspace& W, const StreamDesc* SD, int gslot, int lane, PsyBLdsT<NCH>& L, int par = -1,
                                          int resv_size = 0, int resv_max = 0) {
     const int C = T.channels_out, Cp = T.psy_channels;
     const int st = W.gslot_stream[gslot];
@@ -816,6 +837,7 @@
     const int q = gslot - sd.gslot0 - 1;
     if (q < 0) return;
     if (par >= 0 && q % T.mode_gr != par) return;
+    const bool shortw = LAZY ? psy_need_s(T, W, sd, gslot) != 0 : true;
     double pcfact = 0.0;
     if (!T.disable_reservoir) pcfact = resv_max == 0 ? 0.0 : (double)resv_size / resv_max * 0.5;
     const int fs = sd.fslot0 + q / T.mode_gr;
@@ -856,7 +878,7 @@
         }
         wave_sync();
     }
-    for (int ch = 0; ch < Cp; ch++) {
+    if (shortw) for (int ch = 0; ch < Cp; ch++) {
         const int64_t o = (int64_t)gslot * Cp + ch;
         const int pshort = W.prev_short[(int64_t)gslot * C + (ch & 1)];
         for (int it = lane; it < 3 * T.npart_s; it += LHIP_NL) {
@@ -908,7 +930,8 @@
             Eo[E_EN_L + sb] = en_f;
             Eo[E_THM_L + sb] = thm_f;
         }
-        for (int it = lane; it < 3 * SBMAX_s; it += LHIP_NL) {
+        if (!shortw) for (int it = lane; it < 3 * SBMAX_s; it += LHIP_NL) { Eo[E_EN_S + it] = 0.f; Eo[E_THM_S + it] = 0.f; }
+        if (shortw) for (int it = lane; it < 3 * SBMAX_s; it += LHIP_NL) {
             const int sblock = it / SBMAX_s, sb = it - sblock * SBMAX_s;
             const float* ebs = W.eb_s + o * EBS_STRIDE + sblock * CBANDS;
             const float* thr = L.thr_s[ch][sblock];
@@ -939,7 +962,7 @@
         }
     }
     wave_sync();
-    for (int ch = 0; ch < Cp; ch++) {
+    if (shortw) for (int ch = 0; ch < Cp; ch++) {
         const int64_t o = (int64_t)gslot * Cp + ch;
         const float* pk = W.peaks + o * PK_STRIDE;
         const int att = W.att_clean[o];
@@ -963,10 +986,11 @@
         }
     }
     wave_sync();
+    const int nthm = shortw ? SBMAX_l + 3 * SBMAX_s : SBMAX_l;
     if ((T.mode == 0 || T.mode == 1) && T.interChRatio > 0.0 && C > 1) {
         const double r_ = T.interChRatio;
         float nl[2] = {0.f, 0.f};
-        for (int i = lane; i < SBMAX_l + 3 * SBMAX_s; i += LHIP_NL) {
+        for (int i = lane; i < nthm; i += LHIP_NL) {
             const int idx = E_THM_L + i;
             const double l = L.E[0][idx], r = L.E[1][idx];
             nl[0] = (float)(l + r * r_);
@@ -981,7 +1005,7 @@
         const bool do_ns = d_abs(msfix) > 0.0;
         const double athlower_l = do_ns ? v8_pow_base(pb10, T.ATHlower * ath_adjust) : 0.0;
         const double athlower_s = athlower_l * ((double)BLKSIZE_s / BLKSIZE);
-        for (int i = lane; i < SBMAX_l + 3 * SBMAX_s; i += LHIP_NL) {
+        for (int i = lane; i < nthm; i += LHIP_NL) {
             const int it = E_THM_L + i, ie = E_EN_L + i;
             const bool lng = i < SBMAX_l;
             const int sb = lng ? i : (i - SBMAX_l) / 3;
diff --git a/lamejs_amd/csrc/lhip_api.cpp b/lamejs_amd/csrc/lhip_api.cpp
--- a/lamejs_amd/csrc/lhip_api.cpp
+++ b/lamejs_amd/csrc/lhip_api.cpp
@@ -651,7 +651,7 @@
     if (what == 9) { const size_t n = cap < sizeof g_call_prof ? cap : sizeof g_call_prof; memcpy(dst, g_call_prof, n); return (int64_t)n; }
 #endif
     Context* ctx = nullptr;
-    { std::lock_guard<std::mutex> lk(g_ctx_mu); for (auto& kv : g_ctx) if (kv.second->ws.have_last) ctx = kv.second.get(); }
+    { std::lock_guard<std::mutex> lk(g_ctx_mu); ctx = g_last_batch_ctx; }
     if (!ctx) { set_err("no batch has run"); return LHIP_ERR_INTERNAL; }
     std::lock_guard<std::mutex> lk(ctx->mu);
     rt::set_device(ctx->device);
diff --git a/lamejs_amd/csrc/lhip_batch.h b/lamejs_amd/csrc/lhip_batch.h
--- a/lamejs_amd/csrc/lhip_batch.h
+++ b/lamejs_amd/csrc/lhip_batch.h
@@ -98,6 +98,7 @@
 struct BatchPlan {
     TableSet* ts = nullptr;
     bool dev_io = false, resv = false, count_rej = false, use_frame = false, small = false;
+    bool psy_lazy = false;
     bool count_f32 = false;
     int ingest = 0, ingest_tiles = 0; size_t ingest_floats = 0; const IngestDesc* dING = nullptr;
     int S = 0, nfs = 0, ngs = 0, nfr = 0, maxF = 0;
@@ -162,6 +163,12 @@
     }
     static const bool no_frame = []() { const char* e = getenv("LAMEJS_HIP_NO_FRAME_KERNEL"); return e && e[0] == '1'; }();
     P.use_frame = P.maxF <= 1 && !no_frame && S <= ctx->num_cus;
+    {
+        const char* e = getenv("LAMEJS_PSY_LAZY_MIN_FRAMES");
+        int64_t thr = 6 * (int64_t)ctx->num_cus < 1024 ? 1024 : 6 * (int64_t)ctx->num_cus;
+        if (e && *e) { thr = atoll(e); if (thr < 0) thr = 0; }
+        P.psy_lazy = !P.use_frame && !resv && (int64_t)P.nfs >= thr;
+    }
     return true;
 }
 static bool bind_workspace(Context* ctx, BatchPlan& P) {
@@ -438,5 +445,6 @@
     g_stat_frames = P.nfr; g_stat_repaired = P.repaired; g_stat_iters = P.iters; g_last_paths = P.paths; g_last_quant = P.ql;
     WorkSet& ws = ctx->ws;
     ws.lastW = P.W; ws.lastC = P.ts->T.channels_out; ws.lastCp = P.ts->T.psy_channels; ws.have_last = true;
-    return true;
-}
+    { std::lock_guard<std::mutex> lk(g_ctx_mu); g_last_batch_ctx = ctx; }
+    return true;
+}
diff --git a/lamejs_amd/csrc/lhip_context.h b/lamejs_amd/csrc/lhip_context.h
--- a/lamejs_amd/csrc/lhip_context.h
+++ b/lamejs_amd/csrc/lhip_context.h
@@ -56,6 +56,7 @@
 
 static std::mutex g_ctx_mu;
 static std::map<int, std::unique_ptr<Context>> g_ctx;
+static Context* g_last_batch_ctx = nullptr;
 
 static Context* get_context(int device) {
     std::lock_guard<std::mutex> lk(g_ctx_mu);
diff --git a/lamejs_amd/csrc/lhip_kernels.h b/lamejs_amd/csrc/lhip_kernels.h
--- a/lamejs_amd/csrc/lhip_kernels.h
+++ b/lamejs_amd/csrc/lhip_kernels.h
@@ -16,11 +16,11 @@
     return (g >= 0 && it < n) ? it : -1;
 }
 #define WAVE_LDS(TYPE, NAME) __shared__ TYPE NAME##_[WPB]; TYPE& NAME = NAME##_[__builtin_amdgcn_readfirstlane((int)(threadIdx.x >> 6))]
-__global__ __launch_bounds__(64 * WPB) void g_psyA(Tables T, Workspace W, const StreamDesc* SD, const StreamIO* IO, int chn0, int nch) {
+template <int PART> __global__ __launch_bounds__(64 * WPB) void g_psyA(Tables T, Workspace W, const StreamDesc* SD, const StreamIO* IO, int chn0, int nch) {
     WAVE_LDS(PsyALds, L);
     int lane;
     const int it = xcd_wave_item(W.ngslots * nch, &lane);
-    if (it >= 0) kb_psyA(T, W, SD, IO, it / nch, chn0 + it % nch, lane, L);
+    if (it >= 0) kb_psyA<PART, PART == 2>(T, W, SD, IO, it / nch, chn0 + it % nch, lane, L);
 }
 __global__ __launch_bounds__(256) void g_prep(Tables T, Workspace W, const StreamDesc* SD, const StreamIO* IO, int nstreams) {
     kb_prep(T, W, SD, IO, nstreams, (int64_t)blockIdx.x * blockDim.x + threadIdx.x, (int64_t)gridDim.x * blockDim.x);
@@ -33,11 +33,11 @@
 __global__ __launch_bounds__(64) void g_scan_attack(Tables T, Workspace W, const StreamDesc* SD, int ngs) { const int g = blockIdx.x * 64 + threadIdx.x; if (g < ngs) kb_scan_attack(T, W, SD, g); }
 __global__ __launch_bounds__(64) void g_scan_blocktype(Tables T, Workspace W, const StreamDesc* SD, int ngs) { const int g = blockIdx.x * 64 + threadIdx.x; if (g < ngs) kb_scan_blocktype(T, W, SD, g); }
 __global__ __launch_bounds__(ATH_NT) void g_scan_ath(Tables T, Workspace W, const StreamDesc* SD) { __shared__ AthLds L; kb_scan_ath(T, W, SD, blockIdx.x, threadIdx.x, L); }
-template <int NCH> __global__ __launch_bounds__(64 * WPB) void g_psyB(Tables T, PowBase pb, Workspace W, const StreamDesc* SD, int par) {
+template <int NCH, int LAZY> __global__ __launch_bounds__(64 * WPB) void g_psyB(Tables T, PowBase pb, Workspace W, const StreamDesc* SD, int par) {
     WAVE_LDS(PsyBLdsT<NCH>, L);
     int lane;
     const int it = xcd_wave_item(W.ngslots, &lane);
-    if (it >= 0) kb_psyB<NCH>(T, pb, W, SD, it, lane, L, par);
+    if (it >= 0) kb_psyB<NCH, LAZY>(T, pb, W, SD, it, lane, L, par);
 }
 __global__ __launch_bounds__(64, 4) void g_poly(Tables T, Workspace W, const StreamDesc* SD, const StreamIO* IO, int nitems) {
     __shared__ PolyLds L;
diff --git a/lamejs_amd/csrc/lhip_pipeline_hip.h b/lamejs_amd/csrc/lhip_pipeline_hip.h
--- a/lamejs_amd/csrc/lhip_pipeline_hip.h
+++ b/lamejs_amd/csrc/lhip_pipeline_hip.h
@@ -45,11 +45,21 @@
         if (nb < 1) nb = 1;
         LAUNCHB(KT_PREP, g_prep, (int)nb, 256, st, T, W, dSD, dIO, S);
     }
-    LAUNCHB(KT_PSYA, g_psyA, XCD_GRID_W(ngs * C), 64 * WPB, st, T, W, dSD, dIO, 0, C);
-    if (T.psy_channels == 4) LAUNCHB(KT_PSYA, g_psyA, XCD_GRID_W(ngs * 2), 64 * WPB, st, T, W, dSD, dIO, 2, 2);
+    const bool lazy = P.psy_lazy;
+    if (lazy) {
+        LAUNCHB(KT_PSYA, g_psyA<1>, XCD_GRID_W(ngs * C), 64 * WPB, st, T, W, dSD, dIO, 0, C);
+        if (T.psy_channels == 4) LAUNCHB(KT_PSYA, g_psyA<1>, XCD_GRID_W(ngs * 2), 64 * WPB, st, T, W, dSD, dIO, 2, 2);
+    } else {
+        LAUNCHB(KT_PSYA, g_psyA<0>, XCD_GRID_W(ngs * C), 64 * WPB, st, T, W, dSD, dIO, 0, C);
+        if (T.psy_channels == 4) LAUNCHB(KT_PSYA, g_psyA<0>, XCD_GRID_W(ngs * 2), 64 * WPB, st, T, W, dSD, dIO, 2, 2);
+    }
     LAUNCH(KT_SCAN, g_scan_raw, (ngs + 63) / 64, st, T, W, dSD, ngs);
     LAUNCH(KT_SCAN, g_scan_attack, (ngs + 63) / 64, st, T, W, dSD, ngs);
     LAUNCH(KT_SCAN, g_scan_blocktype, (ngs + 63) / 64, st, T, W, dSD, ngs);
+    if (lazy) {
+        LAUNCHB(KT_PSYA, g_psyA<2>, XCD_GRID_W(ngs * C), 64 * WPB, st, T, W, dSD, dIO, 0, C);
+        if (T.psy_channels == 4) LAUNCHB(KT_PSYA, g_psyA<2>, XCD_GRID_W(ngs * 2), 64 * WPB, st, T, W, dSD, dIO, 2, 2);
+    }
     bool forked = false;
     struct AuxJoin {
         void* aux = nullptr;
@@ -78,8 +88,8 @@
         P.paths |= qa.ctr ? LHIP_PATH_RESV_STREAM_HELPERS : LHIP_PATH_RESV_STREAM_NOHELPERS;
         LAUNCHB(KT_QUANT, g_resv_stream, S, 64 * RS_WAVES, st, qa);
     } else {
-    if (T.psy_channels == 4) LAUNCHB(KT_PSYB, g_psyB<4>, XCD_GRID_W(ngs), 64 * WPB, st, T, ts.pb10, W, dSD, -1);
-    else LAUNCHB(KT_PSYB, g_psyB<2>, XCD_GRID_W(ngs), 64 * WPB, st, T, ts.pb10, W, dSD, -1);
+    if (T.psy_channels == 4) { if (lazy) LAUNCHB(KT_PSYB, (g_psyB<4, 1>), XCD_GRID_W(ngs), 64 * WPB, st, T, ts.pb10, W, dSD, -1); else LAUNCHB(KT_PSYB, (g_psyB<4, 0>), XCD_GRID_W(ngs), 64 * WPB, st, T, ts.pb10, W, dSD, -1); }
+    else { if (lazy) LAUNCHB(KT_PSYB, (g_psyB<2, 1>), XCD_GRID_W(ngs), 64 * WPB, st, T, ts.pb10, W, dSD, -1); else LAUNCHB(KT_PSYB, (g_psyB<2, 0>), XCD_GRID_W(ngs), 64 * WPB, st, T, ts.pb10, W, dSD, -1); }
     int qgrid = (nfs + QWAVES - 1) / QWAVES;
     if (qgrid > ctx->num_cus * 2) qgrid = ctx->num_cus * 2;
     qgrid = quant_grid_cap(qgrid);
diff --git a/lamejs_amd/csrc/lhip_pipeline_sim.h b/lamejs_amd/csrc/lhip_pipeline_sim.h
--- a/lamejs_amd/csrc/lhip_pipeline_sim.h
+++ b/lamejs_amd/csrc/lhip_pipeline_sim.h
@@ -72,17 +72,28 @@
     P.paths |= LHIP_PATH_SEPARATE | (T.rs_ratio != 1 ? LHIP_PATH_PREP : 0) | (T.psy_channels == 4 ? LHIP_PATH_PSY4 : 0);
     for (int s = 0; s < S; s++) WAVE_RUN(kb_load(T, W, dSD, dIO, s, lane_));
     if (T.rs_ratio != 1) kb_prep(T, W, dSD, dIO, S, 0, 1);
-    for (int b = 0; b < ngs * C; b++) WAVE_RUN(kb_psyA(T, W, dSD, dIO, b / C, b % C, lane_, LA));
-    if (T.psy_channels == 4) for (int b = 0; b < ngs * 2; b++) WAVE_RUN(kb_psyA(T, W, dSD, dIO, b / 2, 2 + b % 2, lane_, LA));
+    const bool lazy = P.psy_lazy;
+    if (lazy) {
+        for (int b = 0; b < ngs * C; b++) WAVE_RUN(kb_psyA<1>(T, W, dSD, dIO, b / C, b % C, lane_, LA));
+        if (T.psy_channels == 4) for (int b = 0; b < ngs * 2; b++) WAVE_RUN(kb_psyA<1>(T, W, dSD, dIO, b / 2, 2 + b % 2, lane_, LA));
+    } else {
+        for (int b = 0; b < ngs * C; b++) WAVE_RUN(kb_psyA(T, W, dSD, dIO, b / C, b % C, lane_, LA));
+        if (T.psy_channels == 4) for (int b = 0; b < ngs * 2; b++) WAVE_RUN(kb_psyA(T, W, dSD, dIO, b / 2, 2 + b % 2, lane_, LA));
+    }
     for (int b = 0; b < ngs; b++) kb_scan_raw(T, W, dSD, b);
     for (int b = 0; b < ngs; b++) kb_scan_attack(T, W, dSD, b);
     for (int b = 0; b < ngs; b++) kb_scan_blocktype(T, W, dSD, b);
+    if (lazy) {
+        for (int b = 0; b < ngs * C; b++) WAVE_RUN((kb_psyA<2, 1>(T, W, dSD, dIO, b / C, b % C, lane_, LA)));
+        if (T.psy_channels == 4) for (int b = 0; b < ngs * 2; b++) WAVE_RUN((kb_psyA<2, 1>(T, W, dSD, dIO, b / 2, 2 + b % 2, lane_, LA)));
+    }
 #ifdef LHIP_WAVESIM
     { static thread_local AthLds LAth; for (int s = 0; s < S; s++) wsim::run_block(ATH_NT / 64, [&](int wave_, int lane_) { kb_scan_ath(T, W, dSD, s, 64 * wave_ + lane_, LAth); }); }
 #else
     { static thread_local AthLds LAth; for (int s = 0; s < S; s++) kb_scan_ath(T, W, dSD, s, 0, LAth); }
 #endif
-    if (!resv) for (int b = 0; b < ngs; b++) WAVE_RUN(kb_psyB<4>(T, ts.pb10, W, dSD, b, lane_, LB, -1));
+    if (!resv && lazy) for (int b = 0; b < ngs; b++) WAVE_RUN((kb_psyB<4, 1>(T, ts.pb10, W, dSD, b, lane_, LB, -1)));
+    else if (!resv) for (int b = 0; b < ngs; b++) WAVE_RUN(kb_psyB<4>(T, ts.pb10, W, dSD, b, lane_, LB, -1));
     for (int b = 0; b < (ngs * C + POLY_PER_WAVE - 1) / POLY_PER_WAVE; b++) WAVE_RUN(kb_polyphase(T, W, dSD, dIO, b, ngs * C, lane_, LP));
     for (int b = 0; b < ngs; b++) WAVE_RUN(kb_mdct(T, W, dSD, b, lane_, LM));
     if (resv) {
```
